# hyrise/hyrise

Hardware: AMD Instinct MI355X
Metric: rows/sec TableScan+JoinHash, TPC-H SF10 lineitem (higher is better)
Workload: dtype u16

## Files before the change

### __graft_entry__.py

```python
import os
import subprocess
import sys

ROOT = os.path.dirname(os.path.abspath(__file__))
CSRC = os.path.join(ROOT, "hyrise_amd", "csrc")
LIB = os.path.join(ROOT, "hyrise_amd", "libhyrise_amd.so")
HIP_SOURCES = ["runtime.hip", "scan.hip", "join.hip", "aggregate.hip", "aggregate_wide.hip", "aggregate_widest.hip", "projection.hip", "projection_expression.hip", "scan_expression.hip", "exchange.hip", "boundary.hip", "comm.hip", "plan.hip", "result_pool.hip", "sort.hip", "union_positions.hip", "join_sort_merge.hip", "join_nested_loop.hip", "product.hip", "like.hip", "string_order.hip", "string_gather.hip"]


def _newer(target, sources):
    if not os.path.exists(target):
        return True
    t = os.path.getmtime(target)
    return any(os.path.getmtime(s) > t for s in sources)


def _build_library(sources, deps, force):
    from concurrent.futures import ThreadPoolExecutor
    hipcc = os.environ.get("HIPCC", "/opt/rocm/bin/hipcc")
    flags = ["--offload-arch=gfx950", "-O3", "-std=c++17", "-fPIC", "-Wall", "-Wno-unused-function"] + os.environ.get("HY_CXXFLAGS", "").split()
    import hashlib
    objdir = os.path.join(ROOT, "build", "obj" + ("-" + hashlib.sha1(" ".join(flags).encode()).hexdigest()[:8] if os.environ.get("HY_CXXFLAGS") else ""))
    os.makedirs(objdir, exist_ok=True)
    headers = [d for d in deps if not d.endswith(".hip")]
    jobs = []
    for source in sources:
        obj = os.path.join(objdir, os.path.basename(source)[:-4] + ".o")
        included = [os.path.join(CSRC, "aggregate.hip")] if source.endswith(("aggregate_wide.hip", "aggregate_widest.hip")) else []
        if force or _newer(obj, [source] + included + headers):
            jobs.append([hipcc] + flags + ["-c", source, "-o", obj])
    with ThreadPoolExecutor(max_workers=max(1, min(len(jobs), os.cpu_count() or 1))) as pool:
        for result in pool.map(lambda cmd: subprocess.run(cmd, cwd=ROOT, capture_output=True, text=True), jobs):
            if result.returncode != 0:
                sys.stderr.write(result.stdout + result.stderr)
                raise subprocess.CalledProcessError(result.returncode, result.args)
            if result.stderr.strip():
                sys.stderr.write(result.stderr)
    objects = [os.path.join(objdir, os.path.basename(source)[:-4] + ".o") for source in sources]
    subprocess.check_call([hipcc, "--offload-arch=gfx950", "-shared", "-fPIC", "-o", os.environ.get("HY_LIBRARY_OUT", LIB)] + objects + ["-ldl"], cwd=ROOT)


def build(force=False):
    sources = [os.path.join(CSRC, s) for s in HIP_SOURCES]
    deps = sources + [os.path.join(CSRC, h) for h in ("hy_device.hpp", "hy_options.hpp", "hy_decode.hpp", "hy_arithmetic.hpp", "hy_scan_job.hpp", "hy_expression.hpp", "hy_expression_rows.hpp", "join_pkfk.hpp", "join_star.hpp", "aggregate_small.hpp", "fused_small.hpp", "sort_words.hpp", "sort_keys.hpp", "join_outer_emit.hpp", "string_entries.hpp")] + [os.path.join(ROOT, "include", "hyrise_amd.h")]
    if force or _newer(LIB, deps):
        _build_library(sources, deps, force)
    host_tests = os.path.join(ROOT, "tests", "cpp", "host_tests")
    host_sources = [os.path.join(ROOT, "tests", "cpp", "host_tests.cpp"), os.path.join(ROOT, "hyrise_amd", "host", "hyrise_host.hpp"), LIB]
    if force or _newer(host_tests, host_sources):
        subprocess.check_call(["g++", "-std=c++17", "-O1", "-Wall", "-Wno-unused-function", "-o", host_tests, host_sources[0],
                               "-L" + os.path.join(ROOT, "hyrise_amd"), "-lhyrise_amd", "-Wl,-rpath,$ORIGIN/../../hyrise_amd"], cwd=ROOT)
    sort_tests = os.path.join(ROOT, "tests", "cpp", "sort_tests")
    sort_sources = [os.path.join(ROOT, "tests", "cpp", "sort_tests.cpp"), host_sources[1], LIB]
    if force or _newer(sort_tests, sort_sources):
        subprocess.check_call(["g++", "-std=c++17", "-O1", "-Wall", "-Wno-unused-function", "-o", sort_tests, sort_sources[0],
                               "-L" + os.path.join(ROOT, "hyrise_amd"), "-lhyrise_amd", "-Wl,-rpath,$ORIGIN/../../hyrise_amd"], cwd=ROOT)
    union_tests = os.path.join(ROOT, "tests", "cpp", "union_positions_tests")
    union_sources = [os.path.join(ROOT, "tests", "cpp", "union_positions_tests.cpp"), host_sources[1], LIB]
    if force or _newer(union_tests, union_sources):
        subprocess.check_call(["g++", "-std=c++17", "-O1", "-Wall", "-Wno-unused-function", "-o", union_tests, union_sources[0],
                               "-L" + os.path.join(ROOT, "hyrise_amd"), "-lhyrise_amd", "-Wl,-rpath,$ORIGIN/../../hyrise_amd"], cwd=ROOT)
    smj_tests = os.path.join(ROOT, "tests", "cpp", "join_sort_merge_tests")
    smj_sources = [os.path.join(ROOT, "tests", "cpp", "join_sort_merge_tests.cpp"), host_sources[1], LIB]
    if force or _newer(smj_tests, smj_sources):
        subprocess.check_call(["g++", "-std=c++17", "-O1", "-Wall", "-Wno-unused-function", "-o", smj_tests, smj_sources[0],
                               "-L" + os.path.join(ROOT, "hyrise_amd"), "-lhyrise_amd", "-Wl,-rpath,$ORIGIN/../../hyrise_amd"], cwd=ROOT)
    nlj_tests = os.path.join(ROOT, "tests", "cpp", "join_nested_loop_tests")
    nlj_sources = [os.path.join(ROOT, "tests", "cpp", "join_nested_loop_tests.cpp"), host_sources[1], LIB]
    if force or _newer(nlj_tests, nlj_sources):
        subprocess.check_call(["g++", "-std=c++17", "-O1", "-Wall", "-Wno-unused-function", "-o", nlj_tests, nlj_sources[0],
                               "-L" + os.path.join(ROOT, "hyrise_amd"), "-lhyrise_amd", "-Wl,-rpath,$ORIGIN/../../hyrise_amd"], cwd=ROOT)
    limit_tests = os.path.join(ROOT, "tests", "cpp", "limit_tests")
    limit_sources = [os.path.join(ROOT, "tests", "cpp", "limit_tests.cpp"), host_sources[1], LIB]
    if force or _newer(limit_tests, limit_sources):
        subprocess.check_call(["g++", "-std=c++17", "-O1", "-Wall", "-Wno-unused-function", "-o", limit_tests, limit_sources[0],
                               "-L" + os.path.join(ROOT, "hyrise_amd"), "-lhyrise_amd", "-Wl,-rpath,$ORIGIN/../../hyrise_amd"], cwd=ROOT)
    aggregate_columns_tests = os.path.join(ROOT, "tests", "cpp", "aggregate_columns_tests")
    aggregate_columns_sources = [os.path.join(ROOT, "tests", "cpp", "aggregate_columns_tests.cpp"), host_sources[1], LIB]
    if force or _newer(aggregate_columns_tests, aggregate_columns_sources):
        subprocess.check_call(["g++", "-std=c++17", "-O1", "-Wall", "-Wno-unused-function", "-o", aggregate_columns_tests, aggregate_columns_sources[0],
                               "-L" + os.path.join(ROOT, "hyrise_amd"), "-lhyrise_amd", "-Wl,-rpath,$ORIGIN/../../hyrise_amd"], cwd=ROOT)
    in_list_tests = os.path.join(ROOT, "tests", "cpp", "in_list_tests")
    in_list_sources = [os.path.join(ROOT, "tests", "cpp", "in_list_tests.cpp"), host_sources[1], LIB]
    if force or _newer(in_list_tests, in_list_sources):
        subprocess.check_call(["g++", "-std=c++17", "-O1", "-Wall", "-Wno-unused-function", "-o", in_list_tests, in_list_sources[0],
                               "-L" + os.path.join(ROOT, "hyrise_amd"), "-lhyrise_amd", "-Wl,-rpath,$ORIGIN/../../hyrise_amd"], cwd=ROOT)
    projection_tests = os.path.join(ROOT, "tests", "cpp", "projection_tests")
    projection_sources = [os.path.join(ROOT, "tests", "cpp", "projection_tests.cpp"), host_sources[1], LIB]
    if force or _newer(projection_tests, projection_sources):
        subprocess.check_call(["g++", "-std=c++17", "-O1", "-Wall", "-Wno-unused-function", "-o", projection_tests, projection_sources[0],
                               "-L" + os.path.join(ROOT, "hyrise_amd"), "-lhyrise_amd", "-Wl,-rpath,$ORIGIN/../../hyrise_amd"], cwd=ROOT)
    expression_scan_tests = os.path.join(ROOT, "tests", "cpp", "expression_scan_tests")
    expression_scan_sources = [os.path.join(ROOT, "tests", "cpp", "expression_scan_tests.cpp"), host_sources[1], LIB]
    if force or _newer(expression_scan_tests, expression_scan_sources):
        subprocess.check_call(["g++", "-std=c++17", "-O1", "-Wall", "-Wno-unused-function", "-o", expression_scan_tests, expression_scan_sources[0],
                               "-L" + os.path.join(ROOT, "hyrise_amd"), "-lhyrise_amd", "-Wl,-rpath,$ORIGIN/../../hyrise_amd"], cwd=ROOT)
    product_tests = os.path.join(ROOT, "tests", "cpp", "product_tests")
    product_sources = [os.path.join(ROOT, "tests", "cpp", "product_tests.cpp"), host_sources[1], LIB]
    if force or _newer(product_tests, product_sources):
        subprocess.check_call(["g++", "-std=c++17", "-O1", "-Wall", "-Wno-unused-function", "-o", product_tests, product_sources[0],
                               "-L" + os.path.join(ROOT, "hyrise_amd"), "-lhyrise_amd", "-Wl,-rpath,$ORIGIN/../../hyrise_amd"], cwd=ROOT)
    like_device_tests = os.path.join(ROOT, "tests", "cpp", "like_device_tests")
    like_device_sources = [os.path.join(ROOT, "tests", "cpp", "like_device_tests.cpp"), host_sources[1], LIB]
    if force or _newer(like_device_tests, like_device_sources):
        subprocess.check_call(["g++", "-std=c++17", "-O1", "-Wall", "-Wno-unused-function", "-o", like_device_tests, like_device_sources[0],
                               "-L" + os.path.join(ROOT, "hyrise_amd"), "-lhyrise_amd", "-Wl,-rpath,$ORIGIN/../../hyrise_amd"], cwd=ROOT)
    string_columns_tests = os.path.join(ROOT, "tests", "cpp", "string_columns_tests")
    string_columns_sources = [os.path.join(ROOT, "tests", "cpp", "string_columns_tests.cpp"), host_sources[1], LIB]
    if force or _newer(string_columns_tests, string_columns_sources):
        subprocess.check_call(["g++", "-std=c++17", "-O1", "-Wall", "-Wno-unused-function", "-o", string_columns_tests, string_columns_sources[0],
                               "-L" + os.path.join(ROOT, "hyrise_amd"), "-lhyrise_amd", "-Wl,-rpath,$ORIGIN/../../hyrise_amd"], cwd=ROOT)
    string_order_tests = os.path.join(ROOT, "tests", "cpp", "string_order_tests")
    string_order_sources = [os.path.join(ROOT, "tests", "cpp", "string_order_tests.cpp"), host_sources[1], LIB]
    if force or _newer(string_order_tests, string_order_sources):
        subprocess.check_call(["g++", "-std=c++17", "-O1", "-Wall", "-Wno-unused-function", "-o", string_order_tests, string_order_sources[0],
                               "-L" + os.path.join(ROOT, "hyrise_amd"), "-lhyrise_amd", "-Wl,-rpath,$ORIGIN/../../hyrise_amd"], cwd=ROOT)
    string_gather_tests = os.path.join(ROOT, "tests", "cpp", "string_gather_tests")
    string_gather_sources = [os.path.join(ROOT, "tests", "cpp", "string_gather_tests.cpp"), host_sources[1], LIB]
    if force or _newer(string_gather_tests, string_gather_sources):
        subprocess.check_call(["g++", "-std=c++17", "-O1", "-Wall", "-Wno-unused-function", "-o", string_gather_tests, string_gather_sources[0],
                               "-L" + os.path.join(ROOT, "hyrise_amd"), "-lhyrise_amd", "-Wl,-rpath,$ORIGIN/../../hyrise_amd"], cwd=ROOT)
    chain = os.path.join(ROOT, "tests", "cpp", "operator_chain")
    chain_sources = [os.path.join(ROOT, "tests", "cpp", "operator_chain.cpp"), host_sources[1], LIB]
    if force or _newer(chain, chain_sources):
        subprocess.check_call(["g++", "-std=c++17", "-O2", "-Wall", "-Wno-unused-function", "-o", chain, chain_sources[0],
                               "-L" + os.path.join(ROOT, "hyrise_amd"), "-lhyrise_amd", "-ldl", "-Wl,-rpath,$ORIGIN/../../hyrise_amd"], cwd=ROOT)
    multi_tests = os.path.join(ROOT, "tests", "cpp", "multi_gpu_tests")
    multi_sources = [os.path.join(ROOT, "tests", "cpp", "multi_gpu_tests.cpp"), os.path.join(ROOT, "hyrise_amd", "host", "multi_gpu.hpp"), host_sources[1], LIB]
    if force or _newer(multi_tests, multi_sources):
        subprocess.check_call(["g++", "-std=c++17", "-O1", "-Wall", "-Wno-unused-function", "-pthread", "-o", multi_tests, multi_sources[0],
                               "-L" + os.path.join(ROOT, "hyrise_amd"), "-lhyrise_amd", "-Wl,-rpath,$ORIGIN/../../hyrise_amd"], cwd=ROOT)
    subprocess.check_call(["make", "-s", "-C", os.path.join(ROOT, "oracle"), "liboracle.so"])
    reference = os.environ.get("HY_REFERENCE", "/root/reference")
    if os.path.isdir(os.path.join(reference, "third_party", "tpch-dbgen")):
        subprocess.check_call(["make", "-s", "-C", os.path.join(ROOT, "oracle"), "ref", f"REFERENCE={reference}"])
    if ROOT not in sys.path:
        sys.path.insert(0, ROOT)
    import hyrise_amd
    from hyrise_amd import abi
    abi.load_library()


def smoke():
    if ROOT not in sys.path:
        sys.path.insert(0, ROOT)
    sys.path.insert(0, os.path.join(ROOT, "tests"))
    import numpy as np
    from hyrise_amd import abi
    from hyrise_amd.operators import make_predicate, table_scan
    from hyrise_amd.storage import DeviceColumn, make_column
    import support

    lib = abi.load_library()
    abi.check(lib.hy_init(0))
    rng = np.random.default_rng(1)
    days = (rng.integers(0, 2406, 500_000) + rng.integers(1, 122, 500_000)).astype(np.int32)
    host = make_column(days, None, abi.ENC_DICTIONARY)
    dev = DeviceColumn(host)
    predicate = make_predicate(abi.PRED_BETWEEN_UPPER_EXCLUSIVE, abi.TYPE_INT, 731, 1096)
    got = table_scan(dev, predicate)
    want = support.oracle_scan(host, predicate)
    support.assert_scan_equal(got, want, "smoke")
    print(f"smoke OK: {got.total} matches of {host.rows} rows, PosLists bit-identical to the oracle")


if __name__ == "__main__":
    build(force="--force" in sys.argv)
    if "--smoke" in sys.argv:
        smoke()
```

### hyrise_amd/abi.py

```python
import ctypes as C
import os

HERE = os.path.dirname(os.path.abspath(__file__))
LIB_PATH = os.path.join(HERE, "libhyrise_amd.so")

OK, ERR_INVALID, ERR_UNSUPPORTED, ERR_DEVICE, ERR_CAPACITY = 0, 1, 2, 3, 4
TYPE_NULL, TYPE_INT, TYPE_LONG, TYPE_FLOAT, TYPE_DOUBLE, TYPE_STRING = range(6)
(PRED_EQUALS, PRED_NOT_EQUALS, PRED_LESS_THAN, PRED_LESS_THAN_EQUALS, PRED_GREATER_THAN, PRED_GREATER_THAN_EQUALS,
 PRED_BETWEEN_INCLUSIVE, PRED_BETWEEN_LOWER_EXCLUSIVE, PRED_BETWEEN_UPPER_EXCLUSIVE, PRED_BETWEEN_EXCLUSIVE,
 PRED_IN, PRED_NOT_IN, PRED_LIKE, PRED_NOT_LIKE, PRED_LIKE_INSENSITIVE, PRED_NOT_LIKE_INSENSITIVE,
 PRED_IS_NULL, PRED_IS_NOT_NULL) = range(18)
(JOIN_INNER, JOIN_LEFT, JOIN_RIGHT, JOIN_FULL_OUTER, JOIN_CROSS, JOIN_SEMI, JOIN_ANTI_NULL_AS_TRUE,
 JOIN_ANTI_NULL_AS_FALSE) = range(8)
AGG_MIN, AGG_MAX, AGG_SUM, AGG_AVG, AGG_COUNT, AGG_COUNT_DISTINCT, AGG_STDDEV_SAMP, AGG_ANY = range(8)
ENC_UNENCODED, ENC_DICTIONARY, ENC_FRAME_OF_REFERENCE, ENC_REFERENCE, ENC_MVCC, ENC_RUN_LENGTH, ENC_LZ4 = range(7)
SORT_NONE, SORT_ASCENDING_NULLS_FIRST, SORT_DESCENDING_NULLS_FIRST, SORT_ASCENDING_NULLS_LAST, SORT_DESCENDING_NULLS_LAST = range(5)
MEM_HOST, MEM_DEVICE = 0, 1
CHUNK_SCANNED, CHUNK_ALL_MATCH, CHUNK_NONE_MATCH = 0, 1, 2
INVALID_VALUE_ID = 0xFFFFFFFF
INVALID_CHUNK_ID = 0xFFFFFFFF
FOR_BLOCK_SIZE = 2048
SCAN_MATERIALIZE_ALL_MATCH = 1
SCAN_CHUNK_REGIONS = 2
POSLIST_DENSE, POSLIST_CHUNK_REGIONS = 0, 1
POOL_KEEP_MEDIAN = 1
CHUNK_DEFAULT_SIZE = 65535


class RowID(C.Structure):
    _fields_ = [("chunk_id", C.c_uint32), ("chunk_offset", C.c_uint32)]


class Segment(C.Structure):
    _fields_ = [("encoding", C.c_uint32), ("data_type", C.c_uint32), ("size", C.c_uint32), ("width", C.c_uint32),
                ("data", C.c_void_p), ("aux", C.c_void_p), ("aux_size", C.c_uint32), ("ref_chunk_id", C.c_uint32),
                ("nulls", C.c_void_p), ("ref", C.c_void_p), ("sorted_by", C.c_uint32), ("bits", C.c_uint32)]


class Lz4Blocks(C.Structure):
    _fields_ = [("blocks", C.POINTER(C.c_void_p)), ("block_bytes", C.POINTER(C.c_uint32)), ("block_count", C.c_uint32), ("block_size", C.c_uint32),
                ("last_block_size", C.c_uint32), ("dictionary_bytes", C.c_uint32), ("dictionary", C.c_void_p)]


class Value(C.Union):
    _fields_ = [("i32", C.c_int32), ("i64", C.c_int64), ("f32", C.c_float), ("f64", C.c_double),
                ("value_id", C.c_uint32)]


class Predicate(C.Structure):
    _fields_ = [("condition", C.c_uint32), ("value_type", C.c_uint32), ("value", Value), ("value2", Value),
                ("per_chunk_lower", C.c_void_p), ("per_chunk_upper", C.c_void_p), ("per_chunk_found", C.c_void_p),
                ("column_is_nullable", C.c_uint32), ("reserved", C.c_uint32), ("match_words", C.c_void_p), ("match_word_offsets", C.c_void_p)]


MAX_IN_LIST = 256
MAX_LIKE_PATTERN = 256
LIKE_ANY_ONE, LIKE_ANY_RUN = 0x100, 0x200


class StringDictionaryChunk(C.Structure):
    _fields_ = [("n_entries", C.c_uint32), ("string_length", C.c_uint32), ("chars", C.c_void_p), ("offsets", C.c_void_p)]


class InList(C.Structure):
    _fields_ = [("value_type", C.c_uint32), ("n_values", C.c_uint32), ("values", C.c_void_p), ("negated", C.c_uint32), ("column_is_nullable", C.c_uint32),
                ("per_chunk_value_ids", C.c_void_p)]


class ScanResult(C.Structure):
    _fields_ = [("mem", C.c_uint32), ("flags", C.c_uint32), ("matches", C.c_void_p), ("capacity", C.c_uint64),
                ("offsets", C.c_void_p), ("counts", C.c_void_p), ("chunk_state", C.c_void_p),
                ("total_matches", C.c_uint64)]


class JoinResult(C.Structure):
    _fields_ = [("mem", C.c_uint32), ("radix_bits", C.c_uint32), ("left_pos", C.c_void_p), ("right_pos", C.c_void_p),
                ("capacity", C.c_uint64), ("slice_offsets", C.c_void_p), ("slice_capacity", C.c_uint32),
                ("n_slices", C.c_uint32), ("n_pairs", C.c_uint64), ("left_is_build", C.c_uint32),
                ("flags", C.c_uint32), ("status", C.c_void_p)]


JOIN_ASYNC = 1


class JoinStatus(C.Structure):
    _fields_ = [("n_pairs", C.c_uint64), ("n_slices", C.c_uint32), ("fits", C.c_uint32), ("build_confirmed", C.c_uint32), ("error", C.c_uint32),
                ("reserved", C.c_uint64)]


class SortMergeResult(C.Structure):
    _fields_ = [("mem", C.c_uint32), ("reserved", C.c_uint32), ("left_pos", C.c_void_p), ("right_pos", C.c_void_p), ("capacity", C.c_uint64),
                ("n_pairs", C.c_uint64), ("n_matched", C.c_uint64), ("n_left_outer", C.c_uint64)]


class NestedLoopResult(C.Structure):
    _fields_ = [("mem", C.c_uint32), ("reserved", C.c_uint32), ("left_pos", C.c_void_p), ("right_pos", C.c_void_p), ("capacity", C.c_uint64), ("n_pairs", C.c_uint64)]


class ProductResult(C.Structure):
    _fields_ = [("mem", C.c_uint32), ("reserved", C.c_uint32), ("left_pos", C.c_void_p), ("right_pos", C.c_void_p), ("pair_offsets", C.c_void_p),
                ("capacity", C.c_uint64), ("n_rows", C.c_uint64)]


class JoinPredicate(C.Structure):
    _fields_ = [("left_column", C.c_void_p), ("right_column", C.c_void_p), ("condition", C.c_uint32), ("reserved", C.c_uint32)]


MAX_SECONDARY_PREDICATES = 4
NLJ_MAX_COMPARISONS = 250_000_000_000
NLJ_MAX_TEMPORARY_BYTES = 1 << 31
(OPT_ALLOW_ANY_ARCH, OPT_JOIN_RANK_TABLE, OPT_JOIN_HINT, OPT_JOIN_BREAK_HINT, OPT_JOIN_PKFK, OPT_JOIN_LDS_BUILD, OPT_JOIN_LDS_BUILD_TILES, OPT_JOIN_FILL_WGS_PER_CU,
 OPT_JOIN_HAND_OVER_RANKS, OPT_AGG_PARTITION_BITS, OPT_AGG_SPILL_SHIFT, OPT_AGG_SMALL_DOMAIN, OPT_FUSED_SMALL_DOMAIN, OPT_SCAN_TWO_COLUMNS, OPT_STAR_FUSED_PROBE, OPT_STAR_FUSED_FINISH,
 OPT_LDS_ORDERED_ATOMICS, OPT_PRODUCT_NONTEMPORAL) = range(18)
KERNEL_OTHER, KERNEL_SCAN, KERNEL_JOIN_PROBE, KERNEL_JOIN_COUNT, KERNEL_JOIN_BUILD, KERNEL_AGGREGATE, KERNEL_PROJECTION, KERNEL_LIKE, KERNEL_STRING_RANK = range(9)
ARITH_ADD, ARITH_SUB, ARITH_MUL, ARITH_DIV, ARITH_MOD = range(5)


class Operand(C.Structure):
    _fields_ = [("column", C.c_void_p), ("literal_type", C.c_uint32), ("literal", Value)]


MAX_PROJECTION_NODES, MAX_PROJECTION_DEPTH, MAX_PROJECTION_COLUMNS, MAX_PROJECTION_TESTS = 32, 6, 8, 4
(PROJ_COLUMN, PROJ_LITERAL, PROJ_ARITHMETIC, PROJ_COMPARISON, PROJ_COLUMN_TEST, PROJ_IS_NULL, PROJ_IS_NOT_NULL, PROJ_AND, PROJ_OR, PROJ_UNARY_MINUS, PROJ_CASE,
 PROJ_BETWEEN, PROJ_CAST, PROJ_EXTRACT, PROJ_FUNCTION, PROJ_SUBQUERY, PROJ_PARAMETER) = range(17)


class ProjectionNode(C.Structure):
    _fields_ = [("kind", C.c_uint32), ("op", C.c_uint32), ("index", C.c_uint32), ("literal_type", C.c_uint32), ("literal", Value)]


class ProjectionTest(C.Structure):
    _fields_ = [("column", C.c_void_p), ("predicate", Predicate), ("in_list", C.POINTER(InList))]


class ProjectionProgram(C.Structure):
    _fields_ = [("n_nodes", C.c_uint32), ("n_columns", C.c_uint32), ("n_tests", C.c_uint32), ("reserved", C.c_uint32),
                ("columns", C.c_void_p * MAX_PROJECTION_COLUMNS), ("tests", ProjectionTest * MAX_PROJECTION_TESTS), ("nodes", ProjectionNode * MAX_PROJECTION_NODES)]


UNION_FORCE_SORT = 1
UNION_MAX_CLUSTERS = 8
SORT_LIMIT_FORCE_FULL_SORT, SORT_LIMIT_FORCE_SELECT = 1, 2


class SortKey(C.Structure):
    _fields_ = [("column", C.c_void_p), ("mode", C.c_uint32), ("reserved", C.c_uint32)]


class AggregateSpec(C.Structure):
    _fields_ = [("function", C.c_uint32), ("column", C.c_void_p)]


EXPR_COLUMN, EXPR_LITERAL, EXPR_ARITHMETIC = range(3)
MAX_EXPRESSION_NODES, MAX_FILTERS = 12, 4
FILTER_VALIDATE = 0x100


class ExpressionNode(C.Structure):
    _fields_ = [("kind", C.c_uint32), ("op", C.c_uint32), ("column", C.c_void_p), ("literal_type", C.c_uint32), ("reserved", C.c_uint32),
                ("literal", Value)]


class Expression(C.Structure):
    _fields_ = [("n_nodes", C.c_uint32), ("reserved", C.c_uint32), ("nodes", ExpressionNode * MAX_EXPRESSION_NODES)]


class Filter(C.Structure):
    _fields_ = [("column", C.c_void_p), ("predicate", Predicate)]


class FusedAggregate(C.Structure):
    _fields_ = [("function", C.c_uint32), ("reserved", C.c_uint32), ("input", C.POINTER(Expression))]


class AggregateColumn(C.Structure):
    _fields_ = [("data_type", C.c_uint32), ("reserved", C.c_uint32), ("values", C.c_void_p), ("is_null", C.c_void_p)]


class AggregateResult(C.Structure):
    _fields_ = [("mem", C.c_uint32), ("group_capacity", C.c_uint32), ("n_groups", C.c_uint32),
                ("reserved", C.c_uint32), ("group_row_ids", C.c_void_p), ("columns", C.POINTER(AggregateColumn))]


class AggregateColumns(C.Structure):
    _fields_ = [("skip_groupby_mask", C.c_uint64), ("n_groups", C.c_uint32), ("reserved", C.c_uint32),
                ("aggregate_columns", C.POINTER(C.c_void_p)), ("groupby_columns", C.POINTER(C.c_void_p)), ("group_row_ids", C.c_void_p)]


STAR_NO_OP = 0xFFFFFFFF
MAX_STAR_DIMENSIONS, MAX_STAR_AGGREGATES = 8, 8


class StarDimension(C.Structure):
    _fields_ = [("key", C.c_void_p), ("filter_column", C.c_void_p), ("predicate", Predicate), ("fact_key", C.c_void_p)]


class StarColumn(C.Structure):
    _fields_ = [("table", C.c_uint32), ("reserved", C.c_uint32), ("column", C.c_void_p)]


class StarAggregate(C.Structure):
    _fields_ = [("function", C.c_uint32), ("op", C.c_uint32), ("left", StarColumn), ("right", StarColumn)]


MAX_STAR_FILTERS = 4


class StarFilter(C.Structure):
    _fields_ = [("column", C.c_void_p), ("predicate", Predicate), ("in_list", C.POINTER(InList))]


class StarDimensionWhere(C.Structure):
    _fields_ = [("key", C.c_void_p), ("fact_key", C.c_void_p), ("filters", C.POINTER(StarFilter)), ("n_filters", C.c_uint32), ("reserved", C.c_uint32)]


SYMBOLS = [
    ("hy_abi_version", C.c_int32, []),
    ("hy_init", C.c_int32, [C.c_int32]),
    ("hy_set_option", C.c_int32, [C.c_uint32, C.c_int64]),
    ("hy_get_option", C.c_int32, [C.c_uint32, C.POINTER(C.c_int64)]),
    ("hy_shutdown", C.c_int32, []),
    ("hy_last_error", C.c_char_p, []),
    ("hy_set_stream", C.c_int32, [C.c_void_p]),
    ("hy_synchronize", C.c_int32, []),
    ("hy_device_malloc", C.c_int32, [C.POINTER(C.c_void_p), C.c_size_t]),
    ("hy_device_free", C.c_int32, [C.c_void_p]),
    ("hy_memcpy_h2d", C.c_int32, [C.c_void_p, C.c_void_p, C.c_size_t]),
    ("hy_memcpy_d2h", C.c_int32, [C.c_void_p, C.c_void_p, C.c_size_t]),
    ("hy_device_count", C.c_int32, [C.POINTER(C.c_int32)]),
    ("hy_set_profiling", C.c_int32, [C.c_int32]),
    ("hy_profile_read", C.c_int32, [C.POINTER(C.c_float), C.POINTER(C.c_uint32)]),
    ("hy_profile_read_kernel", C.c_int32, [C.c_uint32, C.POINTER(C.c_float), C.POINTER(C.c_uint32)]),
    ("hy_profile_event_overhead", C.c_int32, [C.POINTER(C.c_float)]),
    ("hy_bind_device", C.c_int32, [C.c_int32]),
    ("hy_comm_unique_id", C.c_int32, [C.c_void_p]),
    ("hy_comm_init_rank", C.c_int32, [C.c_void_p, C.c_uint32, C.c_uint32, C.POINTER(C.c_void_p)]),
    ("hy_comm_init_all", C.c_int32, [C.POINTER(C.c_int32), C.c_uint32, C.POINTER(C.c_void_p)]),
    ("hy_comm_destroy", C.c_int32, [C.c_void_p]),
    ("hy_comm_rank", C.c_int32, [C.c_void_p, C.POINTER(C.c_uint32), C.POINTER(C.c_uint32)]),
    ("hy_comm_group_begin", C.c_int32, []),
    ("hy_comm_group_end", C.c_int32, []),
    ("hy_comm_all_reduce", C.c_int32, [C.c_void_p, C.c_void_p, C.c_void_p, C.c_uint64, C.c_uint32, C.c_uint32]),
    ("hy_comm_all_gather", C.c_int32, [C.c_void_p, C.c_void_p, C.c_void_p, C.c_uint64]),
    ("hy_comm_all_to_all_v", C.c_int32, [C.c_void_p, C.c_void_p, C.POINTER(C.c_uint64), C.c_void_p, C.POINTER(C.c_uint64)]),
    ("hy_column_create", C.c_int32, [C.POINTER(Segment), C.c_uint32, C.c_uint32, C.POINTER(C.c_void_p)]),
    ("hy_column_destroy", C.c_int32, [C.c_void_p]),
    ("hy_column_row_count", C.c_int32, [C.c_void_p, C.POINTER(C.c_uint64)]),
    ("hy_column_chunk_count", C.c_int32, [C.c_void_p, C.POINTER(C.c_uint32)]),
    ("hy_table_scan", C.c_int32, [C.c_void_p, C.POINTER(Predicate), C.c_void_p, C.c_uint32, C.POINTER(ScanResult)]),
    ("hy_table_scan_in_list", C.c_int32, [C.c_void_p, C.POINTER(InList), C.c_void_p, C.c_uint32, C.POINTER(ScanResult)]),
    ("hy_string_dictionary_create", C.c_int32, [C.POINTER(StringDictionaryChunk), C.c_uint32, C.c_uint32, C.POINTER(C.c_void_p)]),
    ("hy_string_dictionary_destroy", C.c_int32, [C.c_void_p]),
    ("hy_string_dictionary_match_layout", C.c_int32, [C.c_void_p, C.c_void_p]),
    ("hy_like_tokenize", C.c_int32, [C.c_char_p, C.c_uint32, C.c_uint32, C.c_void_p, C.POINTER(C.c_uint32)]),
    ("hy_like_matches", C.c_int32, [C.c_void_p, C.c_char_p, C.c_uint32, C.c_uint32, C.c_uint32, C.c_void_p]),
    ("hy_table_scan_like", C.c_int32, [C.c_void_p, C.c_void_p, C.c_char_p, C.c_uint32, C.c_uint32, C.c_uint32, C.c_void_p, C.c_uint32, C.POINTER(ScanResult)]),
    ("hy_in_list_cast", C.c_int32, [C.c_uint32, C.c_void_p, C.c_void_p, C.c_uint32, C.c_void_p, C.POINTER(C.c_uint32), C.POINTER(C.c_uint32)]),
    ("hy_table_scan_columns", C.c_int32, [C.c_void_p, C.c_void_p, C.c_uint32, C.POINTER(ScanResult)]),
    ("hy_string_dictionary_ranks", C.c_int32, [C.c_void_p, C.c_void_p, C.c_uint32, C.c_void_p]),
    ("hy_table_scan_columns_strings", C.c_int32, [C.c_void_p, C.c_void_p, C.c_void_p, C.c_void_p, C.c_uint32, C.POINTER(ScanResult)]),
    ("hy_string_dictionary_order", C.c_int32, [C.c_void_p, C.c_uint32, C.c_void_p, C.POINTER(C.c_uint32)]),
    ("hy_column_string_ranks", C.c_int32, [C.c_void_p, C.c_void_p, C.POINTER(C.c_void_p)]),
    ("hy_string_column_gather", C.c_int32, [C.c_void_p, C.c_void_p, C.c_void_p, C.c_uint64, C.c_uint32, C.POINTER(C.c_void_p), C.POINTER(C.c_void_p)]),
    ("hy_string_ranks_gather", C.c_int32, [C.c_void_p, C.c_void_p, C.POINTER(C.c_void_p), C.POINTER(C.c_void_p)]),
    ("hy_string_dictionary_chunk_size", C.c_int32, [C.c_void_p, C.c_uint32, C.POINTER(C.c_uint32), C.POINTER(C.c_uint64)]),
    ("hy_string_dictionary_read_chunk", C.c_int32, [C.c_void_p, C.c_uint32, C.c_void_p, C.c_void_p]),
    ("hy_projection_arithmetic", C.c_int32, [C.c_uint32, C.POINTER(Operand), C.POINTER(Operand), C.POINTER(C.c_void_p)]),
    ("hy_projection_expression", C.c_int32, [C.POINTER(ProjectionProgram), C.POINTER(C.c_void_p)]),
    ("hy_table_scan_expression", C.c_int32, [C.POINTER(ProjectionProgram), C.c_void_p, C.c_uint32, C.POINTER(ScanResult)]),
    ("hy_column_read_chunk", C.c_int32, [C.c_void_p, C.c_uint32, C.c_void_p, C.c_void_p]),
    ("hy_column_data_type", C.c_uint32, [C.c_void_p]),
    ("hy_column_chunk_rows", C.c_uint32, [C.c_void_p, C.c_uint32]),
    ("hy_validate", C.c_int32, [C.c_void_p, C.c_uint32, C.c_uint32, C.c_uint32, C.POINTER(ScanResult)]),
    ("hy_predicate_cast", C.c_int32, [C.c_uint32, C.c_uint32, C.c_uint32, C.c_void_p, C.c_uint32, C.c_void_p, C.POINTER(Predicate)]),
    ("hy_join_output_chunks", C.c_int32, [C.c_void_p, C.c_uint32, C.c_void_p, C.POINTER(C.c_uint32)]),
    ("hy_poslist_translate", C.c_int32, [C.c_void_p, C.POINTER(ScanResult), C.c_uint32, C.c_void_p, C.c_uint64, C.POINTER(C.c_uint64)]),
    ("hy_join_hash", C.c_int32, [C.c_void_p, C.c_void_p, C.c_uint32, C.POINTER(JoinResult)]),
    ("hy_join_hash_finish", C.c_int32, [C.c_void_p, C.c_void_p, C.c_uint32, C.POINTER(JoinResult)]),
    ("hy_join_hash_predicates", C.c_int32, [C.c_void_p, C.c_void_p, C.c_uint32, C.POINTER(JoinPredicate), C.c_uint32, C.POINTER(JoinResult)]),
    ("hy_join_hash_radix_bits", C.c_int32, [C.c_uint64, C.c_uint64, C.POINTER(C.c_uint32)]),
    ("hy_join_hash_count", C.c_int32, [C.c_void_p, C.c_void_p, C.c_uint32, C.POINTER(C.c_uint64)]),
    ("hy_join_sort_merge", C.c_int32, [C.c_void_p, C.c_void_p, C.c_uint32, C.c_uint32, C.POINTER(SortMergeResult)]),
    ("hy_join_sort_merge_count", C.c_int32, [C.c_void_p, C.c_void_p, C.c_uint32, C.c_uint32, C.POINTER(C.c_uint64)]),
    ("hy_join_nested_loop", C.c_int32, [C.c_void_p, C.c_void_p, C.c_uint32, C.c_uint32, C.POINTER(JoinPredicate), C.c_uint32, C.POINTER(NestedLoopResult)]),
    ("hy_join_nested_loop_count", C.c_int32, [C.c_void_p, C.c_void_p, C.c_uint32, C.c_uint32, C.POINTER(JoinPredicate), C.c_uint32, C.POINTER(C.c_uint64)]),
    ("hy_product", C.c_int32, [C.c_void_p, C.c_void_p, C.POINTER(ProductResult)]),
    ("hy_product_count", C.c_int32, [C.c_void_p, C.c_void_p, C.POINTER(C.c_uint64)]),
    ("hy_aggregate_hash", C.c_int32, [C.POINTER(C.c_void_p), C.c_uint32, C.POINTER(AggregateSpec), C.c_uint32,
                                      C.POINTER(AggregateResult)]),
    ("hy_aggregate_hash_columns", C.c_int32, [C.POINTER(C.c_void_p), C.c_uint32, C.POINTER(AggregateSpec), C.c_uint32, C.c_uint32,
                                              C.POINTER(AggregateColumns)]),
    ("hy_star_join_aggregate", C.c_int32, [C.POINTER(StarDimension), C.c_uint32, C.POINTER(StarColumn), C.c_uint32, C.POINTER(StarAggregate), C.c_uint32,
                                           C.POINTER(AggregateResult), C.POINTER(C.c_uint64)]),
    ("hy_star_join_aggregate_where", C.c_int32, [C.POINTER(StarDimensionWhere), C.c_uint32, C.POINTER(StarFilter), C.c_uint32, C.POINTER(StarColumn), C.c_uint32,
                                                 C.POINTER(StarAggregate), C.c_uint32, C.POINTER(AggregateResult), C.POINTER(C.c_uint64)]),
    ("hy_scan_project_aggregate", C.c_int32, [C.POINTER(Filter), C.c_uint32, C.POINTER(C.c_void_p), C.c_uint32, C.POINTER(FusedAggregate), C.c_uint32,
                                              C.POINTER(AggregateResult)]),
    ("hy_column_export", C.c_int32, [C.c_void_p, C.c_void_p, C.c_void_p]),
    ("hy_repartition_count", C.c_int32, [C.c_void_p, C.c_uint32, C.POINTER(C.c_uint64)]),
    ("hy_repartition_pack", C.c_int32, [C.c_void_p, C.c_uint32, C.c_uint32, C.c_void_p, C.c_void_p, C.c_uint64, C.POINTER(C.c_uint64)]),
    ("hy_gather_row_ids", C.c_int32, [C.c_void_p, C.c_uint64, C.c_uint32, C.c_void_p, C.c_uint64, C.c_void_p]),
    ("hy_poslist_gather", C.c_int32, [C.c_void_p, C.c_void_p, C.c_uint64, C.c_void_p]),
    ("hy_sort", C.c_int32, [C.POINTER(SortKey), C.c_uint32, C.c_void_p, C.c_uint64, C.POINTER(C.c_uint64)]),
    ("hy_sort_limit", C.c_int32, [C.POINTER(SortKey), C.c_uint32, C.c_uint64, C.c_uint32, C.c_void_p, C.c_uint64, C.POINTER(C.c_uint64), C.POINTER(C.c_uint32)]),
    ("hy_column_gather", C.c_int32, [C.c_void_p, C.c_void_p, C.c_uint64, C.c_uint32, C.POINTER(C.c_void_p)]),
    ("hy_union_positions", C.c_int32, [C.POINTER(C.c_void_p), C.POINTER(C.c_void_p), C.c_uint32, C.c_uint32, C.POINTER(C.c_void_p), C.c_uint64, C.POINTER(C.c_uint64),
                                       C.POINTER(C.c_uint32)]),
    ("hy_result_pool_acquire", C.c_int32, [C.c_uint64, C.POINTER(C.c_void_p)]),
    ("hy_result_pool_acquire_pair", C.c_int32, [C.c_uint64, C.POINTER(C.c_void_p), C.POINTER(C.c_void_p)]),
    ("hy_result_pool_release", C.c_int32, [C.c_void_p]),
    ("hy_result_pool_calibrate", C.c_int32, [C.c_void_p, C.c_void_p, C.c_uint32, C.c_uint64, C.c_uint32, C.c_uint32, C.POINTER(C.c_float), C.POINTER(C.c_uint32)]),
    ("hy_result_pool_trim", C.c_int32, []),
    ("hy_result_pool_stats", C.c_int32, [C.POINTER(C.c_uint64), C.POINTER(C.c_uint64), C.POINTER(C.c_uint32)]),
]


class HyriseAmdError(RuntimeError):
    def __init__(self, status, message):
        super().__init__(f"hyrise_amd status {status}: {message}")
        self.status = status


_lib = None


def load_library():
    global _lib
    if _lib is not None:
        return _lib
    path = os.environ.get("HY_LIBRARY", LIB_PATH)
    if not os.path.exists(path):
        raise ImportError(f"{path} is missing: run `python -c 'import __graft_entry__ as g; g.build()'` "
                          "(hipcc --offload-arch=gfx950). hyrise_amd has no CPU fallback.")
    lib = C.CDLL(path)
    for name, restype, argtypes in SYMBOLS:
        fn = getattr(lib, name)
        fn.restype = restype
        fn.argtypes = argtypes
    _lib = lib
    return lib


def check(status):
    if status != OK:
        raise HyriseAmdError(status, load_library().hy_last_error().decode("utf-8", "replace"))


class option:

    def __init__(self, option_id, value):
        self.option_id, self.value, self.before = option_id, value, C.c_int64(0)

    def __enter__(self):
        lib = load_library()
        check(lib.hy_get_option(self.option_id, C.byref(self.before)))
        check(lib.hy_set_option(self.option_id, self.value))
        return self

    def __exit__(self, *exc):
        check(load_library().hy_set_option(self.option_id, self.before.value))
        return False


_SWITCHES = {
    "HY_SCAN_NO_TWO_COLUMNS": (OPT_SCAN_TWO_COLUMNS, 0), "HY_STAR_NO_FUSED_PROBE": (OPT_STAR_FUSED_PROBE, 0), "HY_STAR_NO_FUSED_FINISH": (OPT_STAR_FUSED_FINISH, 0),
    "HY_JOIN_NO_RANK_TABLE": (OPT_JOIN_RANK_TABLE, 0), "HY_JOIN_NO_HINT": (OPT_JOIN_HINT, 0), "HY_JOIN_BREAK_HINT": (OPT_JOIN_BREAK_HINT, None),
    "HY_JOIN_NO_PKFK": (OPT_JOIN_PKFK, 0), "HY_JOIN_NO_LDS_BUILD": (OPT_JOIN_LDS_BUILD, 0), "HY_JOIN_LDS_BUILD_TILES": (OPT_JOIN_LDS_BUILD_TILES, None),
    "HY_JOIN_FILL_WGS_PER_CU": (OPT_JOIN_FILL_WGS_PER_CU, None), "HY_JOIN_HAND_OVER_RANKS": (OPT_JOIN_HAND_OVER_RANKS, None),
    "HY_AGG_PARTITION_BITS": (OPT_AGG_PARTITION_BITS, None), "HY_AGG_SPILL_SHIFT": (OPT_AGG_SPILL_SHIFT, None), "HY_AGG_NO_SMALL_DOMAIN": (OPT_AGG_SMALL_DOMAIN, 0),
    "HY_FUSED_NO_SMALL_DOMAIN": (OPT_FUSED_SMALL_DOMAIN, 0), "HY_LDS_NO_ORDERED_ATOMICS": (OPT_LDS_ORDERED_ATOMICS, 0)
}


class switches:

    def __init__(self, named):
        self.named, self.stack, self.env = dict(named), [], []

    def __enter__(self):
        for name, value in self.named.items():
            if name in _SWITCHES:
                option_id, fixed = _SWITCHES[name]
                o = option(option_id, fixed if fixed is not None else int(value))
                o.__enter__()
                self.stack.append(o)
            else:
                self.env.append((name, os.environ.get(name)))
                os.environ[name] = str(value)
        return self

    def __exit__(self, *exc):
        for o in reversed(self.stack):
            o.__exit__(*exc)
        for name, before in self.env:
            if before is None:
                del os.environ[name]
            else:
                os.environ[name] = before
        return False
```

### hyrise_amd/csrc/join.hip

```cpp
#include "hy_device.hpp"
#include "hy_decode.hpp"
#include "hy_arithmetic.hpp"
#include "hy_scan_job.hpp"

#include <algorithm>
#include <atomic>
#include <cmath>
#include <chrono>
#include <cstring>
#include <type_traits>

namespace hy {

constexpr uint32_t JOIN_TILE = 4096;
constexpr uint32_t JOIN_THREADS = 512;
constexpr uint32_t JOIN_WAVES = JOIN_THREADS / 64;
constexpr uint32_t JOIN_WAVE_ROWS = JOIN_TILE / JOIN_WAVES;
constexpr uint32_t JOIN_ROUNDS = JOIN_WAVE_ROWS / 64;
constexpr uint32_t JOIN_STAGE = JOIN_TILE + 256;
constexpr uint32_t MAX_PARTITIONS = 256;
typedef uint32_t u32x2_t __attribute__((ext_vector_type(2)));
typedef uint32_t u32x4_t __attribute__((ext_vector_type(4)));
constexpr uint32_t PROBE_SIZE_PER_CHUNK = 65535u * 2u;
constexpr uint32_t BLOOM_BITS = 1u << 20;
// ... 3351 lines not shown
  Directory& d = b.directory;
  d.keys = nullptr;
  d.keys32 = nullptr;
  d.row_ids = job.plan.id32 ? nullptr : b.rows.as<hy_row_id>();
  d.ids32 = job.plan.id32 ? b.rows.as<uint32_t>() : nullptr;
  d.n = total;
  d.key_min = mailbox->key_min;
  d.key_max = mailbox->key_max;
  d.shift = 0;
  d.n_buckets = 1;
  d.dir = nullptr;
  return HY_OK;
}

static hy_status sort_build_keys(BuildJob& job, uint64_t key_bits_or) {
  BuildSide& b = job.b;
  const bool key32 = job.plan.key32, id32 = job.plan.id32;
  HY_TRY(b.keys_tmp.alloc((key32 ? 4 : 8) * (job.total + 4)));
  HY_TRY(b.rows_tmp.alloc((id32 ? 4 : 8) * job.total));
  const bool staged = key32 && id32 && lds_atomics_are_lane_ordered(job.stream);
  uint32_t moving_bytes = 0;
  for (uint32_t byte = 0; byte < 8; ++byte)
    if (((key_bits_or >> (8 * byte)) & 0xFF) != 0 || (!key32 && (key_bits_or >> 63))) moving_bytes |= 1u << byte;
  void* keys = b.keys.ptr;
  void* rows = b.rows.ptr;
  HY_TRY(lsd_sort_passes(key32, id32, staged, &keys, &rows, b.keys_tmp.ptr, b.rows_tmp.ptr, job.total, moving_bytes, job.stream));
  if (keys != b.keys.ptr) { swap(b.keys, b.keys_tmp); swap(b.rows, b.rows_tmp); }
  if (key32) HY_HIP(hipMemsetAsync(b.keys.as<uint32_t>() + job.total, 0, 16, job.stream));
  return HY_OK;
}

static hy_status build_directory(BuildJob& job, bool ends_known, uint64_t first_key, uint64_t last_key) {
  BuildSide& b = job.b;
  const bool key32 = job.plan.key32, id32 = job.plan.id32;
  const uint64_t total = job.total;
  Directory& d = b.directory;
  d.keys = key32 ? nullptr : b.keys.as<uint64_t>();
  d.keys32 = key32 ? b.keys.as<uint32_t>() : nullptr;
  d.row_ids = id32 ? nullptr : b.rows.as<hy_row_id>();
  d.ids32 = id32 ? b.rows.as<uint32_t>() : nullptr;
  d.n = total;
  d.key_min = d.key_max = 0;
  d.shift = 0;
  d.n_buckets = 1;
  if (total) {
    if (!ends_known) {
      JoinMailbox* mailbox = nullptr;
      JoinMailbox* mailbox_dev = nullptr;
      HY_TRY(join_mailbox(&mailbox, &mailbox_dev));
      with_key_type(key32, [&](auto key) {
        using K = decltype(key);
        hipLaunchKernelGGL(publish_build_flags<K>, dim3(1), dim3(1), 0, job.stream, b.flags.as<uint32_t>(), b.keys.as<K>(), total, mailbox_dev);
      });
      HY_HIP(hipStreamSynchronize(job.stream));
      first_key = mailbox->first_key;
      last_key = mailbox->last_key;
    }
    d.key_min = first_key;
    d.key_max = last_key;
    uint32_t buckets = 1;
    while (buckets < total && buckets < (1u << 27)) buckets <<= 1;
    const uint64_t range = d.key_max - d.key_min;
    uint32_t shift = 0;
    while (shift < 64 && (range >> shift) >= buckets) ++shift;
    d.shift = shift;
    d.n_buckets = static_cast<uint32_t>((range >> shift) + 1);
  }
  HY_TRY(b.dir.alloc(4 * (size_t{d.n_buckets} + 2)));
  d.dir = b.dir.as<uint32_t>();
  if (!total) {
    HY_HIP(hipMemsetAsync(b.dir.ptr, 0, 4 * (size_t{d.n_buckets} + 2), job.stream));
    return HY_OK;
  }
  const dim3 grid(static_cast<uint32_t>((total + 255) / 256));
  with_key_type(key32, [&](auto key) {
    using K = decltype(key);
    hipLaunchKernelGGL(directory_fill<K>, grid, dim3(256), 0, job.stream, b.keys.as<K>(), total, d.key_min, d.shift, d.n_buckets, b.dir.as<uint32_t>());
  });
  return HY_OK;
}

static hy_status prepare_build(const hy_column* build, const BuildWants& wants, BuildSide& b, hipStream_t stream) {
  BuildJob job{build, wants, plan_build(build, wants), b, stream};
  const uint32_t n_slices = build->n_slices;
  HY_TRY(job.counts.alloc(4 * size_t{n_slices + 1}));
  HY_TRY(job.offsets.alloc(8 * size_t{n_slices + 2}));
  HY_TRY(b.flags.alloc(64));
  if (wants.bloom) {
    HY_TRY(b.bloom.alloc(BLOOM_BITS));
    if (!job.plan.hinted) HY_HIP(hipMemsetAsync(b.bloom.ptr, 0, BLOOM_BITS, stream));
  }
  MaterializeArgs& m = job.m;
  m.segments = build->d_segments;
  m.views = build->d_slice_views;
  m.slices = build->d_slices;
  m.n_slices = n_slices;
  m.keep_nulls = wants.keep_nulls;
  m.bloom_in = nullptr;
  m.bloom_out = wants.bloom ? b.bloom.as<uint8_t>() : nullptr;
  m.slice_counts = job.counts.as<uint32_t>();
  m.any_null = b.flags.as<uint32_t>() + 2;
  m.hashed_type = wants.hashed_type;
  if (n_slices && job.plan.dense) {
    m.row_base = build->d_row_base;
    job.total = build->rows;
  } else if (n_slices) {
    hipLaunchKernelGGL((join_materialize<0, false, false>), dim3(n_slices), dim3(256), 0, stream, m);
    hipLaunchKernelGGL(scan_counts, dim3(1), dim3(1024), 0, stream, job.counts.as<uint32_t>(), job.offsets.as<uint64_t>(), n_slices);
    HY_HIP(hipMemcpyAsync(&job.total, job.offsets.as<uint64_t>() + n_slices, 8, hipMemcpyDeviceToHost, stream));
    HY_HIP(hipStreamSynchronize(stream));
  }
  b.n = job.total;
  if (job.plan.identity_candidate && job.total) {
    if (job.plan.hinted) return fill_hinted(job);
    bool built = false;
    HY_TRY(fill_identity(job, &built));
    if (built) return HY_OK;
  }
  JoinMailbox* mailbox = nullptr;
  JoinMailbox* mailbox_dev = nullptr;
  HY_TRY(materialise_keys(job, &mailbox, &mailbox_dev));
  bool ends_known = false;
  uint64_t first_key = 0, last_key = 0;
  if (job.total) {
    ends_known = mailbox->unsorted == 0;
    first_key = mailbox->first_key;
    last_key = mailbox->last_key;
    bool rank_table = false;
    HY_TRY(rank_table_from_keys(job, mailbox, mailbox_dev, &rank_table));
    if (rank_table) return HY_OK;
    if (mailbox->unsorted) HY_TRY(sort_build_keys(job, mailbox->key_or));
  }
  return build_directory(job, ends_known, first_key, last_key);
}

static uint32_t stream_grid(uint32_t n_tiles, int workgroups_per_cu) {
  uint32_t per_cu = workgroups_per_cu > 0 ? static_cast<uint32_t>(workgroups_per_cu) : 1;
  if (FIXED_JOIN_WGS_PER_CU > 0) per_cu = static_cast<uint32_t>(FIXED_JOIN_WGS_PER_CU);
  const uint32_t resident = device_cu_count() * per_cu / 8 * 8;
  const uint32_t needed = 8 * (((n_tiles + 7) / 8 + STREAM_WAVES - 1) / STREAM_WAVES);
  return std::max<uint32_t>(8, std::min<uint32_t>(resident, needed));
}

static uint32_t device_cu_count() {
  int device = 0, cus = 256;
  (void)hipGetDevice(&device);
  (void)hipDeviceGetAttribute(&cus, hipDeviceAttributeMultiprocessorCount, device);
  return static_cast<uint32_t>(cus);
}

#include "join_star.hpp"

static thread_local int t_last_join_used_rank_table = 0;
static thread_local int t_last_join_used_pkfk = 0;
static thread_local int t_last_join_hinted_attempt = 0;
static thread_local int t_last_join_hinted = 0;
static thread_local bool t_join_returned_async = false;
constexpr uint32_t JOIN_TRACE_TILES = 1u << 15;
static uint64_t* g_join_trace = nullptr;
static uint32_t g_join_trace_tiles = 0;

static bool same_chunk_layout(const hy_column* a, const hy_column* b) {
  if (a->n_chunks != b->n_chunks) return false;
  for (uint32_t c = 0; c < a->n_chunks; ++c) if (a->host_segments[c].size != b->host_segments[c].size) return false;
  return true;
}

static uint32_t flip_condition(uint32_t condition) {
  switch (condition) {
    case HY_PRED_LESS_THAN: return HY_PRED_GREATER_THAN;
    case HY_PRED_LESS_THAN_EQUALS: return HY_PRED_GREATER_THAN_EQUALS;
    case HY_PRED_GREATER_THAN: return HY_PRED_LESS_THAN;
    case HY_PRED_GREATER_THAN_EQUALS: return HY_PRED_LESS_THAN_EQUALS;
    default: return condition;
  }
}

static std::atomic<int> g_lds_atomic_order{0};
static std::atomic<int> g_lds_order_in_effect{0};
static bool lds_atomics_are_lane_ordered(hipStream_t stream) {
  if (!option(HY_OPT_LDS_ORDERED_ATOMICS)) {
    g_lds_order_in_effect.store(2, std::memory_order_relaxed);
    return false;
  }
  int state = g_lds_atomic_order.load(std::memory_order_acquire);
  if (state == 0) {
    state = 2;
    uint32_t* failures = nullptr;
    if (hipMalloc(reinterpret_cast<void**>(&failures), 4) == hipSuccess) {
      uint32_t host = 1;
      bool ok = hipMemsetAsync(failures, 0, 4, stream) == hipSuccess;
      for (uint32_t seed = 0; ok && seed < 4; ++seed) hipLaunchKernelGGL(lds_atomic_order_probe, dim3(512), dim3(512), 0, stream, failures, seed);
      ok = ok && hipMemcpyAsync(&host, failures, 4, hipMemcpyDeviceToHost, stream) == hipSuccess && hipStreamSynchronize(stream) == hipSuccess;
      (void)hipFree(failures);
      if (ok && host == 0) state = 1;
    }
    g_lds_atomic_order.store(state, std::memory_order_release);
  }
  g_lds_order_in_effect.store(state, std::memory_order_relaxed);
  return state == 1;
}


hy_status sort_pairs_u32(uint32_t** keys, uint32_t** ids, uint32_t* keys_tmp, uint32_t* ids_tmp, uint64_t n, uint32_t key_bits, hipStream_t stream) {
  if (n < 2) return HY_OK;
  const uint32_t moving_bytes = (1u << std::min<uint32_t>(4, (key_bits + 7) / 8)) - 1;
  void* sorted_keys = *keys;
  void* sorted_ids = *ids;
  HY_TRY(lsd_sort_passes(true, true, lds_atomics_are_lane_ordered(stream), &sorted_keys, &sorted_ids, keys_tmp, ids_tmp, n, moving_bytes, stream));
  *keys = static_cast<uint32_t*>(sorted_keys);
  *ids = static_cast<uint32_t*>(sorted_ids);
  return HY_OK;
}

static bool probe_keys_scattered(const hy_column* probe) {
  for (uint32_t c = 0; c < probe->n_chunks; ++c) {
    const hy_segment& seg = probe->host_segments[c];
    if (!(seg.encoding == HY_ENC_FRAME_OF_REFERENCE && seg.width <= 2)) return true;
  }
  return false;
}

__global__ __launch_bounds__(64) void sample_key_spans(const SliceView* views, uint32_t n_slices, uint32_t* local_samples) {
  const uint32_t slice = static_cast<uint32_t>((static_cast<uint64_t>(blockIdx.x) * n_slices) / gridDim.x);
  const SliceView view = views[slice];
  if (view.row_count < 64 || (view.kind != VIEW_INT32 && view.kind != VIEW_FOR32)) return;
  const uint32_t row = view.row_begin + ((blockIdx.x * 2654435761u) % (view.row_count - 63)) + threadIdx.x;
  uint32_t key = static_cast<const uint32_t*>(view.data)[row];
  if (view.kind == VIEW_FOR32) key += static_cast<uint32_t>(static_cast<const int32_t*>(view.aux)[row / HY_FOR_BLOCK_SIZE]);
  int32_t low = static_cast<int32_t>(key), high = static_cast<int32_t>(key);
  for (int d = 32; d > 0; d >>= 1) {
    const int32_t other_low = __shfl_xor(low, d), other_high = __shfl_xor(high, d);
    low = other_low < low ? other_low : low;
    high = other_high > high ? other_high : high;
  }
  if (threadIdx.x == 0 && static_cast<int64_t>(high) - static_cast<int64_t>(low) < 65536) atomicAdd(local_samples, 1u);
}

static hy_status probe_keys_lack_locality(const hy_column* probe, hipStream_t stream, bool* scattered) {
  *scattered = false;
  if (!probe_keys_scattered(probe) || !probe->d_slice_views || probe->n_slices == 0) return HY_OK;
  uint32_t known = probe->join_hint.probe_locality.load(std::memory_order_relaxed);
  if (known == 0) {
    constexpr uint32_t SAMPLES = 1024;
    uint32_t* host = nullptr;
    uint32_t* mapped = nullptr;
    HY_TRY(pinned_staging(64, reinterpret_cast<void**>(&host), reinterpret_cast<void**>(&mapped)));
    DeviceBuffer counter;
    HY_TRY(counter.alloc(64));
    HY_HIP(hipMemsetAsync(counter.ptr, 0, 4, stream));
    hipLaunchKernelGGL(sample_key_spans, dim3(SAMPLES), dim3(64), 0, stream, probe->d_slice_views, probe->n_slices, counter.as<uint32_t>());
    HY_HIP(hipMemcpyAsync(host, counter.ptr, 4, hipMemcpyDeviceToHost, stream));
    HY_HIP(hipStreamSynchronize(stream));
    known = *host * 4 >= SAMPLES * 3 ? 1u : 2u;
    probe->join_hint.probe_locality.store(known, std::memory_order_relaxed);
  }
  *scattered = known == 2;
  return HY_OK;
}

struct JoinRequest {
  const hy_column* build;
  const hy_column* probe;
  bool build_right;
  uint32_t mode;
  bool semi_anti;
  bool keep_nulls_build;
  bool keep_nulls_probe;
  uint32_t hashed_type;
  bool general;
  uint32_t radix_bits;
  bool host_result;
  bool count_only;
  bool async;
  bool probe_filtered;
  bool pack_build_ids;
  hy_join_result* result;
  uint64_t* count_out;
  hy_row_id* user_build;
  hy_row_id* user_probe;
  uint64_t* user_slice_offsets;
  uint64_t capacity;
  uint32_t slice_capacity;
  uint32_t n_secondary;
  SecondaryPredicate secondary[HY_MAX_SECONDARY_PREDICATES];
};

static bool builds_over_right_input(const hy_column* left, const hy_column* right, uint32_t mode) {
  return mode == HY_JOIN_LEFT || mode == HY_JOIN_ANTI_NULL_AS_TRUE || mode == HY_JOIN_ANTI_NULL_AS_FALSE || mode == HY_JOIN_SEMI || (mode == HY_JOIN_INNER && left->rows > right->rows);
}

static hy_status resolve_join_request(const hy_column* left, const hy_column* right, uint32_t mode, hy_join_result* result, bool count_only, uint64_t* count_out,
                                      const hy_join_predicate* secondary, uint32_t n_secondary, JoinRequest* request) {
  if (mode == HY_JOIN_FULL_OUTER || mode == HY_JOIN_CROSS || mode > HY_JOIN_ANTI_NULL_AS_FALSE) return fail(HY_ERR_UNSUPPORTED, "JoinHash does not support join mode %u (join_hash.cpp:38-44)", mode);
  if (n_secondary > HY_MAX_SECONDARY_PREDICATES) return fail(HY_ERR_UNSUPPORTED, "more than %u secondary join predicates stay on the CPU path", HY_MAX_SECONDARY_PREDICATES);
  if (n_secondary && mode == HY_JOIN_ANTI_NULL_AS_TRUE) return fail(HY_ERR_UNSUPPORTED, "JoinHash does not support secondary predicates with AntiNullAsTrue (join_hash.cpp:39-44)");
  for (uint32_t p = 0; p < n_secondary; ++p) {
    const hy_join_predicate& predicate = secondary[p];
    if (!predicate.left_column || !predicate.right_column) return fail(HY_ERR_INVALID, "secondary join predicate %u: column missing", p);
    if (predicate.condition > HY_PRED_GREATER_THAN_EQUALS) return fail(HY_ERR_INVALID, "secondary join predicate %u: condition %u is no comparison", p, predicate.condition);
    for (const hy_column* column : {predicate.left_column, predicate.right_column}) {
      if (column->is_mvcc || (column->ref && column->ref->is_mvcc)) return fail(HY_ERR_INVALID, "MVCC columns are read by hy_validate only");
      if (column->data_type < HY_TYPE_INT || column->data_type > HY_TYPE_DOUBLE) return fail(HY_ERR_UNSUPPORTED, "secondary join predicates on strings stay on the CPU path");
    }
    if (!same_chunk_layout(predicate.left_column, left) || !same_chunk_layout(predicate.right_column, right))
      return fail(HY_ERR_INVALID, "secondary join predicate %u: the columns do not have the chunk layout of the join's input tables", p);
  }
  for (const hy_column* column : {left, right}) {
    if (column->is_mvcc || (column->ref && column->ref->is_mvcc)) return fail(HY_ERR_INVALID, "MVCC columns are read by hy_validate only");
    if (column->data_type < HY_TYPE_INT || column->data_type > HY_TYPE_DOUBLE) return fail(HY_ERR_UNSUPPORTED, "string join keys stay on the CPU path");
  }
  JoinRequest& q = *request;
  q = JoinRequest{};
  const uint32_t l = left->data_type, r = right->data_type;
  const bool l_float = l == HY_TYPE_FLOAT || l == HY_TYPE_DOUBLE, r_float = r == HY_TYPE_FLOAT || r == HY_TYPE_DOUBLE;
  if (l_float && r_float) q.hashed_type = (l == HY_TYPE_DOUBLE || r == HY_TYPE_DOUBLE) ? HY_TYPE_DOUBLE : HY_TYPE_FLOAT;
  else if (l_float || r_float) q.hashed_type = l_float ? l : r;
  q.general = n_secondary != 0 || q.hashed_type != 0;
  q.mode = mode;
  q.build_right = builds_over_right_input(left, right, mode);
  q.build = q.build_right ? right : left;
  q.probe = q.build_right ? left : right;
  q.semi_anti = mode == HY_JOIN_SEMI || mode == HY_JOIN_ANTI_NULL_AS_TRUE || mode == HY_JOIN_ANTI_NULL_AS_FALSE;
  q.keep_nulls_build = mode == HY_JOIN_ANTI_NULL_AS_TRUE;
  q.keep_nulls_probe = mode == HY_JOIN_LEFT || mode == HY_JOIN_RIGHT || mode == HY_JOIN_ANTI_NULL_AS_TRUE || mode == HY_JOIN_ANTI_NULL_AS_FALSE;
  q.radix_bits = calculate_radix_bits(q.build->rows);
  if (result && result->radix_bits != 0xFFFFFFFFu) q.radix_bits = result->radix_bits;
  if (q.radix_bits > 8) return fail(HY_ERR_INVALID, "radix_bits %u > 8", q.radix_bits);
  q.result = result;
  q.count_only = count_only;
  q.count_out = count_out;
  q.host_result = !result || result->mem == HY_MEM_HOST;
  q.async = !count_only && !q.host_result && (result->flags & HY_JOIN_ASYNC) && result->status;
  q.capacity = count_only ? ~0ull : result->capacity;
  q.slice_capacity = count_only ? 0xFFFFFFFFu : result->slice_capacity;
  if (!q.host_result && !count_only &&
      (reinterpret_cast<uintptr_t>(result->left_pos) % 16 != 0 || reinterpret_cast<uintptr_t>(result->right_pos) % 16 != 0 || reinterpret_cast<uintptr_t>(result->slice_offsets) % 8 != 0))
    return fail(HY_ERR_INVALID, "hy_join_hash: a device-memory result needs left_pos / right_pos on 16-byte and slice_offsets on 8-byte boundaries");
  if (!count_only) {
    q.user_build = q.build_right ? result->right_pos : result->left_pos;
    q.user_probe = q.build_right ? result->left_pos : result->right_pos;
    q.user_slice_offsets = result->slice_offsets;
    if (!q.user_probe && result->capacity) return fail(HY_ERR_INVALID, "join result: PosList buffer for the probe side missing");
    if (!q.semi_anti && !q.user_build && result->capacity) return fail(HY_ERR_INVALID, "join result: PosList buffer for the build side missing");
    if (!q.user_slice_offsets) return fail(HY_ERR_INVALID, "join result: slice_offsets missing");
  }
  q.probe_filtered = q.build->rows < q.probe->rows && !q.keep_nulls_probe;
  q.pack_build_ids = !q.semi_anti && !count_only && q.build->n_chunks <= 65536;
  for (uint32_t c = 0; c < q.build->n_chunks && q.pack_build_ids; ++c) q.pack_build_ids = q.build->host_segments[c].size <= 65536;
  q.n_secondary = n_secondary;
  for (uint32_t p = 0; p < n_secondary; ++p) {
    q.secondary[p].build = (q.build_right ? secondary[p].right_column : secondary[p].left_column)->d_segments;
    q.secondary[p].probe = (q.build_right ? secondary[p].left_column : secondary[p].right_column)->d_segments;
    q.secondary[p].condition = q.build_right ? flip_condition(secondary[p].condition) : secondary[p].condition;
  }
  return HY_OK;
}

static bool probe_takes_pk_kernels(const JoinRequest& q, hipStream_t stream, bool* probe_views) {
  const hy_column* probe = q.probe;
  bool views = !probe->is_reference && probe->n_slices > 0 && FIXED_JOIN_FETCH_AHEAD;
  for (uint32_t c = 0; c < probe->n_chunks && views; ++c) {
    const hy_segment& seg = probe->host_segments[c];
    views = !seg.nulls && reinterpret_cast<uintptr_t>(seg.data) % 16 == 0 && ((seg.encoding == HY_ENC_UNENCODED && seg.data_type == HY_TYPE_INT) || seg.encoding == HY_ENC_FRAME_OF_REFERENCE);
  }
  *probe_views = views;
  return views && q.hashed_type == 0 && q.n_secondary == 0 && probe->rows < 0xFFFF0000ull && option(HY_OPT_JOIN_PKFK) && (q.count_only || q.capacity <= 0xFFFFFFFFull) &&
         lds_atomics_are_lane_ordered(stream);
}

static bool hint_confirmed(const JoinRequest& q, const BuildSide& b, const JoinMailbox* mailbox, bool* retry) {
  if (!b.hinted || !mailbox->build_unconfirmed) return true;
  q.build->join_hint.state.store(2, std::memory_order_release);
  *retry = true;
  return false;
}

static uint64_t* attach_join_trace(uint32_t n_tiles) {
  if (!HY_DEBUG_ENV("HY_JOIN_TRACE")) return nullptr;
  static uint64_t* trace_buffer = nullptr;
  if (!trace_buffer) (void)hipMalloc(reinterpret_cast<void**>(&trace_buffer), 8 * 6 * JOIN_TRACE_TILES);
  if (n_tiles > JOIN_TRACE_TILES) return nullptr;
  g_join_trace = trace_buffer;
  g_join_trace_tiles = n_tiles;
  return trace_buffer;
}

struct JoinOutput {
  DeviceBuffer d_build, d_probe, d_slice_offsets;
  hy_row_id* build = nullptr;
  hy_row_id* probe = nullptr;
  uint64_t* slice_offsets = nullptr;
};

static hy_status begin_output(const JoinRequest& q, uint32_t max_slices, JoinOutput& out) {
  out.build = q.semi_anti ? nullptr : q.user_build;
  out.probe = q.user_probe;
  out.slice_offsets = q.user_slice_offsets;
  if (q.count_only || !q.host_result) return HY_OK;
  HY_TRY(out.d_slice_offsets.alloc(8 * (size_t{max_slices} + 2)));
  out.slice_offsets = out.d_slice_offsets.as<uint64_t>();
  return HY_OK;
}

static hy_status size_output_lists(const JoinRequest& q, const JoinMailbox* mailbox, hipStream_t stream, StageClock& clock, JoinOutput& out) {
  if (!q.host_result) return HY_OK;
  HY_HIP(hipStreamSynchronize(stream));
  clock.mark("pass 1 done");
  if (!mailbox->fits) return HY_OK;
  if (!q.semi_anti) {
    HY_TRY(out.d_build.alloc(8 * mailbox->n_pairs));
    out.build = out.d_build.as<hy_row_id>();
  }
  HY_TRY(out.d_probe.alloc(8 * mailbox->n_pairs));
  out.probe = out.d_probe.as<hy_row_id>();
  return HY_OK;
}

static hy_status copy_output_back(const JoinRequest& q, const JoinMailbox* mailbox, hipStream_t stream, const JoinOutput& out) {
  if (!q.host_result || !mailbox->fits) return HY_OK;
  if (mailbox->n_pairs) {
    HY_HIP(hipMemcpyAsync(q.user_probe, out.probe, 8 * mailbox->n_pairs, hipMemcpyDeviceToHost, stream));
    if (!q.semi_anti) HY_HIP(hipMemcpyAsync(q.user_build, out.build, 8 * mailbox->n_pairs, hipMemcpyDeviceToHost, stream));
  }
  HY_HIP(hipMemcpyAsync(q.user_slice_offsets, out.slice_offsets, 8 * (size_t{mailbox->n_slices} + 1), hipMemcpyDeviceToHost, stream));
  return HY_OK;
}

static hy_status report_join_result(hy_join_result* result, uint64_t n_pairs, uint32_t n_slices, uint32_t error) {
  result->n_slices = n_slices;
  result->n_pairs = n_pairs;
  if (n_slices > result->slice_capacity) return fail(HY_ERR_CAPACITY, "join produces %u output PosLists, slice capacity is %u", n_slices, result->slice_capacity);
  if (n_pairs > result->capacity) return fail(HY_ERR_CAPACITY, "join produces %llu pairs, capacity is %llu", static_cast<unsigned long long>(n_pairs), static_cast<unsigned long long>(result->capacity));
  if (error) return fail(HY_ERR_UNSUPPORTED, "a probe row matches more than 4 194 303 build rows");
  return HY_OK;
}

static hy_status raise_pk_count_lds() {
  static OncePerDevice raised;
  uint64_t device_bit = 0;
  if (raised.pending(&device_bit)) {
    HY_HIP(hipFuncSetAttribute(reinterpret_cast<const void*>(pk_count_lds), hipFuncAttributeMaxDynamicSharedMemorySize, static_cast<int>(pk_count_lds_bytes(PK_LDS_KEYS - 1, PK_LDS_MAX_PARTITIONS))));
    raised.done(device_bit);
  }
  return HY_OK;
}

static hy_status raise_pk_emit_lds() {
  static OncePerDevice raised;
  uint64_t device_bit = 0;
  if (raised.pending(&device_bit)) {
    HY_HIP(hipFuncSetAttribute(reinterpret_cast<const void*>(pk_emit<true>), hipFuncAttributeMaxDynamicSharedMemorySize, 4 * pk_emit_lds_words(MAX_PARTITIONS)));
    HY_HIP(hipFuncSetAttribute(reinterpret_cast<const void*>(pk_emit<false>), hipFuncAttributeMaxDynamicSharedMemorySize, 4 * pk_emit_lds_words(MAX_PARTITIONS)));
    HY_HIP(hipFuncSetAttribute(reinterpret_cast<const void*>(pk_emit<true, true>), hipFuncAttributeMaxDynamicSharedMemorySize, 4 * pk_emit_lds_words(MAX_PARTITIONS)));
    HY_HIP(hipFuncSetAttribute(reinterpret_cast<const void*>(pk_emit<false, true>), hipFuncAttributeMaxDynamicSharedMemorySize, 4 * pk_emit_lds_words(MAX_PARTITIONS)));
    HY_HIP(hipFuncSetAttribute(reinterpret_cast<const void*>(pk_emit<true, false, true>), hipFuncAttributeMaxDynamicSharedMemorySize, 4 * pk_emit_lds_words(MAX_PARTITIONS)));
    raised.done(device_bit);
  }
  return HY_OK;
}

struct PkBuffers {
  DeviceBuffer cells, small, row_masks, row_ranks;
};

static hy_status pk_arguments(const JoinRequest& q, const BuildSide& b, JoinMailbox* mailbox_dev, const JoinOutput& out, uint32_t n_groups, PkBuffers& buffers, PkArgs& k) {
  const uint32_t n_tiles = q.probe->n_slices * PK_TILES_PER_SLICE, partitions = 1u << q.radix_bits;
  const uint32_t stride = (n_tiles + 1 + 3) & ~3u;
  HY_TRY(buffers.cells.alloc(size_t{12} * partitions * stride));
  const size_t at_origin = align_up(8 * size_t{partitions}, 8), at_slice_base = at_origin + 8 * (size_t{partitions} + 1), at_words = align_up(at_slice_base + 4 * (size_t{n_groups} + 1), 8);
  HY_TRY(buffers.small.alloc(at_words + 64));
  k.views = q.probe->d_slice_views;
  k.n_tiles = n_tiles;
  k.stride = stride;
  k.mode = q.mode;
  k.radix_bits = q.radix_bits;
  k.keep_nulls = q.keep_nulls_probe;
  k.n_groups = n_groups;
  k.build_bloom = q.probe_filtered ? b.bloom.as<uint8_t>() : nullptr;
  k.bloom_is_bits = b.bloom_is_bits ? 1u : 0u;
  k.rank = b.rank;
  k.ids32 = b.directory.ids32;
  k.row_ids = b.directory.row_ids;
  k.counts = buffers.cells.as<uint32_t>();
  k.rel_elements = k.counts + size_t{partitions} * stride;
  k.rel_pairs = k.rel_elements + size_t{partitions} * stride;
  char* small_base = buffers.small.as<char>();
  k.totals = reinterpret_cast<uint32_t*>(small_base);
  k.origin_pairs = reinterpret_cast<uint64_t*>(small_base + at_origin);
  k.slice_base = reinterpret_cast<uint32_t*>(small_base + at_slice_base);
  k.group_first_tile = q.probe->d_first_slice;
  k.ticket = reinterpret_cast<uint32_t*>(small_base + at_words);
  k.plan = reinterpret_cast<JoinPlan*>(small_base + at_words + 16);
  k.mailbox = mailbox_dev;
  k.capacity = q.capacity;
  k.slice_capacity = q.slice_capacity;
  if (uint64_t* trace = attach_join_trace(n_tiles)) k.trace = trace;
  k.slice_offsets = out.slice_offsets;
  k.status = q.async ? q.result->status : nullptr;
  k.verdict = b.hinted ? b.verdict : nullptr;
  k.fill_records = b.hinted ? b.fill_records : nullptr;
  k.n_fill_records = b.hinted ? b.n_fill_records : 0;
  k.hint_min = b.hint_min;
  k.hint_max = b.hint_max;
  k.hint_allows_duplicates = b.hint_allows_duplicates ? 1u : 0u;
  return HY_OK;
}

static hy_status launch_pk_count(const JoinRequest& q, const BuildSide& b, PkBuffers& buffers, PkArgs& k, bool* build_in_lds, bool* hand_over_ranks, hipStream_t stream) {
  const uint32_t n_tiles = k.n_tiles, partitions = 1u << q.radix_bits;
  *hand_over_ranks = false;
  *build_in_lds = b.rank.range < PK_LDS_KEYS && partitions <= PK_LDS_MAX_PARTITIONS && n_tiles >= static_cast<uint64_t>(option(HY_OPT_JOIN_LDS_BUILD_TILES)) && option(HY_OPT_JOIN_LDS_BUILD);
  hipEvent_t count_started = nullptr, count_stopped = nullptr;
  if (*build_in_lds) {
    HY_TRY(buffers.row_masks.alloc(size_t{n_tiles} * (2 * PK_TILE / 8)));
    k.row_masks = buffers.row_masks.as<uint8_t>();
    HY_TRY(raise_pk_count_lds());
    const uint32_t groups = std::min<uint32_t>(device_cu_count(), (n_tiles + PK_LDS_SUBTILES - 1) / PK_LDS_SUBTILES);
    profile_events(&count_started, &count_stopped, HY_KERNEL_JOIN_COUNT);
    hipExtLaunchKernelGGL(pk_count_lds, dim3(groups), dim3(1024), pk_count_lds_bytes(b.rank.range, partitions), stream, count_started, count_stopped, 0, k);
    return HY_OK;
  }
  profile_events(&count_started, &count_stopped, HY_KERNEL_JOIN_COUNT);
  const int64_t hand_over_from = option(HY_OPT_JOIN_HAND_OVER_RANKS);
  if (q.mode == HY_JOIN_INNER && !q.count_only && hand_over_from > 0 && q.probe->rows >= static_cast<uint64_t>(hand_over_from) && (b.rank.range >> 5) * 8 >= (hand_over_from == 1 ? 0u : (1u << 20)))
    HY_TRY(probe_keys_lack_locality(q.probe, stream, hand_over_ranks));
  const uint32_t tile_grid = 8 * ((n_tiles + 7) / 8);
  if (*hand_over_ranks) {
    HY_TRY(buffers.row_ranks.alloc(4 * size_t{n_tiles} * PK_TILE));
    k.row_ranks = buffers.row_ranks.as<uint32_t>();
    hipExtLaunchKernelGGL(pk_count<true>, dim3(tile_grid), dim3(PK_COUNT_THREADS), 0, stream, count_started, count_stopped, 0, k);
  } else hipExtLaunchKernelGGL(pk_count<false>, dim3(tile_grid), dim3(PK_COUNT_THREADS), 0, stream, count_started, count_stopped, 0, k);
  return HY_OK;
}

static hy_status launch_pk_emit(const JoinRequest& q, BuildSide& b, PkArgs& k, bool build_in_lds, bool hand_over_ranks, uint32_t max_slices, hipStream_t stream) {
  HY_TRY(raise_pk_emit_lds());
  hipEvent_t started = nullptr, stopped = nullptr;
  profile_events(&started, &stopped, HY_KERNEL_JOIN_PROBE);
  const uint32_t cut_grid = std::min<uint32_t>(max_slices, q.slice_capacity);
  const int64_t group = FIXED_JOIN_EMIT_TILE_GROUP;
  k.emit_group_shift = 32;
  if (group > 0) { k.emit_group_shift = 0; while (k.emit_group_shift < 16 && (int64_t{1} << (k.emit_group_shift + 1)) <= group) ++k.emit_group_shift; }
  k.cut_blocks = (cut_grid + 7) / 8 * 8;
  k.cleaning = b.cleaning;
  const dim3 grid(k.cut_blocks + 8 * ((k.n_tiles + 7) / 8));
  const size_t lds_bytes = 4 * pk_emit_lds_words(1u << q.radix_bits);
  const bool inner = q.mode == HY_JOIN_INNER;
  if (build_in_lds && inner) hipExtLaunchKernelGGL((pk_emit<true, true>), grid, dim3(PK_THREADS), lds_bytes, stream, started, stopped, 0, k);
  else if (build_in_lds) hipExtLaunchKernelGGL((pk_emit<false, true>), grid, dim3(PK_THREADS), lds_bytes, stream, started, stopped, 0, k);
  else if (hand_over_ranks) hipExtLaunchKernelGGL((pk_emit<true, false, true>), grid, dim3(PK_THREADS), lds_bytes, stream, started, stopped, 0, k);
  else if (inner) hipExtLaunchKernelGGL(pk_emit<true>, grid, dim3(PK_THREADS), lds_bytes, stream, started, stopped, 0, k);
  else hipExtLaunchKernelGGL(pk_emit<false>, grid, dim3(PK_THREADS), lds_bytes, stream, started, stopped, 0, k);
  HY_HIP(hipGetLastError());
  block_cleaning_queued(b);
  t_last_join_used_pkfk = build_in_lds ? 2 : 1;
  return HY_OK;
}

static hy_status probe_pkfk(const JoinRequest& q, BuildSide& b, StageClock& clock, bool* retry, hipStream_t stream) {
  const uint32_t partitions = 1u << q.radix_bits;
  const uint32_t n_groups = q.radix_bits ? partitions : q.probe->n_chunks;
  const uint32_t max_slices = static_cast<uint32_t>(q.probe->rows / PROBE_SIZE_PER_CHUNK) + n_groups + 1;
  JoinMailbox* mailbox = nullptr;
  JoinMailbox* mailbox_dev = nullptr;
  HY_TRY(join_mailbox(&mailbox, &mailbox_dev));
  JoinOutput out;
  HY_TRY(begin_output(q, max_slices, out));
  PkBuffers buffers;
  PkArgs k{};
  HY_TRY(pk_arguments(q, b, mailbox_dev, out, n_groups, buffers, k));
  bool build_in_lds = false, hand_over_ranks = false;
  HY_TRY(launch_pk_count(q, b, buffers, k, &build_in_lds, &hand_over_ranks, stream));
  hipLaunchKernelGGL(pk_scan, dim3(partitions), dim3(PK_SCAN_THREADS), 0, stream, k);
  clock.mark("pass 1 launched");
  if (q.count_only) {
    HY_HIP(hipStreamSynchronize(stream));
    if (hint_confirmed(q, b, mailbox, retry) && q.count_out) *q.count_out = mailbox->n_pairs;
    return HY_OK;
  }
  HY_TRY(size_output_lists(q, mailbox, stream, clock, out));
  k.build_out = out.build;
  k.probe_out = out.probe;
  HY_TRY(launch_pk_emit(q, b, k, build_in_lds, hand_over_ranks, max_slices, stream));
  clock.mark("pass 2 launched");
  HY_TRY(copy_output_back(q, mailbox, stream, out));
  if (q.async) {
    t_join_returned_async = true;
    return HY_OK;
  }
  HY_HIP(hipStreamSynchronize(stream));
  clock.mark("pass 2 done");
  if (!hint_confirmed(q, b, mailbox, retry)) return HY_OK;
  return report_join_result(q.result, mailbox->n_pairs, mailbox->n_slices, mailbox->error);
}

static hy_status raise_probe_emit_lds() {
  static OncePerDevice raised;
  uint64_t device_bit = 0;
  if (raised.pending(&device_bit)) {
    HY_HIP(hipFuncSetAttribute(reinterpret_cast<const void*>(probe_emit_cached), hipFuncAttributeMaxDynamicSharedMemorySize, 4 * probe_emit_cached_lds_words(MAX_PARTITIONS)));
    HY_HIP(hipFuncSetAttribute(reinterpret_cast<const void*>(probe_emit_generic<false>), hipFuncAttributeMaxDynamicSharedMemorySize, 4 * probe_emit_lds_words(MAX_PARTITIONS)));
    HY_HIP(hipFuncSetAttribute(reinterpret_cast<const void*>(probe_emit_generic<true>), hipFuncAttributeMaxDynamicSharedMemorySize, 4 * probe_emit_lds_words(MAX_PARTITIONS)));
    HY_HIP(hipFuncSetAttribute(reinterpret_cast<const void*>(rt_probe_emit), hipFuncAttributeMaxDynamicSharedMemorySize, 4 * rt_probe_emit_lds_words(MAX_PARTITIONS)));
    raised.done(device_bit);
  }
  return HY_OK;
}

struct ProbeBuffers {
  DeviceBuffer hist, base, partner, meta, uncached, words, first_cell, origin, slice_base;
  std::vector<uint64_t> group_first_cell;
  uint64_t second_at = 0, cells = 0;
  JoinPlan* plan = nullptr;
};

static hy_status probe_arguments(const JoinRequest& q, const BuildSide& b, JoinMailbox* mailbox_dev, ProbeBuffers& buffers, ProbeArgs& a, hipStream_t stream) {
  const uint32_t n_tiles = q.probe->n_slices * (SLICE_ROWS / JOIN_TILE);
  const uint64_t cells = uint64_t{1u << q.radix_bits} * n_tiles;
  const uint64_t second_at = (cells + 1 + SCAN_BLOCK - 1) / SCAN_BLOCK * SCAN_BLOCK;
  buffers.cells = cells;
  buffers.second_at = second_at;
  HY_TRY(buffers.hist.alloc(4 * (second_at + cells + 1)));
  HY_TRY(buffers.base.alloc(8 * (second_at + cells + 2)));
  a.segments = q.probe->d_segments;
  a.slices = q.probe->d_slices;
  a.views = q.probe->d_slice_views;
  a.n_tiles = n_tiles;
  a.mode = q.mode;
  a.radix_bits = q.radix_bits;
  a.keep_nulls = q.keep_nulls_probe;
  a.build_rows_zero = q.build->rows == 0;
  a.build_bloom = q.probe_filtered ? b.bloom.as<uint8_t>() : nullptr;
  a.dir = b.directory;
  a.rank = b.rank;
  a.trace = attach_join_trace(n_tiles);
  a.pack_build_ids = b.directory.ids32 ? 1 : 0;
  a.hashed_type = q.hashed_type;
  a.n_secondary = q.n_secondary;
  for (uint32_t p = 0; p < q.n_secondary; ++p) a.secondary[p] = q.secondary[p];
  a.hist_elements = buffers.hist.as<uint32_t>();
  a.hist_pairs = buffers.hist.as<uint32_t>() + second_at;
  a.base_elements = buffers.base.as<uint64_t>();
  a.base_pairs = buffers.base.as<uint64_t>() + second_at;
  if (!q.count_only && n_tiles && !b.rank.entries) {
    HY_TRY(buffers.partner.alloc(4 * size_t{n_tiles} * JOIN_TILE));
    HY_TRY(buffers.meta.alloc(2 * size_t{n_tiles} * JOIN_TILE));
    HY_TRY(buffers.uncached.alloc(4 * size_t{n_tiles} * 2));
    a.uncached_tiles = buffers.uncached.as<uint32_t>() + n_tiles;
    a.row_partner = buffers.partner.as<uint32_t>();
    a.row_meta = buffers.meta.as<uint32_t>();
    a.tile_uncached = buffers.uncached.as<uint32_t>();
  }
  HY_TRY(buffers.words.alloc(256));
  uint32_t* words = buffers.words.as<uint32_t>();
  hipLaunchKernelGGL(zero_two, dim3(static_cast<uint32_t>(std::min<uint64_t>(64, (second_at - cells + 32 + 255) / 256))), dim3(256), 0, stream, buffers.hist.as<uint32_t>() + cells, size_t{second_at - cells},
                     words, size_t{32});
  a.error = &mailbox_dev->error;
  a.n_uncached = words + 1;
  a.xcd_tickets = words + 8;
  buffers.plan = reinterpret_cast<JoinPlan*>(words + 16);
  a.plan = buffers.plan;
  return HY_OK;
}

static hy_status output_groups(const JoinRequest& q, ProbeBuffers& buffers, uint32_t n_groups, const uint64_t** dev_first_cell, hipStream_t stream) {
  *dev_first_cell = nullptr;
  HY_TRY(buffers.origin.alloc(8 * (size_t{n_groups} + 1)));
  HY_TRY(buffers.slice_base.alloc(4 * (size_t{n_groups} + 1)));
  if (q.radix_bits) return HY_OK;
  std::vector<uint64_t>& first_cell = buffers.group_first_cell;
  first_cell.assign(size_t{n_groups} + 1, 0);
  uint64_t tile = 0;
  for (uint32_t c = 0; c < q.probe->n_chunks; ++c) {
    const uint32_t chunk_slices = (q.probe->host_segments[c].size + SLICE_ROWS - 1) / SLICE_ROWS;
    first_cell[c] = tile;
    tile += (chunk_slices ? chunk_slices : 1) * (SLICE_ROWS / JOIN_TILE);
  }
  first_cell[n_groups] = tile;
  HY_TRY(buffers.first_cell.alloc(8 * (size_t{n_groups} + 1)));
  HY_HIP(hipMemcpyAsync(buffers.first_cell.ptr, first_cell.data(), 8 * (size_t{n_groups} + 1), hipMemcpyHostToDevice, stream));
  *dev_first_cell = buffers.first_cell.as<uint64_t>();
  return HY_OK;
}

static hy_status launch_probe_count(const JoinRequest& q, bool rank_path, bool fetch_ahead, const ProbeArgs& a, ProbeBuffers& buffers, const JoinOutput& out, const uint64_t* dev_first_cell,
                                    uint32_t n_groups, JoinMailbox* mailbox_dev, hipStream_t stream) {
  const uint32_t n_tiles = a.n_tiles, partitions = 1u << q.radix_bits;
  const uint64_t cells = buffers.cells, second_at = buffers.second_at;
  if (!n_tiles) {
    HY_HIP(hipMemsetAsync(buffers.base.ptr, 0, 8 * (second_at + cells + 2), stream));
  } else {
    if (rank_path && fetch_ahead) {
      int per_cu = 0;
      HY_HIP(hipOccupancyMaxActiveBlocksPerMultiprocessor(&per_cu, reinterpret_cast<const void*>(rt_stream_count), 64 * STREAM_WAVES, 4 * stream_count_lds_words(partitions)));
      hipLaunchKernelGGL(rt_stream_count, dim3(stream_grid(n_tiles, per_cu)), dim3(64 * STREAM_WAVES), 4 * stream_count_lds_words(partitions), stream, a);
    } else if (rank_path) hipLaunchKernelGGL(rt_probe_count, dim3(probe_grid(n_tiles)), dim3(JOIN_THREADS), 0, stream, a);
    else if (q.general) hipLaunchKernelGGL(probe_count<true>, dim3(probe_grid(n_tiles)), dim3(JOIN_THREADS), 0, stream, a);
    else hipLaunchKernelGGL(probe_count<false>, dim3(probe_grid(n_tiles)), dim3(JOIN_THREADS), 0, stream, a);
    HY_TRY(exclusive_scan(buffers.hist.as<uint32_t>(), buffers.base.as<uint64_t>(), second_at + cells, stream, second_at));
  }
  hipLaunchKernelGGL(plan_output, dim3(1), dim3(256), 0, stream, a.base_elements, a.base_pairs, dev_first_cell, n_groups, n_tiles, cells, q.capacity, q.slice_capacity,
                     buffers.origin.as<uint64_t>(), buffers.slice_base.as<uint32_t>(), out.slice_offsets, n_tiles && a.row_meta ? a.n_uncached : nullptr, buffers.plan, mailbox_dev);
  return HY_OK;
}

static hy_status launch_probe_emit(const JoinRequest& q, bool rank_path, ProbeArgs& a, const uint64_t* dev_first_cell, uint32_t n_groups, uint32_t max_slices, const JoinMailbox* mailbox,
                                   hipStream_t stream) {
  const uint32_t n_tiles = a.n_tiles, partitions = 1u << q.radix_bits;
  if (!n_tiles) return HY_OK;
  HY_TRY(raise_probe_emit_lds());
  const uint32_t cut_grid = std::min<uint32_t>(max_slices, q.slice_capacity);
  if (rank_path) {
    a.lane_ordered_atomics = lds_atomics_are_lane_ordered(stream) ? 1u : 0u;
    hipEvent_t started = nullptr, stopped = nullptr;
    profile_events(&started, &stopped, HY_KERNEL_JOIN_PROBE);
    hipExtLaunchKernelGGL(rt_probe_emit, dim3(probe_grid(n_tiles)), dim3(JOIN_THREADS), 4 * rt_probe_emit_lds_words(partitions), stream, started, stopped, 0, a);
    if (cut_grid) hipLaunchKernelGGL(rt_probe_cuts, dim3(cut_grid), dim3(JOIN_THREADS), 0, stream, a, dev_first_cell, n_groups);
    return HY_OK;
  }
  int per_cu = 0;
  HY_HIP(hipOccupancyMaxActiveBlocksPerMultiprocessor(&per_cu, reinterpret_cast<const void*>(probe_emit_cached), JOIN_THREADS, 4 * probe_emit_cached_lds_words(partitions)));
  uint32_t workgroups_per_cu = per_cu > 0 ? static_cast<uint32_t>(per_cu) : 1;
  if (FIXED_JOIN_WGS_PER_CU > 0) workgroups_per_cu = static_cast<uint32_t>(FIXED_JOIN_WGS_PER_CU);
  const uint32_t resident = device_cu_count() * workgroups_per_cu / 8 * 8;
  const uint32_t cached_grid = std::max<uint32_t>(8, std::min<uint32_t>(resident, probe_grid(n_tiles)));
  profile_begin(stream, HY_KERNEL_JOIN_PROBE);
  hipLaunchKernelGGL(probe_emit_cached, dim3(cached_grid), dim3(JOIN_THREADS), 4 * probe_emit_cached_lds_words(partitions), stream, a);
  profile_end(stream);
  if (cut_grid) hipLaunchKernelGGL(probe_cuts, dim3(cut_grid), dim3(64), 0, stream, a, dev_first_cell, n_groups);
  if (!q.host_result || mailbox->n_uncached) {
    const dim3 generic_grid(std::min<uint32_t>(n_tiles, device_cu_count() * 2));
    if (q.general) hipLaunchKernelGGL(probe_emit_generic<true>, generic_grid, dim3(JOIN_THREADS), 4 * probe_emit_lds_words(partitions), stream, a);
    else hipLaunchKernelGGL(probe_emit_generic<false>, generic_grid, dim3(JOIN_THREADS), 4 * probe_emit_lds_words(partitions), stream, a);
  }
  return HY_OK;
}

static hy_status probe_general(const JoinRequest& q, const BuildSide& b, bool fetch_ahead, StageClock& clock, hipStream_t stream) {
  const bool rank_path = b.rank.entries != nullptr;
  JoinMailbox* mailbox = nullptr;
  JoinMailbox* mailbox_dev = nullptr;
  HY_TRY(join_mailbox(&mailbox, &mailbox_dev));
  ProbeBuffers buffers;
  ProbeArgs a{};
  HY_TRY(probe_arguments(q, b, mailbox_dev, buffers, a, stream));
  const uint32_t n_groups = q.radix_bits ? 1u << q.radix_bits : q.probe->n_chunks;
  const uint64_t* dev_first_cell = nullptr;
  HY_TRY(output_groups(q, buffers, n_groups, &dev_first_cell, stream));
  const uint32_t max_slices = static_cast<uint32_t>(q.probe->rows / PROBE_SIZE_PER_CHUNK) + n_groups + 1;
  JoinOutput out;
  HY_TRY(begin_output(q, max_slices, out));
  HY_TRY(launch_probe_count(q, rank_path, fetch_ahead, a, buffers, out, dev_first_cell, n_groups, mailbox_dev, stream));
  clock.mark("pass 1 launched");
  if (q.count_only) {
    HY_HIP(hipStreamSynchronize(stream));
    if (mailbox->error) return fail(HY_ERR_UNSUPPORTED, "a probe row matches more than 4 194 303 build rows");
    if (q.count_out) *q.count_out = mailbox->n_pairs;
    return HY_OK;
  }
  HY_TRY(size_output_lists(q, mailbox, stream, clock, out));
  a.partition_element_origin = buffers.origin.as<uint64_t>();
  a.partition_slice_base = buffers.slice_base.as<uint32_t>();
  a.build_out = out.build;
  a.probe_out = out.probe;
  a.slice_offsets = out.slice_offsets;
  HY_TRY(launch_probe_emit(q, rank_path, a, dev_first_cell, n_groups, max_slices, mailbox, stream));
  HY_HIP(hipGetLastError());
  clock.mark("pass 2 launched");
  HY_TRY(copy_output_back(q, mailbox, stream, out));
  HY_HIP(hipStreamSynchronize(stream));
  clock.mark("pass 2 done");
  return report_join_result(q.result, mailbox->n_pairs, mailbox->n_slices, mailbox->error);
}

static hy_status run_join_once(const hy_column* left, const hy_column* right, uint32_t mode, hy_join_result* result, bool count_only, uint64_t* count_out,
                               const hy_join_predicate* secondary, uint32_t n_secondary, bool* retry) {
  JoinRequest q;
  HY_TRY(resolve_join_request(left, right, mode, result, count_only, count_out, secondary, n_secondary, &q));
  hipStream_t stream = current_stream();
  BuildSide b;
  StageClock clock;
  bool probe_views = false;
  const bool probe_takes_pk = probe_takes_pk_kernels(q, stream, &probe_views);
  const BuildWants wants{q.keep_nulls_build, q.probe_filtered, q.pack_build_ids, q.n_secondary == 0, q.semi_anti && q.n_secondary == 0, probe_takes_pk, q.hashed_type};
  HY_TRY(prepare_build(q.build, wants, b, stream));
  const bool rank_path = b.rank.entries != nullptr;
  t_last_join_used_rank_table = rank_path ? (b.rank.identity_rows ? 2 : 1) : 0;
  t_last_join_used_pkfk = 0;
  t_last_join_hinted_attempt = b.hinted ? 1 : 0;
  clock.mark("build side launched");
  if (result) {
    result->radix_bits = q.radix_bits;
    result->left_is_build = q.build_right ? 0 : 1;
    result->n_slices = 0;
    result->n_pairs = 0;
  }
  if (mode == HY_JOIN_ANTI_NULL_AS_TRUE && b.any_null) {
    if (count_out) *count_out = 0;
    if (result && result->slice_offsets && q.host_result) result->slice_offsets[0] = 0;
    if (result && result->slice_offsets && !q.host_result) HY_HIP(hipMemsetAsync(result->slice_offsets, 0, 8, stream));
    return HY_OK;
  }
  const bool pk_path = rank_path && probe_takes_pk && static_cast<int64_t>(b.rank.key_min) >= INT32_MIN && static_cast<int64_t>(b.rank.key_min + b.rank.range) <= INT32_MAX;
  if (b.bloom_is_bits && !pk_path) return fail(HY_ERR_DEVICE, "join: a bit filter was built for kernels that do not run");
  if (pk_path) return probe_pkfk(q, b, clock, retry, stream);
  return probe_general(q, b, rank_path && probe_views, clock, stream);
}

__global__ __launch_bounds__(256) void join_any_null_byte(const uint8_t* bytes, uint64_t n, uint32_t* found) {
  bool any = false;
  for (uint64_t i = static_cast<uint64_t>(blockIdx.x) * 256 + threadIdx.x; i < n; i += static_cast<uint64_t>(gridDim.x) * 256) any = any || bytes[i] != 0;
  if (__any(any) && (threadIdx.x & 63) == 0) *found = 1;
}
struct MaterialisedInput {
  DeviceBuffer values, nulls, bases;
  hy_column* column = nullptr;
  MaterialisedInput() = default;
  MaterialisedInput(const MaterialisedInput&) = delete;
  MaterialisedInput& operator=(const MaterialisedInput&) = delete;
  ~MaterialisedInput() { if (column) (void)hy_column_destroy(column); }
};
constexpr uint64_t MATERIALISE_FROM_ROWS = 1u << 17;
static hy_status materialise_reference_input(const hy_column* input, MaterialisedInput& out) {
  if (!input->is_reference || input->data_type != HY_TYPE_INT || input->rows < MATERIALISE_FROM_ROWS || input->has_dictionary_without_values || input->is_mvcc ||
      (input->ref && (input->ref->is_mvcc || input->ref->has_dictionary_without_values))) return HY_OK;
  hipStream_t stream = current_stream();
  const uint32_t n_chunks = input->n_chunks;
  std::vector<uint64_t> bases(size_t{n_chunks} + 1, 0);
  for (uint32_t c = 0; c < n_chunks; ++c) bases[c + 1] = (bases[c] + input->host_segments[c].size + 3) & ~uint64_t{3};
  const uint64_t padded = bases[n_chunks];
  HY_TRY(out.bases.alloc(8 * (size_t{n_chunks} + 1)));
  HY_TRY(out.values.alloc(4 * padded + 64));
  HY_TRY(out.nulls.alloc(padded + 64));
  HY_HIP(hipMemcpyAsync(out.bases.ptr, bases.data(), 8 * (size_t{n_chunks} + 1), hipMemcpyHostToDevice, stream));
  HY_HIP(hipMemsetAsync(out.nulls.ptr, 0, padded + 64, stream));
  uint32_t* found = reinterpret_cast<uint32_t*>(out.nulls.as<uint8_t>() + ((padded + 3) & ~uint64_t{3}) + 16);
  HY_TRY(export_column_at(input, out.values.ptr, out.nulls.as<uint8_t>(), out.bases.as<uint64_t>()));
  hipLaunchKernelGGL(join_any_null_byte, dim3(static_cast<uint32_t>(std::min<uint64_t>((padded + 255) / 256, 2048))), dim3(256), 0, stream, out.nulls.as<uint8_t>(), padded, found);
  uint32_t any = 0;
  HY_HIP(hipMemcpyAsync(&any, found, 4, hipMemcpyDeviceToHost, stream));
  HY_HIP(hipStreamSynchronize(stream));
  if (any) return HY_OK;
  std::vector<hy_segment> segments(n_chunks ? n_chunks : 1);
  for (uint32_t c = 0; c < n_chunks; ++c) {
    hy_segment& s = segments[c];
    std::memset(&s, 0, sizeof(s));
    s.encoding = HY_ENC_UNENCODED;
    s.data_type = HY_TYPE_INT;
    s.size = input->host_segments[c].size;
    s.width = 4;
    s.data = out.values.as<int32_t>() + bases[c];
    s.ref_chunk_id = 0xFFFFFFFFu;
  }
  return hy_column_create(segments.data(), n_chunks, HY_MEM_DEVICE, &out.column);
}

static hy_status run_join(const hy_column* left, const hy_column* right, uint32_t mode, hy_join_result* result, bool count_only, uint64_t* count_out,
                          const hy_join_predicate* secondary = nullptr, uint32_t n_secondary = 0) {
  MaterialisedInput left_keys, right_keys;
  HY_TRY(materialise_reference_input(left, left_keys));
  HY_TRY(materialise_reference_input(right, right_keys));
  if (left_keys.column) left = left_keys.column;
  if (right_keys.column) right = right_keys.column;
  const uint32_t radix_bits = result ? result->radix_bits : 0;
  bool retry = false;
  t_join_returned_async = false;
  hy_status status = run_join_once(left, right, mode, result, count_only, count_out, secondary, n_secondary, &retry);
  t_last_join_hinted = t_last_join_hinted_attempt ? 1 : 0;
  if (status == HY_OK && retry) {
    if (result) result->radix_bits = radix_bits;
    retry = false;
    status = run_join_once(left, right, mode, result, count_only, count_out, secondary, n_secondary, &retry);
    t_last_join_hinted = 2;
  }
  if (result && !count_only && result->mem == HY_MEM_DEVICE && (result->flags & HY_JOIN_ASYNC) && result->status && !t_join_returned_async &&
      (status == HY_OK || status == HY_ERR_CAPACITY)) {
    hipLaunchKernelGGL(publish_join_status, dim3(1), dim3(1), 0, current_stream(), result->status, result->n_pairs, result->n_slices, status == HY_OK ? 1u : 0u);
  }
  return status;
}

}

using namespace hy;

extern "C" {

hy_status hy_join_hash(const hy_column* left, const hy_column* right, uint32_t mode, hy_join_result* result) {
  if (!left || !right || !result) return fail(HY_ERR_INVALID, "hy_join_hash: null argument");
  HY_TRY(on_this_device(left, "hy_join_hash"));
  HY_TRY(on_this_device(right, "hy_join_hash"));
  HY_TRY(plain_column(left, &left));
  HY_TRY(plain_column(right, &right));
  return run_join(left, right, mode, result, false, nullptr);
}

hy_status hy_join_hash_finish(const hy_column* left, const hy_column* right, uint32_t mode, hy_join_result* result) {
  if (!left || !right || !result) return fail(HY_ERR_INVALID, "hy_join_hash_finish: null argument");
  if (!(result->flags & HY_JOIN_ASYNC) || !result->status || result->mem != HY_MEM_DEVICE) return HY_OK;
  HY_TRY(on_this_device(left, "hy_join_hash_finish"));
  HY_TRY(on_this_device(right, "hy_join_hash_finish"));
  hipStream_t stream = current_stream();
  void* host = nullptr;
  void* device = nullptr;
  HY_TRY(pinned_staging(sizeof(hy_join_status), &host, &device));
  HY_HIP(hipMemcpyAsync(host, result->status, sizeof(hy_join_status), hipMemcpyDeviceToHost, stream));
  HY_HIP(hipStreamSynchronize(stream));
  const hy_join_status seen = *static_cast<const hy_join_status*>(host);
  if (seen.build_confirmed) return report_join_result(result, seen.n_pairs, seen.n_slices, seen.error);
  HY_TRY(plain_column(left, &left));
  HY_TRY(plain_column(right, &right));
  (builds_over_right_input(left, right, mode) ? right : left)->join_hint.state.store(2, std::memory_order_release);
  const uint32_t flags = result->flags;
  result->flags = flags & ~HY_JOIN_ASYNC;
  const hy_status status = run_join(left, right, mode, result, false, nullptr);
  result->flags = flags;
  t_last_join_hinted = 2;
  if (status == HY_OK || status == HY_ERR_CAPACITY) {
    hipLaunchKernelGGL(publish_join_status, dim3(1), dim3(1), 0, stream, result->status, result->n_pairs, result->n_slices, status == HY_OK ? 1u : 0u);
    HY_HIP(hipStreamSynchronize(stream));
  }
  return status;
}

hy_status hy_join_hash_predicates(const hy_column* left, const hy_column* right, uint32_t mode, const hy_join_predicate* secondary, uint32_t n_secondary,
                                  hy_join_result* result) {
  if (!left || !right || !result || (n_secondary && !secondary)) return fail(HY_ERR_INVALID, "hy_join_hash_predicates: null argument");
  HY_TRY(on_this_device(left, "hy_join_hash_predicates"));
  HY_TRY(on_this_device(right, "hy_join_hash_predicates"));
  for (uint32_t i = 0; i < n_secondary; ++i) {
    HY_TRY(on_this_device(secondary[i].left_column, "hy_join_hash_predicates"));
    HY_TRY(on_this_device(secondary[i].right_column, "hy_join_hash_predicates"));
  }
  HY_TRY(plain_column(left, &left));
  HY_TRY(plain_column(right, &right));
  std::vector<hy_join_predicate> plain_secondary(secondary, secondary + n_secondary);
  for (hy_join_predicate& predicate : plain_secondary) {
    HY_TRY(plain_column(predicate.left_column, &predicate.left_column));
    HY_TRY(plain_column(predicate.right_column, &predicate.right_column));
  }
  return run_join(left, right, mode, result, false, nullptr, plain_secondary.data(), n_secondary);
}

hy_status hy_join_hash_count(const hy_column* left, const hy_column* right, uint32_t mode, uint64_t* n_pairs) {
  if (!left || !right || !n_pairs) return fail(HY_ERR_INVALID, "hy_join_hash_count: null argument");
  HY_TRY(on_this_device(left, "hy_join_hash_count"));
  HY_TRY(on_this_device(right, "hy_join_hash_count"));
  HY_TRY(plain_column(left, &left));
  HY_TRY(plain_column(right, &right));
  return run_join(left, right, mode, nullptr, true, n_pairs);
}

hy_status hy_join_hash_radix_bits(uint64_t build_rows, uint64_t probe_rows, uint32_t* radix_bits) {
  (void)probe_rows;
  if (!radix_bits) return fail(HY_ERR_INVALID, "hy_join_hash_radix_bits: null argument");
  *radix_bits = calculate_radix_bits(build_rows);
  return HY_OK;
}

int hy_debug_join_lane_ordered_atomics() { return g_lds_atomic_order.load(); }

int hy_debug_lds_order_in_effect(void) { return g_lds_order_in_effect.load(); }

int hy_debug_join_used_rank_table(void) { return t_last_join_used_rank_table; }

int hy_debug_join_build_was_hinted(void) { return t_last_join_hinted; }

int hy_debug_join_used_pkfk(void) { return t_last_join_used_pkfk; }

int hy_debug_join_trace(uint64_t* out, uint32_t capacity_tiles) {
  if (!g_join_trace) return 0;
  const uint32_t n = g_join_trace_tiles < capacity_tiles ? g_join_trace_tiles : capacity_tiles;
  (void)hipDeviceSynchronize();
  (void)hipMemcpy(out, g_join_trace, size_t{n} * 48, hipMemcpyDeviceToHost);
  return static_cast<int>(n);
}

}
```

### hyrise_amd/csrc/join_pkfk.hpp

```cpp
#pragma once

#ifndef HY_PK_TILE
#define HY_PK_TILE 8192
#endif
#ifndef HY_PK_WAVES_PER_SIMD
#define HY_PK_WAVES_PER_SIMD 4
#endif
constexpr uint32_t PK_TILE = HY_PK_TILE;
constexpr uint32_t PK_TILES_PER_SLICE = SLICE_ROWS / PK_TILE;
constexpr uint32_t PK_ROUNDS = 16;
constexpr uint32_t PK_THREADS = PK_TILE / PK_ROUNDS;
constexpr uint32_t PK_WAVES = PK_THREADS / 64;
constexpr uint32_t PK_WAVE_ROWS = PK_TILE / PK_WAVES;
constexpr uint32_t PK_COUNT_WAVE_ROWS = 2048;
constexpr uint32_t PK_COUNT_THREADS = 64 * (PK_TILE / PK_COUNT_WAVE_ROWS);
constexpr uint32_t PK_COUNT_BATCHES = PK_COUNT_WAVE_ROWS / 512;
constexpr uint32_t PK_SCAN_THREADS = 512;
constexpr uint32_t PK_SCAN_CHUNK = 8192;
static_assert(SLICE_ROWS % PK_TILE == 0 && HY_FOR_BLOCK_SIZE % PK_WAVE_ROWS == 0 && HY_FOR_BLOCK_SIZE == PK_COUNT_WAVE_ROWS && PK_TILE % PK_COUNT_WAVE_ROWS == 0,
              "a wave's rows must lie in one FrameOfReference block");
static_assert(PK_TILE <= (1u << 13), "a staged pair keeps its row in 13 bits");

struct PkArgs {
  const SliceView* views;
  uint32_t n_tiles;
  uint32_t stride;
  uint32_t mode;
  uint32_t radix_bits;
  uint32_t keep_nulls;
  uint32_t n_groups;
  const uint8_t* build_bloom;
  RankTable rank;
  const uint32_t* ids32;
  const hy_row_id* row_ids;
  uint32_t* counts;
  uint32_t* rel_elements;
  uint32_t* rel_pairs;
  uint32_t* totals;
  uint64_t* origin_pairs;
  uint32_t* slice_base;
  const uint32_t* group_first_tile;
  uint32_t* ticket;
  JoinPlan* plan;
  JoinMailbox* mailbox;
  uint64_t capacity;
  uint32_t slice_capacity;
  hy_row_id* build_out;
  hy_row_id* probe_out;
  uint64_t* slice_offsets;
  uint32_t emit_group_shift;
  uint32_t* row_ranks;
  uint32_t cut_blocks;
  uint32_t bloom_is_bits;
  uint64_t* trace;
  uint8_t* row_masks;
  const BuildVerdict* verdict;
  const uint64_t* fill_records;
  uint32_t n_fill_records;
  uint64_t hint_min, hint_max;
  uint32_t hint_allows_duplicates;
  hy_join_status* status;
  FillCleaning cleaning;
};
constexpr uint32_t PK_LDS_KEYS = 1u << 20;
constexpr uint32_t PK_LDS_WORDS = PK_LDS_KEYS / 32;
constexpr uint32_t PK_LDS_SUBTILES = 4;
constexpr uint32_t PK_LDS_MAX_PARTITIONS = 128;
__host__ __device__ inline uint32_t pk_lds_presence_words(uint64_t range) { return (static_cast<uint32_t>(range >> 5) + 1 + 3) & ~3u; }
__host__ __device__ inline size_t pk_count_lds_bytes(uint64_t range, uint32_t partitions) { return 4 * (size_t{pk_lds_presence_words(range)} + size_t{PK_LDS_SUBTILES} * partitions * COUNT_COPIES); }

__device__ __forceinline__ SliceView pk_tile_view(const PkArgs& a, uint32_t tile) {
  SliceView view = uniform_view(a.views + tile / PK_TILES_PER_SLICE);
  if constexpr (PK_TILES_PER_SLICE > 1) {
    const uint32_t offset = (tile % PK_TILES_PER_SLICE) * PK_TILE;
    view.row_begin += offset;
    view.row_count = view.row_count > offset ? (view.row_count - offset < PK_TILE ? view.row_count - offset : PK_TILE) : 0;
  }
  return view;
}

__device__ __forceinline__ bool pk_bloom_test(const PkArgs& a, uint32_t key) {
  const uint32_t index = key & (BLOOM_BITS - 1);
  if (a.bloom_is_bits) return (reinterpret_cast<const uint32_t*>(a.build_bloom)[index >> 5] >> (index & 31)) & 1;
  return a.build_bloom[index] != 0;
}

__device__ __forceinline__ uint32_t pk_block_tile(uint32_t n_tiles) { return (blockIdx.x & 7) * ((n_tiles + 7) / 8) + (blockIdx.x >> 3); }

template <bool INNER>
__device__ __forceinline__ bool pk_emits(uint32_t mode, bool found, bool* null_partner) {
  if constexpr (INNER) { *null_partner = false; return found; }
  const bool outer = mode == HY_JOIN_LEFT || mode == HY_JOIN_RIGHT;
  *null_partner = outer && !found;
  return outer ? true : (mode == HY_JOIN_INNER || mode == HY_JOIN_SEMI) ? found : !found;
}

constexpr uint32_t PK_NO_RANK = 0xFFFFFFFFu;
template <uint32_t WIDTH, bool LDS = false, bool RANKS = false>
__device__ __forceinline__ void pk_count_wave(const PkArgs& a, const SliceView& view, uint32_t wave, uint32_t lane, uint32_t* cells, const uint32_t* presence = nullptr,
                                              uint8_t* masks = nullptr, uint32_t* tile_ranks = nullptr) {
  const char* base = static_cast<const char*>(view.data);
  const uint32_t row_count = view.row_count;
  const uint32_t wave_first = wave * PK_COUNT_WAVE_ROWS;
  if (wave_first >= row_count) return;
  u32x4_t words[PK_COUNT_BATCHES][2];
#pragma unroll
  for (uint32_t b = 0; b < PK_COUNT_BATCHES; ++b) {
    const uint32_t first = wave_first + b * 512 + lane * 8;
    load_batch_words<WIDTH>(base, view.row_begin + (first < row_count ? first : 0), words[b]);
  }
  typedef __attribute__((address_space(4))) const uint32_t constant_word;
  const uint32_t bias = view.kind == VIEW_INT32 ? 0u : ((constant_word*)view.aux)[__builtin_amdgcn_readfirstlane(static_cast<int>((view.row_begin + wave_first) / HY_FOR_BLOCK_SIZE))];
  const uint32_t origin = static_cast<uint32_t>(a.rank.key_min), range = static_cast<uint32_t>(a.rank.range);
  const uint32_t mask = a.radix_bits ? (1u << a.radix_bits) - 1 : 0u;
  const uint32_t copy = ((lane >> 4) & 3) | ((lane & 1) << 2);
  uint32_t counted = 0;
  if constexpr (!LDS && !RANKS) {
    if ((a.mode == HY_JOIN_INNER || a.mode == HY_JOIN_SEMI) && wave_first + PK_COUNT_WAVE_ROWS <= row_count) {
      const uint32_t delta = bias - origin, beyond = range + 32;
      const char* table = reinterpret_cast<const char*>(a.rank.entries);
      uint32_t counted_here = 0;
#pragma unroll
      for (uint32_t g = 0; g < PK_COUNT_BATCHES; g += 2) {
        uint32_t bits[2][8];
#pragma unroll
        for (uint32_t b = 0; b < 2; ++b) {
#pragma unroll
          for (uint32_t j = 0; j < 8; ++j) {
            const uint32_t distance = batch_word<WIDTH>(words[g + b], j) + delta;
            const uint32_t clamped = distance < beyond ? distance : beyond;
            bits[b][j] = *reinterpret_cast<const uint32_t*>(table + ((clamped >> 2) & ~7u));
          }
        }
#pragma unroll
        for (uint32_t b = 0; b < 2; ++b) {
          uint32_t found = 0;
#pragma unroll
          for (uint32_t j = 0; j < 8; ++j) {
            const uint32_t distance = batch_word<WIDTH>(words[g + b], j) + delta;
            found |= (distance <= range ? (bits[b][j] >> (distance & 31)) & 1u : 0u) << j;
          }
          if (__any(found != 0xFFu)) continue;
#pragma unroll
          for (uint32_t j = 0; j < 8; ++j) {
            const uint32_t partition = (batch_word<WIDTH>(words[g + b], j) + bias) & mask;
            atomicAdd(&cells[partition * COUNT_COPIES + copy], 0x10001u);
          }
          counted_here |= 1u << (g + b);
        }
      }
      counted = counted_here;
      if (counted == (1u << PK_COUNT_BATCHES) - 1) return;
    }
  }
#pragma unroll
  for (uint32_t g = 0; g < PK_COUNT_BATCHES; g += 2) {
    uint32_t bits[2][8];
    uint32_t bases[RANKS ? 2 : 1][RANKS ? 8 : 1];
#pragma unroll
    for (uint32_t b = 0; b < 2; ++b) {
#pragma unroll
      for (uint32_t j = 0; j < 8; ++j) {
        const uint32_t distance = batch_word<WIDTH>(words[g + b], j) + bias - origin;
        if constexpr (LDS) bits[b][j] = presence[distance <= range ? distance >> 5 : 0u];
        else if constexpr (RANKS) {
          const u32x2_t entry = *reinterpret_cast<const u32x2_t*>(reinterpret_cast<const char*>(a.rank.entries) + (distance <= range ? (distance >> 5) * 8u : 0u));
          bits[b][j] = entry.x;
          bases[b][j] = entry.y;
        } else bits[b][j] = *reinterpret_cast<const uint32_t*>(reinterpret_cast<const char*>(a.rank.entries) + (distance <= range ? (distance >> 5) * 8u : 0u));
      }
    }
    if constexpr (RANKS) {
#pragma unroll
      for (uint32_t b = 0; b < 2; ++b) {
// ... 279 lines not shown
    __hip_atomic_store(a.totals + partition, static_cast<uint32_t>(carry), __ATOMIC_RELAXED, __HIP_MEMORY_SCOPE_AGENT);
    __hip_atomic_store(a.totals + gridDim.x + partition, static_cast<uint32_t>(carry >> 32), __ATOMIC_RELAXED, __HIP_MEMORY_SCOPE_AGENT);
    asm volatile("s_waitcnt vmcnt(0)" ::: "memory");
    const uint32_t arrived = __hip_atomic_fetch_add(a.ticket, 1u, __ATOMIC_RELAXED, __HIP_MEMORY_SCOPE_AGENT);
    s_last = arrived + 1 == gridDim.x ? 1u : 0u;
  }
  __syncthreads();
  if (!s_last) return;
  pk_plan(a, s_tmp, tid);
}

template <uint32_t WIDTH>
struct PkWords { u32x4_t piece[WIDTH]; };
template <uint32_t WIDTH>
__device__ __forceinline__ void pk_load_words(const SliceView& view, uint32_t wave, uint32_t lane, PkWords<WIDTH>& words) {
  const uint32_t first = wave * PK_WAVE_ROWS + lane * PK_ROUNDS;
  const char* base = static_cast<const char*>(view.data) + static_cast<size_t>(view.row_begin + first) * WIDTH;
  constexpr uint32_t rows_per_piece = 16 / WIDTH;
#pragma unroll
  for (uint32_t p = 0; p < WIDTH; ++p) {
    words.piece[p] = u32x4_t{0, 0, 0, 0};
    typedef const __attribute__((address_space(1))) u32x4_t* global_words;
    if (first + p * rows_per_piece < view.row_count) words.piece[p] = *(global_words)(base + p * 16);
  }
}

template <uint32_t WIDTH>
__device__ __forceinline__ void pk_words_to_block(const PkWords<WIDTH>& words, uint32_t* block, uint32_t lane) {
  u32x4_t* mine = reinterpret_cast<u32x4_t*>(reinterpret_cast<char*>(block) + lane * PK_ROUNDS * WIDTH);
#pragma unroll
  for (uint32_t p = 0; p < WIDTH; ++p) mine[p] = words.piece[p];
  __builtin_amdgcn_fence(__ATOMIC_RELEASE, "wavefront");
  __builtin_amdgcn_wave_barrier();
  __builtin_amdgcn_fence(__ATOMIC_ACQUIRE, "wavefront");
}

template <uint32_t WIDTH>
__device__ __forceinline__ uint32_t pk_block_word(const uint32_t* block, uint32_t lane, uint32_t k) {
  if constexpr (WIDTH == 2) return reinterpret_cast<const uint16_t*>(block)[k * 64 + lane];
  else if constexpr (WIDTH == 1) return reinterpret_cast<const uint8_t*>(block)[k * 64 + lane];
  else return block[k * 64 + lane];
}

typedef __attribute__((address_space(3))) uint32_t pk_lds_word;
__device__ __forceinline__ uint32_t pk_lds_address(uint32_t* word) { return static_cast<uint32_t>(reinterpret_cast<uintptr_t>((pk_lds_word*)word)); }
__device__ __forceinline__ pk_lds_word* pk_lds_pointer(uint32_t address) { return reinterpret_cast<pk_lds_word*>(static_cast<uintptr_t>(address)); }
struct PkStageTarget { uint32_t counters, spare, null_partners; };

__device__ __forceinline__ bool pk_bit(uint32_t word, uint32_t position) { return __builtin_amdgcn_ubfe(word, position, 1u) != 0; }
__device__ __forceinline__ uint32_t pk_bits_below(uint32_t word, uint32_t position) { return __popc(__builtin_amdgcn_ubfe(word, 0u, position)); }

template <bool INNER, bool STAGE>
__device__ __forceinline__ uint32_t pk_row_meta(const PkArgs& a, uint32_t key, uint32_t mask, bool valid, bool found, uint32_t k, PkStageTarget& target) {
  bool null_partner;
  const bool emit = pk_emits<INNER>(a.mode, found, &null_partner);
  if constexpr (STAGE) {
    if constexpr (!INNER) target.null_partners |= null_partner ? 1u << k : 0u;
    return (INNER ? found : valid && emit) ? target.counters + 4 * (key & mask) : target.spare;
  } else {
    return valid ? (key & mask) | (null_partner ? 0x200u : 0u) | (emit ? 0x400u : 0u) : INVALID_PARTITION;
  }
}

template <uint32_t WIDTH, bool INNER, bool STAGE, bool MASKS = false, bool RANKS = false>
__device__ __forceinline__ void pk_lookup_rows(const PkArgs& a, const SliceView& view, const uint32_t* block, uint32_t wave, uint32_t lane, uint32_t (&meta)[PK_ROUNDS],
                                               uint32_t (&rank)[PK_ROUNDS], PkStageTarget& target, const uint8_t* tile_masks = nullptr, const uint32_t* tile_ranks = nullptr) {
  const uint32_t row_count = view.row_count;
  const uint32_t wave_first = wave * PK_WAVE_ROWS;
  typedef __attribute__((address_space(4))) const uint32_t constant_word;
  const uint32_t bias = WIDTH == 4 && view.kind == VIEW_INT32 ? 0u : ((constant_word*)view.aux)[__builtin_amdgcn_readfirstlane(static_cast<int>((view.row_begin + (wave_first < row_count ? wave_first : 0u)) / HY_FOR_BLOCK_SIZE))];
  const uint32_t origin = static_cast<uint32_t>(a.rank.key_min), range = static_cast<uint32_t>(a.rank.range);
  const uint32_t mask = a.radix_bits ? (1u << a.radix_bits) - 1 : 0u;
  const int32_t wave_rows = __builtin_amdgcn_readfirstlane(row_count > wave_first ? static_cast<int32_t>(row_count - wave_first) : 0);
  uint32_t raw[PK_ROUNDS];
#pragma unroll
  for (uint32_t k = 0; k < PK_ROUNDS; ++k) raw[k] = pk_block_word<WIDTH>(block, lane, k) + bias;
  if constexpr (RANKS) {
    static_assert(INNER && STAGE && !MASKS, "ranks are handed over by Inner joins on the global-table kernels, to pk_emit");
#pragma unroll
    for (uint32_t k = 0; k < PK_ROUNDS; ++k) {
      const bool in = static_cast<int32_t>(lane) < wave_rows - static_cast<int32_t>(k * 64);
      rank[k] = in ? tile_ranks[wave_first + k * 64 + lane] : PK_NO_RANK;
    }
#pragma unroll
    for (uint32_t k = 0; k < PK_ROUNDS; ++k) meta[k] = pk_row_meta<INNER, STAGE>(a, raw[k], mask, true, rank[k] != PK_NO_RANK, k, target);
  } else if constexpr (MASKS) {
    const uint32_t mask_word = reinterpret_cast<const uint32_t*>(tile_masks + (lane < 32 ? 0u : PK_TILE / 8))[wave * (PK_WAVE_ROWS / 32) + (lane & 31)];
    uint32_t valid = 0, found = 0;
#pragma unroll
    for (uint32_t k = 0; k < PK_ROUNDS; ++k) {
      const uint32_t found_word = lane < 32 ? __builtin_amdgcn_readlane(mask_word, 2 * k) : __builtin_amdgcn_readlane(mask_word, 2 * k + 1);
      const uint32_t valid_word = lane < 32 ? __builtin_amdgcn_readlane(mask_word, 32 + 2 * k) : __builtin_amdgcn_readlane(mask_word, 32 + 2 * k + 1);
      found |= ((found_word >> (lane & 31)) & 1u) << k;
      valid |= ((valid_word >> (lane & 31)) & 1u) << k;
    }
    u32x2_t entry[PK_ROUNDS];
#pragma unroll
    for (uint32_t k = 0; k < PK_ROUNDS; ++k) {
      const uint32_t distance = raw[k] - origin;
      entry[k] = *reinterpret_cast<const u32x2_t*>(reinterpret_cast<const char*>(a.rank.entries) + (((found >> k) & 1) ? (distance >> 5) * 8u : 0u));
    }
#pragma unroll
    for (uint32_t k = 0; k < PK_ROUNDS; ++k) {
      const uint32_t bit = raw[k] - origin;
      rank[k] = entry[k].y + pk_bits_below(entry[k].x, bit);
      meta[k] = pk_row_meta<INNER, STAGE>(a, raw[k], mask, (valid >> k) & 1, (found >> k) & 1, k, target);
    }
  } else {
    u32x2_t entry[PK_ROUNDS];
#pragma unroll
    for (uint32_t k = 0; k < PK_ROUNDS; ++k) {
      const uint32_t distance = raw[k] - origin;
      entry[k] = *reinterpret_cast<const u32x2_t*>(reinterpret_cast<const char*>(a.rank.entries) + (distance <= range ? (distance >> 5) * 8u : 0u));
    }
    if constexpr (INNER && STAGE) {
#pragma unroll
      for (uint32_t k = 0; k < PK_ROUNDS; ++k) {
        const uint32_t distance = raw[k] - origin, bit = distance;
        const bool in = static_cast<int32_t>(lane) < wave_rows - static_cast<int32_t>(k * 64);
        rank[k] = entry[k].y + pk_bits_below(entry[k].x, bit);
        meta[k] = pk_row_meta<INNER, STAGE>(a, raw[k], mask, in, in && distance <= range && pk_bit(entry[k].x, bit), k, target);
      }
    } else {
      uint32_t valid = 0, found = 0;
#pragma unroll
      for (uint32_t k = 0; k < PK_ROUNDS; ++k) {
        const uint32_t distance = raw[k] - origin, bit = distance;
        const bool in = static_cast<int32_t>(lane) < wave_rows - static_cast<int32_t>(k * 64);
        if (in) valid |= 1u << k;
        if (in && distance <= range && pk_bit(entry[k].x, bit)) found |= 1u << k;
        rank[k] = entry[k].y + pk_bits_below(entry[k].x, bit);
      }
      if (a.build_bloom && !a.keep_nulls && __any((valid & ~found) != 0)) {
#pragma unroll
        for (uint32_t k = 0; k < PK_ROUNDS; ++k) {
          if (((valid & ~found) >> k) & 1) { if (!pk_bloom_test(a, raw[k])) valid &= ~(1u << k); }
        }
      }
#pragma unroll
      for (uint32_t k = 0; k < PK_ROUNDS; ++k) meta[k] = pk_row_meta<INNER, STAGE>(a, raw[k], mask, (valid >> k) & 1, (found >> k) & 1, k, target);
    }
  }
}

template <uint32_t WIDTH, bool INNER, bool STAGE, bool MASKS, bool RANKS>
__device__ __forceinline__ void pk_tile_rows_of_width(const PkArgs& a, const SliceView& view, uint32_t* block, uint32_t wave, uint32_t lane, uint32_t (&meta)[PK_ROUNDS],
                                                      uint32_t (&rank)[PK_ROUNDS], PkStageTarget& target, const uint8_t* tile_masks, const uint32_t* tile_ranks) {
  PkWords<WIDTH> words;
  pk_load_words<WIDTH>(view, wave, lane, words);
  pk_words_to_block<WIDTH>(words, block, lane);
  pk_lookup_rows<WIDTH, INNER, STAGE, MASKS, RANKS>(a, view, block, wave, lane, meta, rank, target, tile_masks, tile_ranks);
}

template <bool INNER, bool STAGE, bool MASKS = false, bool RANKS = false>
__device__ __forceinline__ void pk_tile_rows(const PkArgs& a, const SliceView& view, uint32_t* block, uint32_t wave, uint32_t lane, uint32_t (&meta)[PK_ROUNDS], uint32_t (&rank)[PK_ROUNDS],
                                             PkStageTarget& target, const uint8_t* tile_masks = nullptr, const uint32_t* tile_ranks = nullptr) {
  if (view.kind == VIEW_FOR8) pk_tile_rows_of_width<1, INNER, STAGE, MASKS, RANKS>(a, view, block, wave, lane, meta, rank, target, tile_masks, tile_ranks);
  else if (view.kind == VIEW_FOR16) pk_tile_rows_of_width<2, INNER, STAGE, MASKS, RANKS>(a, view, block, wave, lane, meta, rank, target, tile_masks, tile_ranks);
  else pk_tile_rows_of_width<4, INNER, STAGE, MASKS, RANKS>(a, view, block, wave, lane, meta, rank, target, tile_masks, tile_ranks);
}

template <bool INNER, bool MASKS = false>
__device__ __forceinline__ void pk_evaluate(const PkArgs& a, const SliceView& view, uint32_t* block, uint32_t wave, uint32_t lane, uint32_t (&meta)[PK_ROUNDS], uint32_t (&rank)[PK_ROUNDS],
                                            const uint8_t* tile_masks = nullptr) {
  PkStageTarget none = {0, 0, 0};
  pk_tile_rows<INNER, false, MASKS>(a, view, block, wave, lane, meta, rank, none, tile_masks);
}

constexpr uint32_t PK_STAGE_ROW = 0x1FFF, PK_STAGE_NULL = 1u << 21;
constexpr uint32_t PK_LINES = PK_TILE / 16;
__host__ __device__ constexpr size_t pk_wave_pairs_words(uint32_t partitions) {
  return size_t{PK_WAVES} * partitions > 2 * size_t{PK_LINES} ? size_t{PK_WAVES} * partitions : 2 * size_t{PK_LINES};
}
__host__ __device__ constexpr size_t pk_emit_lds_words(uint32_t partitions) {
  return 2 * (size_t{PK_TILE} + partitions + 2) + pk_wave_pairs_words(partitions) + 3 * size_t{partitions} + 32;
}
static_assert(PK_LINES == PK_THREADS, "the copy-out's line table is filled thread = line");
static_assert(2 * PK_LINES <= PK_WAVES * 256, "the line table must not make 256 partitions' LDS larger");

__device__ __forceinline__ uint32_t pk_first_line(uint32_t base) { return (base >> 4) + ((base & 15) != 0 ? 1u : 0u); }
__device__ __forceinline__ uint32_t pk_interior_lines(uint32_t base, uint32_t pairs) {
  const uint32_t first = pk_first_line(base), end = (base + pairs) >> 4;
  return end > first ? end - first : 0u;
}

template <int BUILD>
__device__ __forceinline__ u32x2_t pk_rank_row(const PkArgs& a, uint32_t r) {
  if constexpr (BUILD == BUILD_IDENTITY_65535) {
    uint32_t c = r >> 16, offset = (r & 0xFFFFu) + c;
    if (offset >= 65535u) { ++c; offset -= 65535u; }
    if (offset >= 65535u) { ++c; offset -= 65535u; }
    return u32x2_t{c, offset};
  } else if constexpr (BUILD == BUILD_IDENTITY) {
    uint32_t c = static_cast<uint32_t>(static_cast<double>(r) * a.rank.identity_inverse);
    if (c * a.rank.identity_rows > r) --c;
    uint32_t offset = r - c * a.rank.identity_rows;
    if (offset >= a.rank.identity_rows) { ++c; offset -= a.rank.identity_rows; }
    return u32x2_t{c, offset};
  } else if constexpr (BUILD == BUILD_PACKED) {
    const uint32_t id = a.ids32[r];
    return u32x2_t{id >> 16, id & 0xFFFFu};
  } else {
    return reinterpret_cast<const u32x2_t*>(a.row_ids)[r];
  }
}

template <bool INNER, int BUILD>
__device__ __forceinline__ u32x2_t pk_build_row(const PkArgs& a, uint32_t tag, uint32_t r) {
  if constexpr (INNER) return pk_rank_row<BUILD>(a, r);
  u32x2_t row = {0xFFFFFFFFu, 0xFFFFFFFFu};
  if (!(tag & PK_STAGE_NULL)) row = pk_rank_row<BUILD>(a, r);
  return row;
}

template <bool INNER, int BUILD>
__device__ __forceinline__ void pk_copy_out(const PkArgs& a, const u32x2_t* s_stage, u32x2_t* s_line, const uint32_t* s_out_base, const uint32_t* s_run, uint32_t partitions,
                                            uint32_t lines, uint32_t chunk, uint32_t tile_row_begin, uint32_t tid, uint32_t lane, uint32_t wave) {
  u32x2_t* probe_out = reinterpret_cast<u32x2_t*>(a.probe_out);
  u32x2_t* build_out = reinterpret_cast<u32x2_t*>(a.build_out);
  if (tid < lines) {
    uint32_t p = 0;
    for (uint32_t step = partitions >> 1; step; step >>= 1) p += (s_run[partitions + p + step] >> 16) <= tid ? step : 0u;
    const uint32_t pair_index = 16 * (pk_first_line(s_run[p]) + tid - (s_run[partitions + p] >> 16));
    s_line[tid] = u32x2_t{pair_index - s_out_base[p], pair_index};
  }
  const uint32_t mine = 2 * wave + (lane & 1) + 16 * (lane >> 1);
  uint64_t owned = __ballot(mine < partitions && (s_run[partitions + (mine < partitions ? mine : 0u)] & 0xFFFFu) != 0);
  while (owned) {
    const uint32_t first_bit = __builtin_ctzll(owned);
    owned &= owned - 1;
    const uint32_t second_bit = owned ? static_cast<uint32_t>(__builtin_ctzll(owned)) : 64u;
    owned &= owned - 1;
    const uint32_t b = lane < 32 ? first_bit : second_bit;
    if (b == 64) continue;
    const uint32_t p = 2 * wave + (b & 1) + 16 * (b >> 1);
    const uint32_t base = s_run[p], pairs = s_run[partitions + p] & 0xFFFFu, i = lane & 31;
    const uint32_t first = pk_first_line(base), end = (base + pairs) >> 4;
    const bool interior = end > first;
    const uint32_t pair_index = interior && i >= 16 ? 16 * end + (i - 16) : base + i;
    const bool edge = interior ? (i < 16 ? pair_index < 16 * first : pair_index < base + pairs) : i < pairs;
    if (edge) {
      const u32x2_t record = s_stage[pair_index - s_out_base[p]];
      probe_out[pair_index] = u32x2_t{chunk, tile_row_begin + (record.x & PK_STAGE_ROW)};
      if constexpr (BUILD != BUILD_NONE) build_out[pair_index] = pk_build_row<INNER, BUILD>(a, record.x, record.y);
    }
  }
  __syncthreads();
  for (uint32_t piece = tid; piece < 8 * lines; piece += PK_THREADS) {
    const u32x2_t line = s_line[piece >> 3];
    const uint32_t offset = 2 * (piece & 7);
    const u32x4_t records = *reinterpret_cast<const u32x4_t*>(s_stage + line.x + offset);
    const size_t pair_pos = line.y + offset;
    __builtin_nontemporal_store(u32x4_t{chunk, tile_row_begin + (records.x & PK_STAGE_ROW), chunk, tile_row_begin + (records.z & PK_STAGE_ROW)},
                                reinterpret_cast<u32x4_t*>(probe_out + pair_pos));
    if constexpr (BUILD != BUILD_NONE) {
      const u32x2_t build0 = pk_build_row<INNER, BUILD>(a, records.x, records.y), build1 = pk_build_row<INNER, BUILD>(a, records.z, records.w);
      __builtin_nontemporal_store(u32x4_t{build0.x, build0.y, build1.x, build1.y}, reinterpret_cast<u32x4_t*>(build_out + pair_pos));
    }
  }
}

template <bool INNER, bool MASKS = false, bool RANKS = false>
__device__ __forceinline__ void pk_emit_tile(const PkArgs& a, uint32_t tile, const SliceView& view, uint32_t cell_pairs, uint32_t cell_base,
                                             uint32_t* join_smem, uint32_t tid, uint32_t lane, uint32_t wave) {
  const uint32_t partitions = 1u << a.radix_bits;
  const uint32_t stage_slots = PK_TILE + partitions + 2;
  u32x2_t* s_stage = reinterpret_cast<u32x2_t*>(join_smem);
  uint32_t* s_wave_pairs = reinterpret_cast<uint32_t*>(s_stage + stage_slots);
  uint32_t* s_out_base = s_wave_pairs + pk_wave_pairs_words(partitions);
  uint32_t* s_run = s_out_base + partitions;
  uint32_t* s_scratch = s_run + 2 * partitions;
  const uint32_t scan_waves = partitions > 64 ? partitions / 64 : 1;
  if (a.trace && tid == 0) a.trace[tile * 6 + 0] = wall_clock64();
  for (uint32_t i = tid; i < PK_WAVES * partitions; i += PK_THREADS) s_wave_pairs[i] = 0;
  if (tid < PK_WAVES) s_scratch[16 + tid] = 0;
  uint32_t counter[PK_ROUNDS], rank[PK_ROUNDS];
  PkStageTarget target = {pk_lds_address(s_wave_pairs + wave * partitions), pk_lds_address(s_scratch + 16 + wave), 0u};
  pk_tile_rows<INNER, true, MASKS, RANKS>(a, view, join_smem + wave * 1024, wave, lane, counter, rank, target, MASKS ? a.row_masks + static_cast<size_t>(tile) * (2 * PK_TILE / 8) : nullptr,
                                          RANKS ? a.row_ranks + static_cast<size_t>(tile) * PK_TILE : nullptr);
  __builtin_amdgcn_wave_barrier();
  if (a.trace && tid == 0) a.trace[tile * 6 + 1] = wall_clock64();
  const uint32_t reserve = (cell_pairs ? cell_pairs + 1 : 0) | pk_interior_lines(cell_base, cell_pairs) << 16;
  uint32_t first_in_wave = 0;
  if (wave < scan_waves) {
    const uint32_t inclusive = join_wave_inclusive_scan(reserve);
    first_in_wave = inclusive - reserve;
    if (lane == 63) s_scratch[wave] = inclusive;
  }
  __syncthreads();
  uint32_t before[PK_ROUNDS];
  if constexpr (MASKS) {
#pragma unroll
    for (uint32_t k = 0; k < PK_ROUNDS; ++k) {
      before[k] = 0;
      if (counter[k] != target.spare) before[k] = __hip_atomic_fetch_add(pk_lds_pointer(counter[k]), 1u, __ATOMIC_RELAXED, __HIP_MEMORY_SCOPE_AGENT);
    }
  } else {
#pragma unroll
    for (uint32_t k = 0; k < PK_ROUNDS; ++k) before[k] = __hip_atomic_fetch_add(pk_lds_pointer(counter[k]), 1u, __ATOMIC_RELAXED, __HIP_MEMORY_SCOPE_AGENT);
  }
  __syncthreads();
  if (a.trace && tid == 0) a.trace[tile * 6 + 2] = wall_clock64();
  if (tid < partitions) {
    const uint32_t scanned = first_in_wave + (wave > 0 ? s_scratch[0] : 0u) + (wave > 1 ? s_scratch[1] : 0u) + (wave > 2 ? s_scratch[2] : 0u);
    uint32_t first = scanned & 0xFFFFu;
    if (cell_pairs) first += (first ^ cell_base) & 1u;
    s_out_base[tid] = cell_base - first;
    s_run[tid] = cell_base;
    s_run[partitions + tid] = (scanned & 0xFFFF0000u) | cell_pairs;
    uint32_t run = first;
#pragma unroll
    for (uint32_t w = 0; w < PK_WAVES; ++w) {
      const uint32_t pairs = s_wave_pairs[w * partitions + tid];
      s_wave_pairs[w * partitions + tid] = run;
      run += pairs;
    }
    if (tid == 0) s_scratch[8] = s_scratch[0] + (scan_waves > 1 ? s_scratch[1] : 0u) + (scan_waves > 2 ? s_scratch[2] : 0u) + (scan_waves > 3 ? s_scratch[3] : 0u);
  }
  if (tid >= PK_THREADS - PK_WAVES) s_scratch[16 + (PK_THREADS - 1 - tid)] = stage_slots - 1;
  __syncthreads();
  if (a.trace && tid == 0) a.trace[tile * 6 + 3] = wall_clock64();
  const uint32_t first_row = wave * PK_WAVE_ROWS + lane;
  uint32_t first_slot[PK_ROUNDS];
#pragma unroll
  for (uint32_t k = 0; k < PK_ROUNDS; ++k) first_slot[k] = *pk_lds_pointer(counter[k]);
#pragma unroll
  for (uint32_t k = 0; k < PK_ROUNDS; ++k) {
    const uint32_t slot = first_slot[k] + before[k] < stage_slots - 1 ? first_slot[k] + before[k] : stage_slots - 1;
    uint32_t tag = first_row + k * 64;
    if constexpr (!INNER) tag |= ((target.null_partners >> k) & 1) ? PK_STAGE_NULL : 0u;
    s_stage[slot] = u32x2_t{tag, rank[k]};
  }
  __syncthreads();
  if (a.trace && tid == 0) a.trace[tile * 6 + 4] = wall_clock64();
  const uint32_t lines = s_scratch[8] >> 16;
  const uint32_t chunk = view.chunk, row_begin = view.row_begin;
#define HY_PK_COPY(BUILD) pk_copy_out<INNER, BUILD>(a, s_stage, reinterpret_cast<u32x2_t*>(s_wave_pairs), s_out_base, s_run, partitions, lines, chunk, row_begin, tid, lane, wave)
  if (!a.build_out) HY_PK_COPY(BUILD_NONE);
  else if (a.rank.identity_rows == 65535u) HY_PK_COPY(BUILD_IDENTITY_65535);
  else if (a.rank.identity_rows) HY_PK_COPY(BUILD_IDENTITY);
  else if (a.ids32) HY_PK_COPY(BUILD_PACKED);
  else HY_PK_COPY(BUILD_ROW_IDS);
#undef HY_PK_COPY
  if (a.trace && tid == 0) a.trace[tile * 6 + 5] = wall_clock64();
}

template <bool MASKS = false>
__device__ __forceinline__ void pk_cut_slice(const PkArgs& a, uint32_t slice, uint32_t* smem, uint32_t tid, uint32_t lane, uint32_t wave) {
  uint32_t* s_rows = smem;
  uint32_t* s_members = smem + PK_WAVES * 1024;
  uint32_t* s_emitters = s_members + PK_WAVES * PK_ROUNDS;
  if (!a.plan->fits || slice >= a.plan->n_slices) return;
  uint32_t lo = 0, hi = a.n_groups;
  while (hi - lo > 1) {
    const uint32_t step = (hi - lo + 63) / 64, at = lo + lane * step;
    const uint32_t below = __popcll(__ballot(at < hi && a.slice_base[at] <= slice));
    lo += (below - 1) * step;
    hi = lo + step < hi ? lo + step : hi;
  }
  const uint32_t group = lo;
  const uint32_t partition = a.radix_bits ? group : 0;
  const uint32_t* rel_elements = a.rel_elements + static_cast<size_t>(partition) * a.stride;
  const uint32_t first_tile = a.radix_bits ? 0 : a.group_first_tile[group] * PK_TILES_PER_SLICE, end_tile = a.radix_bits ? a.n_tiles : a.group_first_tile[group + 1] * PK_TILES_PER_SLICE;
  const uint32_t target = rel_elements[first_tile] + (slice - a.slice_base[group]) * PROBE_SIZE_PER_CHUNK;
  uint32_t tile = first_tile, tile_end = end_tile;
  while (tile_end - tile > 1) {
    const uint32_t step = (tile_end - tile + 63) / 64, at = tile + lane * step;
    const uint32_t below = __popcll(__ballot(at < tile_end && rel_elements[at] <= target));
    tile += (below - 1) * step;
    tile_end = tile + step < tile_end ? tile + step : tile_end;
  }
  const uint32_t cut_rank = target - rel_elements[tile];
  const SliceView view = pk_tile_view(a, tile);
  uint32_t meta[PK_ROUNDS], rank[PK_ROUNDS];
  pk_evaluate<false, MASKS>(a, view, s_rows + wave * 1024, wave, lane, meta, rank, MASKS ? a.row_masks + static_cast<size_t>(tile) * (2 * PK_TILE / 8) : nullptr);
  uint64_t members[PK_ROUNDS], emitters[PK_ROUNDS];
#pragma unroll
  for (uint32_t k = 0; k < PK_ROUNDS; ++k) {
    const bool member = (meta[k] & 0x1FF) == partition;
    members[k] = __ballot(member);
    emitters[k] = __ballot(member && (meta[k] & 0x400u));
    if (lane == 0) { s_members[wave * PK_ROUNDS + k] = __popcll(members[k]); s_emitters[wave * PK_ROUNDS + k] = __popcll(emitters[k]); }
  }
  __syncthreads();
  uint32_t members_before = 0, emitters_before = 0;
  for (uint32_t i = 0; i < wave * PK_ROUNDS; ++i) { members_before += s_members[i]; emitters_before += s_emitters[i]; }
  const uint64_t lower_lanes = (1ull << lane) - 1;
  const uint64_t cell_base = a.origin_pairs[partition] + a.rel_pairs[static_cast<size_t>(partition) * a.stride + tile];
#pragma unroll
  for (uint32_t k = 0; k < PK_ROUNDS; ++k) {
    const bool member = (members[k] >> lane) & 1;
    if (member && members_before + __popcll(members[k] & lower_lanes) == cut_rank) a.slice_offsets[slice] = cell_base + emitters_before + __popcll(emitters[k] & lower_lanes);
    members_before += __popcll(members[k]);
    emitters_before += __popcll(emitters[k]);
  }
}

__global__ __launch_bounds__(PK_THREADS) void pk_cuts(PkArgs a) {
  __shared__ __attribute__((aligned(16))) uint32_t s_cut[PK_WAVES * 1024 + 2 * PK_WAVES * PK_ROUNDS];
  const uint32_t tid = threadIdx.x;
  pk_cut_slice(a, blockIdx.x, s_cut, tid, tid & 63, __builtin_amdgcn_readfirstlane(tid >> 6));
}

template <bool INNER, bool MASKS = false, bool RANKS = false>
__global__ __launch_bounds__(PK_THREADS, HY_PK_WAVES_PER_SIMD) void pk_emit(PkArgs a) {
  extern __shared__ __attribute__((aligned(16))) uint32_t join_smem[];
  const uint32_t partitions = 1u << a.radix_bits;
  const uint32_t tid = threadIdx.x, lane = tid & 63, wave = __builtin_amdgcn_readfirstlane(tid >> 6);
  for (uint32_t i = blockIdx.x * PK_THREADS + tid; i < a.cleaning.vectors; i += gridDim.x * PK_THREADS) a.cleaning.filter[i] = u32x4_t{0, 0, 0, 0};
  if (blockIdx.x < a.cut_blocks) { pk_cut_slice<MASKS>(a, blockIdx.x, join_smem, tid, lane, wave); return; }
  const uint32_t block = blockIdx.x - a.cut_blocks;
  uint32_t tile;
  if (a.emit_group_shift < 32) {
    const uint32_t xcd = block & 7, j = block >> 3, shift = a.emit_group_shift;
    const uint32_t whole = ((a.n_tiles + 7) / 8) >> shift << shift;
    tile = j < whole ? ((j >> shift) << (shift + 3)) + (xcd << shift) + (j & ((1u << shift) - 1)) : whole * 8 + (j - whole) * 8 + xcd;
  } else tile = (block & 7) * ((a.n_tiles + 7) / 8) + (block >> 3);
  if (tile >= a.n_tiles) return;
  const SliceView view = pk_tile_view(a, tile);
  const uint32_t fits = a.plan->fits;
  if (!fits || view.row_count == 0) return;
  const size_t cell = static_cast<size_t>(tid < partitions ? tid : 0) * a.stride + tile;
  const uint32_t cell_pairs = tid < partitions ? a.counts[cell] >> 16 : 0;
  const uint32_t cell_base = static_cast<uint32_t>(a.origin_pairs[tid < partitions ? tid : 0]) + a.rel_pairs[cell];
  pk_emit_tile<INNER, MASKS, RANKS>(a, tile, view, cell_pairs, cell_base, join_smem, tid, lane, wave);
}
```

### hyrise_amd/csrc/runtime.hip

```cpp
#include "hy_device.hpp"
#include <algorithm>

#include <atomic>
#include <cstring>
#include <thread>

namespace hy {

static thread_local std::string t_error;
std::atomic<int64_t> g_options[HY_OPT_COUNT];
namespace {
struct OptionDefaults {
  OptionDefaults() {
    for (auto& v : g_options) v.store(0, std::memory_order_relaxed);
    auto set = [](uint32_t id, int64_t v) { g_options[id].store(v, std::memory_order_relaxed); };
    set(HY_OPT_JOIN_RANK_TABLE, 1);
    set(HY_OPT_JOIN_HINT, 1);
    set(HY_OPT_JOIN_PKFK, 1);
    set(HY_OPT_JOIN_LDS_BUILD, 1);
    set(HY_OPT_JOIN_LDS_BUILD_TILES, 2048);
    set(HY_OPT_JOIN_FILL_WGS_PER_CU, 4);
    set(HY_OPT_JOIN_HAND_OVER_RANKS, 1 << 20);
    set(HY_OPT_AGG_SPILL_SHIFT, 3);
    set(HY_OPT_AGG_SMALL_DOMAIN, 1);
    set(HY_OPT_FUSED_SMALL_DOMAIN, 1);
    set(HY_OPT_SCAN_TWO_COLUMNS, 1);
    set(HY_OPT_STAR_FUSED_PROBE, 1);
    set(HY_OPT_STAR_FUSED_FINISH, 1);
    set(HY_OPT_LDS_ORDERED_ATOMICS, 1);
  }
};
OptionDefaults g_option_defaults;
}

static thread_local hipStream_t t_stream = nullptr;
static thread_local Scratch t_scratch;

hy_status fail(hy_status code, const char* fmt, ...) {
  char buffer[1024];
  va_list args;
  va_start(args, fmt);
  vsnprintf(buffer, sizeof(buffer), fmt, args);
  va_end(args);
  t_error = buffer;
  return code;
}
void clear_error() { t_error.clear(); }

static std::atomic<int> g_device{-1};
static thread_local int t_bound_device = -1;
static thread_local int t_own_device = -1;
void bind_thread_device() {
  const int device = t_own_device >= 0 ? t_own_device : g_device.load(std::memory_order_acquire);
  if (device >= 0 && t_bound_device != device) {
    (void)hipSetDevice(device);
    t_bound_device = device;
  }
}

hy_status on_this_device(const hy_column* column, const char* entry_point) {
  if (!column) return HY_OK;
  bind_thread_device();
  const int here = t_bound_device >= 0 ? t_bound_device : 0;
  if (column->device != here) return fail(HY_ERR_INVALID, "%s: the column lives on device %d, the calling thread works on device %d (hy_bind_device)", entry_point, column->device, here);
  return on_this_device(column->ref, entry_point);
}

int this_thread_device() {
  bind_thread_device();
  return t_bound_device >= 0 ? t_bound_device : 0;
}

void bind_thread_to(int device) {
  t_own_device = device;
  bind_thread_device();
}

hipStream_t current_stream() {
  bind_thread_device();
  return t_stream;
}

struct Profile {
  bool enabled = false;
  uint32_t period = 1;
  uint32_t counter[HY_KERNEL_KINDS] = {};
  bool open = false;
  std::vector<hipEvent_t> events;
  std::vector<uint8_t> kinds;
  size_t used = 0;
};
static thread_local Profile t_profile;

static hipEvent_t next_event() {
  Profile& p = t_profile;
  if (p.used == p.events.size()) {
    hipEvent_t e = nullptr;
    (void)hipEventCreate(&e);
    p.events.push_back(e);
  }
  return p.events[p.used++];
}

static bool sampled(uint32_t kind) {
  Profile& p = t_profile;
  if (!p.enabled || p.used >= 16384) return false;
  if (kind >= HY_KERNEL_KINDS) kind = 0;
  if (p.counter[kind]++ % p.period != 0) return false;
  if (p.kinds.size() <= p.used / 2) p.kinds.resize(p.used / 2 + 1);
  p.kinds[p.used / 2] = static_cast<uint8_t>(kind);
  return true;
}

void profile_begin(hipStream_t stream, uint32_t kind) {
  t_profile.open = sampled(kind);
  if (t_profile.open) (void)hipEventRecord(next_event(), stream);
}

void profile_end(hipStream_t stream) {
  if (!t_profile.open) return;
  t_profile.open = false;
  (void)hipEventRecord(next_event(), stream);
}

bool profile_events(hipEvent_t* start, hipEvent_t* stop, uint32_t kind) {
  *start = *stop = nullptr;
  if (!sampled(kind)) return false;
  *start = next_event();
  *stop = next_event();
  return true;
}


struct BufferPool {
  std::vector<std::pair<size_t, void*>> free_blocks;
  ~BufferPool() { for (auto& b : free_blocks) (void)hipFree(b.second); }
};
static thread_local BufferPool t_pool;

hy_status pool_acquire(size_t bytes, void** ptr, size_t* capacity) {
  bind_thread_device();
  size_t rounded = 4096;
  while (rounded < bytes) rounded <<= 1;
  for (size_t i = 0; i < t_pool.free_blocks.size(); ++i) {
    if (t_pool.free_blocks[i].first == rounded) {
      *ptr = t_pool.free_blocks[i].second;
      *capacity = rounded;
      t_pool.free_blocks.erase(t_pool.free_blocks.begin() + i);
      return HY_OK;
    }
  }
  hipError_t err = hipMalloc(ptr, rounded);
  if (err != hipSuccess) {
    for (auto& b : t_pool.free_blocks) (void)hipFree(b.second);
    t_pool.free_blocks.clear();
    err = hipMalloc(ptr, rounded);
  }
  if (err != hipSuccess) { *ptr = nullptr; return fail(HY_ERR_DEVICE, "hipMalloc(%zu) failed: %s", rounded, hipGetErrorString(err)); }
  *capacity = rounded;
  return HY_OK;
}

void pool_release(void* ptr, size_t capacity) {
  if (ptr) t_pool.free_blocks.emplace_back(capacity, ptr);
}

hy_status DeviceBuffer::alloc(size_t bytes) {
  if (ptr) {
    if (!borrowed) pool_release(ptr, capacity);
    ptr = nullptr;
    capacity = 0;
  }
  borrowed = false;
  return pool_acquire(bytes, &ptr, &capacity);
}

void DeviceBuffer::borrow(void* block) {
  if (ptr && !borrowed) pool_release(ptr, capacity);
  ptr = block;
  capacity = 0;
  borrowed = true;
}
// ... 978 lines not shown
```

### include/hyrise_amd.h

```cpp
#ifndef HYRISE_AMD_H_
#define HYRISE_AMD_H_

#include <stddef.h>
#include <stdint.h>

#ifdef __cplusplus
extern "C" {
#endif

#define HY_ABI_VERSION 4

typedef int32_t hy_status;
enum {
  HY_OK = 0,
  HY_ERR_INVALID = 1,
  HY_ERR_UNSUPPORTED = 2,
  HY_ERR_DEVICE = 3,
  HY_ERR_CAPACITY = 4
};

enum { HY_TYPE_NULL = 0, HY_TYPE_INT = 1, HY_TYPE_LONG = 2, HY_TYPE_FLOAT = 3, HY_TYPE_DOUBLE = 4, HY_TYPE_STRING = 5 };

enum {
  HY_PRED_EQUALS = 0, HY_PRED_NOT_EQUALS = 1, HY_PRED_LESS_THAN = 2, HY_PRED_LESS_THAN_EQUALS = 3,
  HY_PRED_GREATER_THAN = 4, HY_PRED_GREATER_THAN_EQUALS = 5,
  HY_PRED_BETWEEN_INCLUSIVE = 6, HY_PRED_BETWEEN_LOWER_EXCLUSIVE = 7, HY_PRED_BETWEEN_UPPER_EXCLUSIVE = 8,
  HY_PRED_BETWEEN_EXCLUSIVE = 9,
  HY_PRED_IN = 10, HY_PRED_NOT_IN = 11, HY_PRED_LIKE = 12, HY_PRED_NOT_LIKE = 13, HY_PRED_LIKE_INSENSITIVE = 14,
  HY_PRED_NOT_LIKE_INSENSITIVE = 15, HY_PRED_IS_NULL = 16, HY_PRED_IS_NOT_NULL = 17
};

enum {
  HY_JOIN_INNER = 0, HY_JOIN_LEFT = 1, HY_JOIN_RIGHT = 2, HY_JOIN_FULL_OUTER = 3, HY_JOIN_CROSS = 4, HY_JOIN_SEMI = 5,
  HY_JOIN_ANTI_NULL_AS_TRUE = 6, HY_JOIN_ANTI_NULL_AS_FALSE = 7
};

enum {
  HY_AGG_MIN = 0, HY_AGG_MAX = 1, HY_AGG_SUM = 2, HY_AGG_AVG = 3, HY_AGG_COUNT = 4, HY_AGG_COUNT_DISTINCT = 5,
  HY_AGG_STDDEV_SAMP = 6, HY_AGG_ANY = 7
};

enum { HY_ENC_UNENCODED = 0, HY_ENC_DICTIONARY = 1, HY_ENC_FRAME_OF_REFERENCE = 2, HY_ENC_REFERENCE = 3,
       HY_ENC_MVCC = 4 ,
       HY_ENC_RUN_LENGTH = 5  };

enum { HY_ENC_LZ4 = 6 };
typedef struct hy_lz4_blocks {
  const void* const* blocks;
  const uint32_t* block_bytes;
  uint32_t block_count;
  uint32_t block_size;
  uint32_t last_block_size;
  uint32_t dictionary_bytes;
  const void* dictionary;
} hy_lz4_blocks;

enum { HY_SORT_NONE = 0, HY_SORT_ASCENDING_NULLS_FIRST = 1, HY_SORT_DESCENDING_NULLS_FIRST = 2, HY_SORT_ASCENDING_NULLS_LAST = 3,
       HY_SORT_DESCENDING_NULLS_LAST = 4 };

enum { HY_MEM_HOST = 0, HY_MEM_DEVICE = 1 };

#define HY_INVALID_VALUE_ID 0xFFFFFFFFu
#define HY_FOR_BLOCK_SIZE 2048u
#define HY_INVALID_COLUMN 0xFFFFu

typedef struct hy_row_id {
  uint32_t chunk_id;
  uint32_t chunk_offset;
} hy_row_id;

typedef struct hy_column hy_column;

typedef struct hy_segment {
  uint32_t encoding;
  uint32_t data_type;
  uint32_t size;
  uint32_t width;
  const void* data;
  const void* aux;
  uint32_t aux_size;
  uint32_t ref_chunk_id;
  const uint64_t* nulls;
  const hy_column* ref;
  uint32_t sorted_by;
  uint32_t bits;
} hy_segment;

typedef union hy_value {
  int32_t i32;
  int64_t i64;
  float f32;
  double f64;
  uint32_t value_id;
} hy_value;

typedef struct hy_predicate {
  uint32_t condition;
  uint32_t value_type;
  hy_value value;
  hy_value value2;
  const uint32_t* per_chunk_lower;
  const uint32_t* per_chunk_upper;
  const uint8_t* per_chunk_found;
  uint32_t column_is_nullable;
  uint32_t reserved;
  const uint64_t* match_words;
  const uint64_t* match_word_offsets;
} hy_predicate;

enum {
  HY_CHUNK_SCANNED = 0,
  HY_CHUNK_ALL_MATCH = 1,
  HY_CHUNK_NONE_MATCH = 2
};

typedef struct hy_scan_result {
  uint32_t mem;
  uint32_t flags;
  hy_row_id* matches;
  uint64_t capacity;
  uint64_t* offsets;
  uint32_t* counts;
  uint8_t* chunk_state;
  uint64_t total_matches;
} hy_scan_result;

#define HY_SCAN_MATERIALIZE_ALL_MATCH 1u
#define HY_SCAN_CHUNK_REGIONS 2u

int32_t hy_abi_version(void);
hy_status hy_init(int32_t device);
hy_status hy_shutdown(void);
const char* hy_last_error(void);
hy_status hy_set_stream(void* hip_stream);
hy_status hy_synchronize(void);
hy_status hy_device_malloc(void** ptr, size_t bytes);
hy_status hy_device_free(void* ptr);
hy_status hy_memcpy_h2d(void* dst, const void* src, size_t bytes);
hy_status hy_memcpy_d2h(void* dst, const void* src, size_t bytes);
hy_status hy_device_count(int32_t* count);
hy_status hy_set_profiling(int32_t enabled);
hy_status hy_profile_read(float* total_milliseconds, uint32_t* launches);
enum { HY_KERNEL_OTHER = 0, HY_KERNEL_SCAN = 1, HY_KERNEL_JOIN_PROBE = 2, HY_KERNEL_JOIN_COUNT = 3, HY_KERNEL_JOIN_BUILD = 4, HY_KERNEL_AGGREGATE = 5,
       HY_KERNEL_PROJECTION = 6, HY_KERNEL_LIKE = 7 ,
       HY_KERNEL_STRING_RANK = 8 , HY_KERNEL_KINDS = 9 };
hy_status hy_profile_read_kernel(uint32_t kernel, float* total_milliseconds, uint32_t* launches);
hy_status hy_profile_event_overhead(float* milliseconds);

#define HY_POOL_KEEP_MEDIAN 1u
hy_status hy_result_pool_acquire(uint64_t bytes, void** ptr);
hy_status hy_result_pool_acquire_pair(uint64_t rows, hy_row_id** left, hy_row_id** right);
hy_status hy_result_pool_release(void* ptr);
hy_status hy_result_pool_calibrate(const hy_column* left, const hy_column* right, uint32_t mode, uint64_t rows, uint32_t candidates, uint32_t flags,
                                   float* ms_per_candidate, uint32_t* chosen);
hy_status hy_result_pool_trim(void);
hy_status hy_result_pool_stats(uint64_t* held_bytes, uint64_t* in_use_bytes, uint32_t* calibrated_pairs);

enum {
  HY_OPT_ALLOW_ANY_ARCH = 0,
  HY_OPT_JOIN_RANK_TABLE = 1,
  HY_OPT_JOIN_HINT = 2,
  HY_OPT_JOIN_BREAK_HINT = 3,
  HY_OPT_JOIN_PKFK = 4,
  HY_OPT_JOIN_LDS_BUILD = 5,
  HY_OPT_JOIN_LDS_BUILD_TILES = 6,
  HY_OPT_JOIN_FILL_WGS_PER_CU = 7,
  HY_OPT_JOIN_HAND_OVER_RANKS = 8,
  HY_OPT_AGG_PARTITION_BITS = 9,
  HY_OPT_AGG_SPILL_SHIFT = 10,
  HY_OPT_AGG_SMALL_DOMAIN = 11,
  HY_OPT_FUSED_SMALL_DOMAIN = 12,
  HY_OPT_SCAN_TWO_COLUMNS = 13,
  HY_OPT_STAR_FUSED_PROBE = 14,
  HY_OPT_STAR_FUSED_FINISH = 15,
  HY_OPT_LDS_ORDERED_ATOMICS = 16,
  HY_OPT_PRODUCT_NONTEMPORAL = 17,
  HY_OPT_COUNT = 18
};
hy_status hy_set_option(uint32_t option, int64_t value);
hy_status hy_get_option(uint32_t option, int64_t* value);

typedef struct hy_comm hy_comm;
enum { HY_COMM_SUM = 0, HY_COMM_MIN = 1, HY_COMM_MAX = 2 };
enum { HY_COMM_ID_BYTES = 128 };
hy_status hy_bind_device(int32_t device);
hy_status hy_comm_unique_id(void* id_128_bytes);
hy_status hy_comm_init_rank(const void* id_128_bytes, uint32_t world, uint32_t rank, hy_comm** comm);
hy_status hy_comm_init_all(const int32_t* devices, uint32_t n_devices, hy_comm** comms );
hy_status hy_comm_destroy(hy_comm* comm);
hy_status hy_comm_rank(const hy_comm* comm, uint32_t* rank, uint32_t* world);
hy_status hy_comm_group_begin(void);
hy_status hy_comm_group_end(void);
hy_status hy_comm_all_reduce(hy_comm* comm, const void* send, void* recv, uint64_t count, uint32_t data_type , uint32_t op);
hy_status hy_comm_all_gather(hy_comm* comm, const void* send, void* recv , uint64_t bytes_per_rank);
hy_status hy_comm_all_to_all_v(hy_comm* comm, const void* send, const uint64_t* send_bytes, void* recv, const uint64_t* recv_bytes);

hy_status hy_column_create(const hy_segment* segments, uint32_t n_chunks, uint32_t mem, hy_column** out);
hy_status hy_column_destroy(hy_column* column);
hy_status hy_column_row_count(const hy_column* column, uint64_t* rows);
hy_status hy_column_chunk_count(const hy_column* column, uint32_t* chunks);

hy_status hy_table_scan(const hy_column* column, const hy_predicate* predicate, const uint32_t* excluded_chunks,
                        uint32_t n_excluded, hy_scan_result* result);
#define HY_MAX_IN_LIST 256
typedef struct hy_in_list {
  uint32_t value_type;
  uint32_t n_values;
  const hy_value* values;
  uint32_t negated;
  uint32_t column_is_nullable;
  const uint32_t* per_chunk_value_ids;
} hy_in_list;
hy_status hy_table_scan_in_list(const hy_column* column, const hy_in_list* list, const uint32_t* excluded_chunks, uint32_t n_excluded,
                                hy_scan_result* result);
hy_status hy_in_list_cast(uint32_t column_type, const uint32_t* literal_types, const hy_value* literals, uint32_t n, hy_value* out,
                          uint32_t* n_out, uint32_t* has_null);
hy_status hy_table_scan_columns(const hy_column* left, const hy_column* right, uint32_t condition,
                                hy_scan_result* result);

typedef struct hy_string_dictionary hy_string_dictionary;
typedef struct hy_string_dictionary_chunk {
  uint32_t n_entries;
  uint32_t string_length;
  const char* chars;
  const uint32_t* offsets;
} hy_string_dictionary_chunk;
hy_status hy_string_dictionary_create(const hy_string_dictionary_chunk* chunks, uint32_t n_chunks, uint32_t mem, hy_string_dictionary** out);
hy_status hy_string_dictionary_destroy(hy_string_dictionary* dict);
hy_status hy_string_dictionary_match_layout(const hy_string_dictionary* dict, uint64_t* word_offsets);
#define HY_MAX_LIKE_PATTERN 256
#define HY_LIKE_ANY_ONE 0x100u
#define HY_LIKE_ANY_RUN 0x200u
hy_status hy_like_tokenize(const char* pattern, uint32_t pattern_bytes, uint32_t condition, uint16_t* tokens, uint32_t* n_tokens);
hy_status hy_like_matches(const hy_string_dictionary* dict, const char* pattern, uint32_t pattern_bytes, uint32_t condition, uint32_t mem,
                          uint64_t* match_words);
hy_status hy_table_scan_like(const hy_column* column, const hy_string_dictionary* dict, const char* pattern, uint32_t pattern_bytes,
                             uint32_t condition, uint32_t column_is_nullable, const uint32_t* excluded_chunks, uint32_t n_excluded,
                             hy_scan_result* result);

hy_status hy_string_dictionary_ranks(const hy_string_dictionary* left, const hy_string_dictionary* right, uint32_t mem, int32_t* ranks);
hy_status hy_table_scan_columns_strings(const hy_column* left, const hy_string_dictionary* left_dict, const hy_column* right,
                                        const hy_string_dictionary* right_dict, uint32_t condition, hy_scan_result* result);

hy_status hy_string_dictionary_order(const hy_string_dictionary* dict, uint32_t mem, int32_t* ranks, uint32_t* n_distinct);
hy_status hy_column_string_ranks(const hy_column* column, const hy_string_dictionary* dict, hy_column** out);

hy_status hy_string_column_gather(const hy_column* column, const hy_string_dictionary* dict, const hy_row_id* positions, uint64_t n, uint32_t chunk_rows,
                                  hy_column** result, hy_string_dictionary** result_dict);
hy_status hy_string_ranks_gather(const hy_string_dictionary* dict, const hy_column* ranks, hy_column** result, hy_string_dictionary** result_dict);
hy_status hy_string_dictionary_chunk_size(const hy_string_dictionary* dict, uint32_t chunk, uint32_t* n_entries, uint64_t* chars_bytes);
hy_status hy_string_dictionary_read_chunk(const hy_string_dictionary* dict, uint32_t chunk, char* chars, uint32_t* offsets);

hy_status hy_validate(const hy_column* mvcc, uint32_t our_tid, uint32_t snapshot_commit_id, uint32_t can_use_chunk_shortcut,
                      hy_scan_result* result);

hy_status hy_predicate_cast(uint32_t condition, uint32_t column_type, uint32_t literal_type, const hy_value* literal, uint32_t literal2_type,
                            const hy_value* literal2, hy_predicate* out);

enum { HY_POSLIST_DENSE = 0, HY_POSLIST_CHUNK_REGIONS = 1 };
hy_status hy_poslist_translate(const hy_column* scanned, const hy_scan_result* result, uint32_t layout, hy_row_id* out, uint64_t capacity, uint64_t* n_out);

hy_status hy_poslist_gather(const hy_column* reference, const hy_row_id* positions, uint64_t n, hy_row_id* out);

typedef struct hy_sort_key {
  const hy_column* column;
  uint32_t mode;
  uint32_t reserved;
} hy_sort_key;
hy_status hy_sort(const hy_sort_key* keys, uint32_t n_keys, hy_row_id* out, uint64_t capacity, uint64_t* n_out);

enum { HY_SORT_LIMIT_FORCE_FULL_SORT = 1, HY_SORT_LIMIT_FORCE_SELECT = 2 };
hy_status hy_sort_limit(const hy_sort_key* keys, uint32_t n_keys, uint64_t limit, uint32_t flags, hy_row_id* out, uint64_t capacity, uint64_t* n_out, uint32_t* path);

hy_status hy_column_gather(const hy_column* column, const hy_row_id* positions, uint64_t n, uint32_t chunk_rows, hy_column** result);

enum { HY_UNION_FORCE_SORT = 1 };
hy_status hy_union_positions(const hy_column* const* left, const hy_column* const* right, uint32_t n_clusters, uint32_t flags, hy_row_id* const* out, uint64_t capacity,
                             uint64_t* n_out, uint32_t* path);

enum { HY_ARITH_ADD = 0, HY_ARITH_SUB = 1, HY_ARITH_MUL = 2, HY_ARITH_DIV = 3, HY_ARITH_MOD = 4 };
typedef struct hy_operand {
  const hy_column* column;
  uint32_t literal_type;
  hy_value literal;
} hy_operand;
hy_status hy_projection_arithmetic(uint32_t op, const hy_operand* left, const hy_operand* right, hy_column** result);
hy_status hy_column_read_chunk(const hy_column* column, uint32_t chunk, void* values, uint64_t* null_words);
uint32_t hy_column_data_type(const hy_column* column);
uint32_t hy_column_chunk_rows(const hy_column* column, uint32_t chunk);

#define HY_MAX_PROJECTION_NODES 32
#define HY_MAX_PROJECTION_DEPTH 6
#define HY_MAX_PROJECTION_COLUMNS 8
#define HY_MAX_PROJECTION_TESTS 4
enum { HY_PROJ_COLUMN = 0, HY_PROJ_LITERAL = 1, HY_PROJ_ARITHMETIC = 2, HY_PROJ_COMPARISON = 3, HY_PROJ_COLUMN_TEST = 4, HY_PROJ_IS_NULL = 5,
       HY_PROJ_IS_NOT_NULL = 6, HY_PROJ_AND = 7, HY_PROJ_OR = 8, HY_PROJ_UNARY_MINUS = 9, HY_PROJ_CASE = 10,
       HY_PROJ_BETWEEN = 11, HY_PROJ_CAST = 12, HY_PROJ_EXTRACT = 13, HY_PROJ_FUNCTION = 14, HY_PROJ_SUBQUERY = 15, HY_PROJ_PARAMETER = 16 };
typedef struct hy_projection_node {
  uint32_t kind;
  uint32_t op;
  uint32_t index;
  uint32_t literal_type;
  hy_value literal;
} hy_projection_node;
typedef struct hy_projection_test {
  const hy_column* column;
  hy_predicate predicate;
  const hy_in_list* in_list;
} hy_projection_test;
typedef struct hy_projection_program {
  uint32_t n_nodes, n_columns, n_tests, reserved;
  const hy_column* columns[HY_MAX_PROJECTION_COLUMNS];
  hy_projection_test tests[HY_MAX_PROJECTION_TESTS];
  hy_projection_node nodes[HY_MAX_PROJECTION_NODES];
} hy_projection_program;
hy_status hy_projection_expression(const hy_projection_program* program, hy_column** result);

hy_status hy_table_scan_expression(const hy_projection_program* program, const uint32_t* excluded_chunks, uint32_t n_excluded,
                                   hy_scan_result* result);

typedef struct hy_join_result {
  uint32_t mem;
  uint32_t radix_bits;
  hy_row_id* left_pos;
  hy_row_id* right_pos;
  uint64_t capacity;
  uint64_t* slice_offsets;
  uint32_t slice_capacity;
  uint32_t n_slices;
  uint64_t n_pairs;
// ... 186 lines not shown
```

Baseline: 371.8 billion.

## Stage PK-FK join pairs as packed 32-bit records to shrink LDS

```diff
diff --git a/__graft_entry__.py b/__graft_entry__.py
--- a/__graft_entry__.py
+++ b/__graft_entry__.py
@@ -42,7 +42,7 @@
 
 def build(force=False):
     sources = [os.path.join(CSRC, s) for s in HIP_SOURCES]
-    deps = sources + [os.path.join(CSRC, h) for h in ("hy_device.hpp", "hy_options.hpp", "hy_decode.hpp", "hy_arithmetic.hpp", "hy_scan_job.hpp", "hy_expression.hpp", "hy_expression_rows.hpp", "join_pkfk.hpp", "join_star.hpp", "aggregate_small.hpp", "fused_small.hpp", "sort_words.hpp", "sort_keys.hpp", "join_outer_emit.hpp", "string_entries.hpp")] + [os.path.join(ROOT, "include", "hyrise_amd.h")]
+    deps = sources + [os.path.join(CSRC, h) for h in ("hy_device.hpp", "hy_options.hpp", "hy_decode.hpp", "hy_arithmetic.hpp", "hy_scan_job.hpp", "hy_expression.hpp", "hy_expression_rows.hpp", "join_pkfk.hpp", "join_pk_stage.hpp", "join_star.hpp", "aggregate_small.hpp", "fused_small.hpp", "sort_words.hpp", "sort_keys.hpp", "join_outer_emit.hpp", "string_entries.hpp")] + [os.path.join(ROOT, "include", "hyrise_amd.h")]
     if force or _newer(LIB, deps):
         _build_library(sources, deps, force)
     host_tests = os.path.join(ROOT, "tests", "cpp", "host_tests")
diff --git a/hyrise_amd/abi.py b/hyrise_amd/abi.py
--- a/hyrise_amd/abi.py
+++ b/hyrise_amd/abi.py
@@ -111,7 +111,7 @@
 NLJ_MAX_TEMPORARY_BYTES = 1 << 31
 (OPT_ALLOW_ANY_ARCH, OPT_JOIN_RANK_TABLE, OPT_JOIN_HINT, OPT_JOIN_BREAK_HINT, OPT_JOIN_PKFK, OPT_JOIN_LDS_BUILD, OPT_JOIN_LDS_BUILD_TILES, OPT_JOIN_FILL_WGS_PER_CU,
  OPT_JOIN_HAND_OVER_RANKS, OPT_AGG_PARTITION_BITS, OPT_AGG_SPILL_SHIFT, OPT_AGG_SMALL_DOMAIN, OPT_FUSED_SMALL_DOMAIN, OPT_SCAN_TWO_COLUMNS, OPT_STAR_FUSED_PROBE, OPT_STAR_FUSED_FINISH,
- OPT_LDS_ORDERED_ATOMICS, OPT_PRODUCT_NONTEMPORAL) = range(18)
+ OPT_LDS_ORDERED_ATOMICS, OPT_PRODUCT_NONTEMPORAL, OPT_JOIN_COMPACT_STAGE) = range(19)
 KERNEL_OTHER, KERNEL_SCAN, KERNEL_JOIN_PROBE, KERNEL_JOIN_COUNT, KERNEL_JOIN_BUILD, KERNEL_AGGREGATE, KERNEL_PROJECTION, KERNEL_LIKE, KERNEL_STRING_RANK = range(9)
 ARITH_ADD, ARITH_SUB, ARITH_MUL, ARITH_DIV, ARITH_MOD = range(5)
 
@@ -368,7 +368,8 @@
     "HY_JOIN_NO_PKFK": (OPT_JOIN_PKFK, 0), "HY_JOIN_NO_LDS_BUILD": (OPT_JOIN_LDS_BUILD, 0), "HY_JOIN_LDS_BUILD_TILES": (OPT_JOIN_LDS_BUILD_TILES, None),
     "HY_JOIN_FILL_WGS_PER_CU": (OPT_JOIN_FILL_WGS_PER_CU, None), "HY_JOIN_HAND_OVER_RANKS": (OPT_JOIN_HAND_OVER_RANKS, None),
     "HY_AGG_PARTITION_BITS": (OPT_AGG_PARTITION_BITS, None), "HY_AGG_SPILL_SHIFT": (OPT_AGG_SPILL_SHIFT, None), "HY_AGG_NO_SMALL_DOMAIN": (OPT_AGG_SMALL_DOMAIN, 0),
-    "HY_FUSED_NO_SMALL_DOMAIN": (OPT_FUSED_SMALL_DOMAIN, 0), "HY_LDS_NO_ORDERED_ATOMICS": (OPT_LDS_ORDERED_ATOMICS, 0)
+    "HY_FUSED_NO_SMALL_DOMAIN": (OPT_FUSED_SMALL_DOMAIN, 0), "HY_LDS_NO_ORDERED_ATOMICS": (OPT_LDS_ORDERED_ATOMICS, 0),
+    "HY_OPT_JOIN_COMPACT_STAGE": (OPT_JOIN_COMPACT_STAGE, None)
 }
 
 
diff --git a/hyrise_amd/csrc/join.hip b/hyrise_amd/csrc/join.hip
--- a/hyrise_amd/csrc/join.hip
+++ b/hyrise_amd/csrc/join.hip
@@ -3527,6 +3527,7 @@
 #include "join_star.hpp"
 
 static thread_local int t_last_join_used_rank_table = 0;
+static thread_local int t_last_join_compact_stage = 0;
 static thread_local int t_last_join_used_pkfk = 0;
 static thread_local int t_last_join_hinted_attempt = 0;
 static thread_local int t_last_join_hinted = 0;
@@ -3830,6 +3831,8 @@
     HY_HIP(hipFuncSetAttribute(reinterpret_cast<const void*>(pk_emit<true, true>), hipFuncAttributeMaxDynamicSharedMemorySize, 4 * pk_emit_lds_words(MAX_PARTITIONS)));
     HY_HIP(hipFuncSetAttribute(reinterpret_cast<const void*>(pk_emit<false, true>), hipFuncAttributeMaxDynamicSharedMemorySize, 4 * pk_emit_lds_words(MAX_PARTITIONS)));
     HY_HIP(hipFuncSetAttribute(reinterpret_cast<const void*>(pk_emit<true, false, true>), hipFuncAttributeMaxDynamicSharedMemorySize, 4 * pk_emit_lds_words(MAX_PARTITIONS)));
+    HY_HIP(hipFuncSetAttribute(reinterpret_cast<const void*>(pk_emit<true, false, false, true>), hipFuncAttributeMaxDynamicSharedMemorySize, 4 * pk_emit_lds_words(MAX_PARTITIONS, true)));
+    HY_HIP(hipFuncSetAttribute(reinterpret_cast<const void*>(pk_emit<false, false, false, true>), hipFuncAttributeMaxDynamicSharedMemorySize, 4 * pk_emit_lds_words(MAX_PARTITIONS, true)));
     raised.done(device_bit);
   }
   return HY_OK;
@@ -3909,6 +3912,16 @@
   return HY_OK;
 }
 
+static bool probe_stages_compact(const JoinRequest& q, bool build_in_lds, bool hand_over_ranks) {
+  if (build_in_lds || hand_over_ranks || !option(HY_OPT_JOIN_COMPACT_STAGE) || q.radix_bits > PK_COMPACT_MAX_RADIX_BITS) return false;
+  const hy_column* probe = q.probe;
+  for (uint32_t c = 0; c < probe->n_chunks; ++c) {
+    const hy_segment& seg = probe->host_segments[c];
+    if (seg.encoding != HY_ENC_FRAME_OF_REFERENCE || (seg.width != 1 && seg.width != 2)) return false;
+  }
+  return probe->n_chunks > 0;
+}
+
 static hy_status launch_pk_emit(const JoinRequest& q, BuildSide& b, PkArgs& k, bool build_in_lds, bool hand_over_ranks, uint32_t max_slices, hipStream_t stream) {
   HY_TRY(raise_pk_emit_lds());
   hipEvent_t started = nullptr, stopped = nullptr;
@@ -3920,15 +3933,19 @@
   k.cut_blocks = (cut_grid + 7) / 8 * 8;
   k.cleaning = b.cleaning;
   const dim3 grid(k.cut_blocks + 8 * ((k.n_tiles + 7) / 8));
-  const size_t lds_bytes = 4 * pk_emit_lds_words(1u << q.radix_bits);
+  const bool compact = probe_stages_compact(q, build_in_lds, hand_over_ranks);
+  const size_t lds_bytes = 4 * pk_emit_lds_words(1u << q.radix_bits, compact);
   const bool inner = q.mode == HY_JOIN_INNER;
-  if (build_in_lds && inner) hipExtLaunchKernelGGL((pk_emit<true, true>), grid, dim3(PK_THREADS), lds_bytes, stream, started, stopped, 0, k);
+  if (compact && inner) hipExtLaunchKernelGGL((pk_emit<true, false, false, true>), grid, dim3(PK_THREADS), lds_bytes, stream, started, stopped, 0, k);
+  else if (compact) hipExtLaunchKernelGGL((pk_emit<false, false, false, true>), grid, dim3(PK_THREADS), lds_bytes, stream, started, stopped, 0, k);
+  else if (build_in_lds && inner) hipExtLaunchKernelGGL((pk_emit<true, true>), grid, dim3(PK_THREADS), lds_bytes, stream, started, stopped, 0, k);
   else if (build_in_lds) hipExtLaunchKernelGGL((pk_emit<false, true>), grid, dim3(PK_THREADS), lds_bytes, stream, started, stopped, 0, k);
   else if (hand_over_ranks) hipExtLaunchKernelGGL((pk_emit<true, false, true>), grid, dim3(PK_THREADS), lds_bytes, stream, started, stopped, 0, k);
   else if (inner) hipExtLaunchKernelGGL(pk_emit<true>, grid, dim3(PK_THREADS), lds_bytes, stream, started, stopped, 0, k);
   else hipExtLaunchKernelGGL(pk_emit<false>, grid, dim3(PK_THREADS), lds_bytes, stream, started, stopped, 0, k);
   HY_HIP(hipGetLastError());
   block_cleaning_queued(b);
+  t_last_join_compact_stage = compact ? 1 : 0;
   t_last_join_used_pkfk = build_in_lds ? 2 : 1;
   return HY_OK;
 }
@@ -4163,6 +4180,7 @@
   const bool rank_path = b.rank.entries != nullptr;
   t_last_join_used_rank_table = rank_path ? (b.rank.identity_rows ? 2 : 1) : 0;
   t_last_join_used_pkfk = 0;
+  t_last_join_compact_stage = 0;
   t_last_join_hinted_attempt = b.hinted ? 1 : 0;
   clock.mark("build side launched");
   if (result) {
@@ -4344,6 +4362,8 @@
 
 int hy_debug_join_used_pkfk(void) { return t_last_join_used_pkfk; }
 
+int hy_debug_join_compact_stage(void) { return t_last_join_compact_stage; }
+
 int hy_debug_join_trace(uint64_t* out, uint32_t capacity_tiles) {
   if (!g_join_trace) return 0;
   const uint32_t n = g_join_trace_tiles < capacity_tiles ? g_join_trace_tiles : capacity_tiles;
diff --git a/hyrise_amd/csrc/join_pk_stage.hpp b/hyrise_amd/csrc/join_pk_stage.hpp
--- /dev/null
+++ b/hyrise_amd/csrc/join_pk_stage.hpp
@@ -0,0 +1,56 @@
+#pragma once
+
+#ifndef HY_PK_TILE
+#define HY_PK_TILE 8192
+#endif
+#ifndef HY_PK_WAVES_PER_SIMD
+#define HY_PK_WAVES_PER_SIMD 4
+#endif
+#ifndef HY_PK_COMPACT_WAVES_PER_SIMD
+#define HY_PK_COMPACT_WAVES_PER_SIMD 6
+#endif
+#if defined(__HIPCC__)
+#define HY_PK_HOST_DEVICE __host__ __device__
+#else
+#define HY_PK_HOST_DEVICE
+#endif
+
+constexpr uint32_t PK_TILE = HY_PK_TILE;
+constexpr uint32_t PK_ROUNDS = 16;
+constexpr uint32_t PK_THREADS = PK_TILE / PK_ROUNDS;
+constexpr uint32_t PK_WAVES = PK_THREADS / 64;
+constexpr uint32_t PK_WAVE_ROWS = PK_TILE / PK_WAVES;
+constexpr uint32_t PK_LINES = PK_TILE / 16;
+constexpr uint32_t PK_CUT_WORDS = PK_WAVES * 1024 + 2 * PK_WAVES * PK_ROUNDS;
+constexpr uint32_t PK_COMPACT_MAX_RADIX_BITS = 8;
+constexpr size_t PK_LDS_PER_CU = 160 * 1024;
+static_assert(PK_TILE <= (1u << 13), "a staged pair keeps its row in 13 bits");
+
+constexpr uint32_t PK_COMPACT_ROW = PK_TILE - 1, PK_COMPACT_NULL_BIT = 13, PK_COMPACT_DELTA_SHIFT = 16;
+static_assert(PK_COMPACT_ROW < (1u << PK_COMPACT_NULL_BIT) && PK_WAVE_ROWS == 1024, "row, null partner and delta share one word; wave = row >> 10");
+struct PkCompactPair { uint32_t row, null_partner, wave, rank; };
+HY_PK_HOST_DEVICE constexpr uint32_t pk_compact_pack(uint32_t row, uint32_t null_partner, uint32_t delta) {
+  return row | null_partner << PK_COMPACT_NULL_BIT | delta << PK_COMPACT_DELTA_SHIFT;
+}
+HY_PK_HOST_DEVICE constexpr uint32_t pk_compact_row(uint32_t record) { return record & PK_COMPACT_ROW; }
+HY_PK_HOST_DEVICE constexpr uint32_t pk_compact_wave(uint32_t record) { return pk_compact_row(record) / PK_WAVE_ROWS; }
+HY_PK_HOST_DEVICE constexpr bool pk_compact_null(uint32_t record) { return (record >> PK_COMPACT_NULL_BIT) & 1u; }
+HY_PK_HOST_DEVICE constexpr uint32_t pk_compact_rank(uint32_t record, uint32_t wave_base) { return wave_base + (record >> PK_COMPACT_DELTA_SHIFT); }
+HY_PK_HOST_DEVICE constexpr PkCompactPair pk_compact_unpack(uint32_t record, uint32_t wave_base) {
+  return PkCompactPair{pk_compact_row(record), pk_compact_null(record) ? 1u : 0u, pk_compact_wave(record), pk_compact_rank(record, wave_base)};
+}
+
+HY_PK_HOST_DEVICE constexpr size_t pk_stage_words(uint32_t partitions, bool compact) {
+  return compact ? (size_t{PK_TILE} + partitions + 2 + 3) / 4 * 4 : 2 * (size_t{PK_TILE} + partitions + 2);
+}
+HY_PK_HOST_DEVICE constexpr size_t pk_wave_pairs_words(uint32_t partitions) {
+  return size_t{PK_WAVES} * partitions > 2 * size_t{PK_LINES} ? size_t{PK_WAVES} * partitions : 2 * size_t{PK_LINES};
+}
+HY_PK_HOST_DEVICE constexpr size_t pk_emit_lds_words(uint32_t partitions, bool compact = false) {
+  return pk_stage_words(partitions, compact) + pk_wave_pairs_words(partitions) + 3 * size_t{partitions} + 32;
+}
+static_assert(PK_LINES == PK_THREADS, "the copy-out's line table is filled thread = line");
+static_assert(2 * PK_LINES <= PK_WAVES * 256, "the line table must not make 256 partitions' LDS larger");
+static_assert(PK_WAVES * 1024 <= PK_TILE, "the rows' stored words go round through the staging area: 1024 words per wave, compact records included");
+static_assert(pk_emit_lds_words(1, true) >= PK_CUT_WORDS && pk_emit_lds_words(1, false) >= PK_CUT_WORDS, "pk_cut_slice runs in pk_emit's LDS");
+static_assert(3 * 4 * pk_emit_lds_words(1u << PK_COMPACT_MAX_RADIX_BITS, true) <= PK_LDS_PER_CU, "three compact workgroups per CU at the widest radix");
diff --git a/hyrise_amd/csrc/join_pkfk.hpp b/hyrise_amd/csrc/join_pkfk.hpp
--- a/hyrise_amd/csrc/join_pkfk.hpp
+++ b/hyrise_amd/csrc/join_pkfk.hpp
@@ -1,17 +1,8 @@
 #pragma once
 
-#ifndef HY_PK_TILE
-#define HY_PK_TILE 8192
-#endif
-#ifndef HY_PK_WAVES_PER_SIMD
-#define HY_PK_WAVES_PER_SIMD 4
-#endif
-constexpr uint32_t PK_TILE = HY_PK_TILE;
+#include "join_pk_stage.hpp"
+
 constexpr uint32_t PK_TILES_PER_SLICE = SLICE_ROWS / PK_TILE;
-constexpr uint32_t PK_ROUNDS = 16;
-constexpr uint32_t PK_THREADS = PK_TILE / PK_ROUNDS;
-constexpr uint32_t PK_WAVES = PK_THREADS / 64;
-constexpr uint32_t PK_WAVE_ROWS = PK_TILE / PK_WAVES;
 constexpr uint32_t PK_COUNT_WAVE_ROWS = 2048;
 constexpr uint32_t PK_COUNT_THREADS = 64 * (PK_TILE / PK_COUNT_WAVE_ROWS);
 constexpr uint32_t PK_COUNT_BATCHES = PK_COUNT_WAVE_ROWS / 512;
@@ -19,7 +10,6 @@
 constexpr uint32_t PK_SCAN_CHUNK = 8192;
 static_assert(SLICE_ROWS % PK_TILE == 0 && HY_FOR_BLOCK_SIZE % PK_WAVE_ROWS == 0 && HY_FOR_BLOCK_SIZE == PK_COUNT_WAVE_ROWS && PK_TILE % PK_COUNT_WAVE_ROWS == 0,
               "a wave's rows must lie in one FrameOfReference block");
-static_assert(PK_TILE <= (1u << 13), "a staged pair keeps its row in 13 bits");
 
 struct PkArgs {
   const SliceView* views;
@@ -605,11 +595,11 @@
   pk_lookup_rows<WIDTH, INNER, STAGE, MASKS, RANKS>(a, view, block, wave, lane, meta, rank, target, tile_masks, tile_ranks);
 }
 
-template <bool INNER, bool STAGE, bool MASKS = false, bool RANKS = false>
+template <bool INNER, bool STAGE, bool MASKS = false, bool RANKS = false, bool NARROW = false>
 __device__ __forceinline__ void pk_tile_rows(const PkArgs& a, const SliceView& view, uint32_t* block, uint32_t wave, uint32_t lane, uint32_t (&meta)[PK_ROUNDS], uint32_t (&rank)[PK_ROUNDS],
                                              PkStageTarget& target, const uint8_t* tile_masks = nullptr, const uint32_t* tile_ranks = nullptr) {
   if (view.kind == VIEW_FOR8) pk_tile_rows_of_width<1, INNER, STAGE, MASKS, RANKS>(a, view, block, wave, lane, meta, rank, target, tile_masks, tile_ranks);
-  else if (view.kind == VIEW_FOR16) pk_tile_rows_of_width<2, INNER, STAGE, MASKS, RANKS>(a, view, block, wave, lane, meta, rank, target, tile_masks, tile_ranks);
+  else if (NARROW || view.kind == VIEW_FOR16) pk_tile_rows_of_width<2, INNER, STAGE, MASKS, RANKS>(a, view, block, wave, lane, meta, rank, target, tile_masks, tile_ranks);
   else pk_tile_rows_of_width<4, INNER, STAGE, MASKS, RANKS>(a, view, block, wave, lane, meta, rank, target, tile_masks, tile_ranks);
 }
 
@@ -621,15 +611,7 @@
 }
 
 constexpr uint32_t PK_STAGE_ROW = 0x1FFF, PK_STAGE_NULL = 1u << 21;
-constexpr uint32_t PK_LINES = PK_TILE / 16;
-__host__ __device__ constexpr size_t pk_wave_pairs_words(uint32_t partitions) {
-  return size_t{PK_WAVES} * partitions > 2 * size_t{PK_LINES} ? size_t{PK_WAVES} * partitions : 2 * size_t{PK_LINES};
-}
-__host__ __device__ constexpr size_t pk_emit_lds_words(uint32_t partitions) {
-  return 2 * (size_t{PK_TILE} + partitions + 2) + pk_wave_pairs_words(partitions) + 3 * size_t{partitions} + 32;
-}
-static_assert(PK_LINES == PK_THREADS, "the copy-out's line table is filled thread = line");
-static_assert(2 * PK_LINES <= PK_WAVES * 256, "the line table must not make 256 partitions' LDS larger");
+static_assert(MAX_PARTITIONS == 1u << PK_COMPACT_MAX_RADIX_BITS, "join_pk_stage.hpp sizes the compact flavour's LDS for the widest radix");
 
 __device__ __forceinline__ uint32_t pk_first_line(uint32_t base) { return (base >> 4) + ((base & 15) != 0 ? 1u : 0u); }
 __device__ __forceinline__ uint32_t pk_interior_lines(uint32_t base, uint32_t pairs) {
@@ -659,15 +641,21 @@
 }
 
 template <bool INNER, int BUILD>
-__device__ __forceinline__ u32x2_t pk_build_row(const PkArgs& a, uint32_t tag, uint32_t r) {
+__device__ __forceinline__ u32x2_t pk_build_row(const PkArgs& a, bool null_partner, uint32_t r) {
   if constexpr (INNER) return pk_rank_row<BUILD>(a, r);
   u32x2_t row = {0xFFFFFFFFu, 0xFFFFFFFFu};
-  if (!(tag & PK_STAGE_NULL)) row = pk_rank_row<BUILD>(a, r);
+  if (!null_partner) row = pk_rank_row<BUILD>(a, r);
   return row;
 }
 
-template <bool INNER, int BUILD>
-__device__ __forceinline__ void pk_copy_out(const PkArgs& a, const u32x2_t* s_stage, u32x2_t* s_line, const uint32_t* s_out_base, const uint32_t* s_run, uint32_t partitions,
+struct PkStagedPair { uint32_t row; bool null_partner; uint32_t rank; };
+template <bool COMPACT>
+__device__ __forceinline__ PkStagedPair pk_staged_pair(uint32_t first, uint32_t second, const uint32_t* s_wave_base) {
+  if constexpr (COMPACT) return PkStagedPair{pk_compact_row(first), pk_compact_null(first), pk_compact_rank(first, s_wave_base[pk_compact_wave(first)])};
+  else return PkStagedPair{first & PK_STAGE_ROW, (first & PK_STAGE_NULL) != 0, second};
+}
+template <bool INNER, int BUILD, bool COMPACT>
+__device__ __forceinline__ void pk_copy_out(const PkArgs& a, const std::conditional_t<COMPACT, uint32_t, u32x2_t>* s_stage, const uint32_t* s_wave_base, u32x2_t* s_line, const uint32_t* s_out_base, const uint32_t* s_run, uint32_t partitions,
                                             uint32_t lines, uint32_t chunk, uint32_t tile_row_begin, uint32_t tid, uint32_t lane, uint32_t wave) {
   u32x2_t* probe_out = reinterpret_cast<u32x2_t*>(a.probe_out);
   u32x2_t* build_out = reinterpret_cast<u32x2_t*>(a.build_out);
@@ -693,33 +681,67 @@
     const uint32_t pair_index = interior && i >= 16 ? 16 * end + (i - 16) : base + i;
     const bool edge = interior ? (i < 16 ? pair_index < 16 * first : pair_index < base + pairs) : i < pairs;
     if (edge) {
-      const u32x2_t record = s_stage[pair_index - s_out_base[p]];
-      probe_out[pair_index] = u32x2_t{chunk, tile_row_begin + (record.x & PK_STAGE_ROW)};
-      if constexpr (BUILD != BUILD_NONE) build_out[pair_index] = pk_build_row<INNER, BUILD>(a, record.x, record.y);
+      PkStagedPair pair;
+      if constexpr (COMPACT) pair = pk_staged_pair<true>(s_stage[pair_index - s_out_base[p]], 0u, s_wave_base);
+      else { const u32x2_t record = s_stage[pair_index - s_out_base[p]]; pair = pk_staged_pair<false>(record.x, record.y, nullptr); }
+      probe_out[pair_index] = u32x2_t{chunk, tile_row_begin + pair.row};
+      if constexpr (BUILD != BUILD_NONE) build_out[pair_index] = pk_build_row<INNER, BUILD>(a, pair.null_partner, pair.rank);
     }
   }
   __syncthreads();
   for (uint32_t piece = tid; piece < 8 * lines; piece += PK_THREADS) {
     const u32x2_t line = s_line[piece >> 3];
     const uint32_t offset = 2 * (piece & 7);
-    const u32x4_t records = *reinterpret_cast<const u32x4_t*>(s_stage + line.x + offset);
+    PkStagedPair pair0, pair1;
+    if constexpr (COMPACT) {
+      const u32x2_t records = *reinterpret_cast<const u32x2_t*>(s_stage + line.x + offset);
+      pair0 = pk_staged_pair<true>(records.x, 0u, s_wave_base);
+      pair1 = pk_staged_pair<true>(records.y, 0u, s_wave_base);
+    } else {
+      const u32x4_t records = *reinterpret_cast<const u32x4_t*>(s_stage + line.x + offset);
+      pair0 = pk_staged_pair<false>(records.x, records.y, nullptr);
+      pair1 = pk_staged_pair<false>(records.z, records.w, nullptr);
+    }
     const size_t pair_pos = line.y + offset;
-    __builtin_nontemporal_store(u32x4_t{chunk, tile_row_begin + (records.x & PK_STAGE_ROW), chunk, tile_row_begin + (records.z & PK_STAGE_ROW)},
-                                reinterpret_cast<u32x4_t*>(probe_out + pair_pos));
+    __builtin_nontemporal_store(u32x4_t{chunk, tile_row_begin + pair0.row, chunk, tile_row_begin + pair1.row}, reinterpret_cast<u32x4_t*>(probe_out + pair_pos));
     if constexpr (BUILD != BUILD_NONE) {
-      const u32x2_t build0 = pk_build_row<INNER, BUILD>(a, records.x, records.y), build1 = pk_build_row<INNER, BUILD>(a, records.z, records.w);
+      const u32x2_t build0 = pk_build_row<INNER, BUILD>(a, pair0.null_partner, pair0.rank), build1 = pk_build_row<INNER, BUILD>(a, pair1.null_partner, pair1.rank);
       __builtin_nontemporal_store(u32x4_t{build0.x, build0.y, build1.x, build1.y}, reinterpret_cast<u32x4_t*>(build_out + pair_pos));
     }
   }
 }
 
-template <bool INNER, bool MASKS = false, bool RANKS = false>
+__device__ __forceinline__ uint32_t pk_wave_min(uint32_t v) {
+#define HY_PK_MIN_STEP(CTRL) v = min(v, static_cast<uint32_t>(__builtin_amdgcn_update_dpp(static_cast<int>(v), static_cast<int>(v), CTRL, 0xF, 0xF, false)))
+  HY_PK_MIN_STEP(0xB1);
+  HY_PK_MIN_STEP(0x4E);
+  HY_PK_MIN_STEP(0x141);
+  HY_PK_MIN_STEP(0x140);
+#undef HY_PK_MIN_STEP
+  const uint32_t row01 = min(static_cast<uint32_t>(__builtin_amdgcn_readlane(static_cast<int>(v), 0)), static_cast<uint32_t>(__builtin_amdgcn_readlane(static_cast<int>(v), 16)));
+  const uint32_t row23 = min(static_cast<uint32_t>(__builtin_amdgcn_readlane(static_cast<int>(v), 32)), static_cast<uint32_t>(__builtin_amdgcn_readlane(static_cast<int>(v), 48)));
+  return min(row01, row23);
+}
+template <bool INNER>
+__device__ __forceinline__ uint32_t pk_wave_rank_base(const uint32_t (&counter)[PK_ROUNDS], const uint32_t (&rank)[PK_ROUNDS], const PkStageTarget& target) {
+  uint32_t lowest = 0xFFFFFFFFu;
+#pragma unroll
+  for (uint32_t k = 0; k < PK_ROUNDS; ++k) {
+    const bool partner = counter[k] != target.spare && (INNER || !((target.null_partners >> k) & 1));
+    lowest = min(lowest, partner ? rank[k] : 0xFFFFFFFFu);
+  }
+  return pk_wave_min(lowest);
+}
+
+template <bool INNER, bool MASKS = false, bool RANKS = false, bool COMPACT = false>
 __device__ __forceinline__ void pk_emit_tile(const PkArgs& a, uint32_t tile, const SliceView& view, uint32_t cell_pairs, uint32_t cell_base,
                                              uint32_t* join_smem, uint32_t tid, uint32_t lane, uint32_t wave) {
   const uint32_t partitions = 1u << a.radix_bits;
   const uint32_t stage_slots = PK_TILE + partitions + 2;
-  u32x2_t* s_stage = reinterpret_cast<u32x2_t*>(join_smem);
-  uint32_t* s_wave_pairs = reinterpret_cast<uint32_t*>(s_stage + stage_slots);
+  static_assert(!COMPACT || (!MASKS && !RANKS), "compact records: the rank table in memory (a table staged in LDS reaches 2^20 ranks under one base)");
+  typedef std::conditional_t<COMPACT, uint32_t, u32x2_t> staged_record;
+  staged_record* s_stage = reinterpret_cast<staged_record*>(join_smem);
+  uint32_t* s_wave_pairs = join_smem + pk_stage_words(partitions, COMPACT);
   uint32_t* s_out_base = s_wave_pairs + pk_wave_pairs_words(partitions);
   uint32_t* s_run = s_out_base + partitions;
   uint32_t* s_scratch = s_run + 2 * partitions;
@@ -729,8 +751,10 @@
   if (tid < PK_WAVES) s_scratch[16 + tid] = 0;
   uint32_t counter[PK_ROUNDS], rank[PK_ROUNDS];
   PkStageTarget target = {pk_lds_address(s_wave_pairs + wave * partitions), pk_lds_address(s_scratch + 16 + wave), 0u};
-  pk_tile_rows<INNER, true, MASKS, RANKS>(a, view, join_smem + wave * 1024, wave, lane, counter, rank, target, MASKS ? a.row_masks + static_cast<size_t>(tile) * (2 * PK_TILE / 8) : nullptr,
+  pk_tile_rows<INNER, true, MASKS, RANKS, COMPACT>(a, view, join_smem + wave * 1024, wave, lane, counter, rank, target, MASKS ? a.row_masks + static_cast<size_t>(tile) * (2 * PK_TILE / 8) : nullptr,
                                           RANKS ? a.row_ranks + static_cast<size_t>(tile) * PK_TILE : nullptr);
+  uint32_t rank_base = 0;
+  if constexpr (COMPACT) rank_base = pk_wave_rank_base<INNER>(counter, rank, target);
   __builtin_amdgcn_wave_barrier();
   if (a.trace && tid == 0) a.trace[tile * 6 + 1] = wall_clock64();
   const uint32_t reserve = (cell_pairs ? cell_pairs + 1 : 0) | pk_interior_lines(cell_base, cell_pairs) << 16;
@@ -774,21 +798,30 @@
   __syncthreads();
   if (a.trace && tid == 0) a.trace[tile * 6 + 3] = wall_clock64();
   const uint32_t first_row = wave * PK_WAVE_ROWS + lane;
+  if constexpr (COMPACT) { if (lane == 0) s_scratch[24 + wave] = rank_base; }
   uint32_t first_slot[PK_ROUNDS];
 #pragma unroll
   for (uint32_t k = 0; k < PK_ROUNDS; ++k) first_slot[k] = *pk_lds_pointer(counter[k]);
 #pragma unroll
   for (uint32_t k = 0; k < PK_ROUNDS; ++k) {
     const uint32_t slot = first_slot[k] + before[k] < stage_slots - 1 ? first_slot[k] + before[k] : stage_slots - 1;
-    uint32_t tag = first_row + k * 64;
-    if constexpr (!INNER) tag |= ((target.null_partners >> k) & 1) ? PK_STAGE_NULL : 0u;
-    s_stage[slot] = u32x2_t{tag, rank[k]};
+    if constexpr (COMPACT) {
+      const uint32_t null_partner = INNER ? 0u : (target.null_partners >> k) & 1;
+#ifdef HY_DEBUG_SWITCHES
+      if (!(slot == stage_slots - 1 || null_partner || !a.build_out || rank[k] - rank_base < 65536u)) __builtin_trap();
+#endif
+      s_stage[slot] = pk_compact_pack(first_row + k * 64, null_partner, rank[k] - rank_base);
+    } else {
+      uint32_t tag = first_row + k * 64;
+      if constexpr (!INNER) tag |= ((target.null_partners >> k) & 1) ? PK_STAGE_NULL : 0u;
+      s_stage[slot] = u32x2_t{tag, rank[k]};
+    }
   }
   __syncthreads();
   if (a.trace && tid == 0) a.trace[tile * 6 + 4] = wall_clock64();
   const uint32_t lines = s_scratch[8] >> 16;
   const uint32_t chunk = view.chunk, row_begin = view.row_begin;
-#define HY_PK_COPY(BUILD) pk_copy_out<INNER, BUILD>(a, s_stage, reinterpret_cast<u32x2_t*>(s_wave_pairs), s_out_base, s_run, partitions, lines, chunk, row_begin, tid, lane, wave)
+#define HY_PK_COPY(BUILD) pk_copy_out<INNER, BUILD, COMPACT>(a, s_stage, s_scratch + 24, reinterpret_cast<u32x2_t*>(s_wave_pairs), s_out_base, s_run, partitions, lines, chunk, row_begin, tid, lane, wave)
   if (!a.build_out) HY_PK_COPY(BUILD_NONE);
   else if (a.rank.identity_rows == 65535u) HY_PK_COPY(BUILD_IDENTITY_65535);
   else if (a.rank.identity_rows) HY_PK_COPY(BUILD_IDENTITY);
@@ -855,8 +888,8 @@
   pk_cut_slice(a, blockIdx.x, s_cut, tid, tid & 63, __builtin_amdgcn_readfirstlane(tid >> 6));
 }
 
-template <bool INNER, bool MASKS = false, bool RANKS = false>
-__global__ __launch_bounds__(PK_THREADS, HY_PK_WAVES_PER_SIMD) void pk_emit(PkArgs a) {
+template <bool INNER, bool MASKS = false, bool RANKS = false, bool COMPACT = false>
+__global__ __launch_bounds__(PK_THREADS, COMPACT && INNER ? HY_PK_COMPACT_WAVES_PER_SIMD : HY_PK_WAVES_PER_SIMD) void pk_emit(PkArgs a) {
   extern __shared__ __attribute__((aligned(16))) uint32_t join_smem[];
   const uint32_t partitions = 1u << a.radix_bits;
   const uint32_t tid = threadIdx.x, lane = tid & 63, wave = __builtin_amdgcn_readfirstlane(tid >> 6);
@@ -876,5 +909,5 @@
   const size_t cell = static_cast<size_t>(tid < partitions ? tid : 0) * a.stride + tile;
   const uint32_t cell_pairs = tid < partitions ? a.counts[cell] >> 16 : 0;
   const uint32_t cell_base = static_cast<uint32_t>(a.origin_pairs[tid < partitions ? tid : 0]) + a.rel_pairs[cell];
-  pk_emit_tile<INNER, MASKS, RANKS>(a, tile, view, cell_pairs, cell_base, join_smem, tid, lane, wave);
-}
+  pk_emit_tile<INNER, MASKS, RANKS, COMPACT>(a, tile, view, cell_pairs, cell_base, join_smem, tid, lane, wave);
+}
diff --git a/hyrise_amd/csrc/runtime.hip b/hyrise_amd/csrc/runtime.hip
--- a/hyrise_amd/csrc/runtime.hip
+++ b/hyrise_amd/csrc/runtime.hip
@@ -28,6 +28,7 @@
     set(HY_OPT_STAR_FUSED_PROBE, 1);
     set(HY_OPT_STAR_FUSED_FINISH, 1);
     set(HY_OPT_LDS_ORDERED_ATOMICS, 1);
+    set(HY_OPT_JOIN_COMPACT_STAGE, 1);
   }
 };
 OptionDefaults g_option_defaults;
diff --git a/include/hyrise_amd.h b/include/hyrise_amd.h
--- a/include/hyrise_amd.h
+++ b/include/hyrise_amd.h
@@ -175,7 +175,8 @@
   HY_OPT_STAR_FUSED_FINISH = 15,
   HY_OPT_LDS_ORDERED_ATOMICS = 16,
   HY_OPT_PRODUCT_NONTEMPORAL = 17,
-  HY_OPT_COUNT = 18
+  HY_OPT_JOIN_COMPACT_STAGE = 18,
+  HY_OPT_COUNT = 19
 };
 hy_status hy_set_option(uint32_t option, int64_t value);
 hy_status hy_get_option(uint32_t option, int64_t* value);
```

Measured after the change: 385.6 billion, median of 6. 1.04x the previous value.
